# Sreyan88/audio-ssl

Hardware: AMD Instinct MI355X
Metric: upstream clips/sec (1s@16kHz, 64-mel) (higher is better)
Workload: dtype bf16; 1 GPU; delores-m upstream step (log-mel + 2 views + q/k conv encoders + MoCo + 3 Barlow heads + bwd + SGD), 1 s @ 16 kHz, 64 mel, batch 512/GPU, queue 65536; global_batch=512, parallelism=dp1

## Files before the change

audio-ssl_amd/csrc/bnpool.hip:

```cpp
#include "common.h"

namespace {

template <typename T_, bool SQ>
__global__ __launch_bounds__(256) void colstats_kernel(const T_* __restrict__ x, long M, int C, long ld, int rows_per_block,
                                                       double* __restrict__ sum, double* __restrict__ sumsq) {
    __shared__ float red[256][17];
    const int cg = threadIdx.x & 7, r0 = threadIdx.x >> 3;
    const int col0 = blockIdx.y * 64 + cg * 8;
    const long row_begin = (long)blockIdx.x * rows_per_block;
    const long row_end = min(M, row_begin + rows_per_block);
    x += (long)blockIdx.z * M * ld;
    sum += (long)blockIdx.z * C;
    if (SQ) sumsq += (long)blockIdx.z * C;
    float s[8], q[8];
#pragma unroll
    for (int i = 0; i < 8; ++i) { s[i] = 0.f; q[i] = 0.f; }
    if (col0 < C)
        for (long r = row_begin + r0; r < row_end; r += 32) {
            const Vec8<T_> v = Vec8<T_>::load(x + r * ld + col0);
#pragma unroll
            for (int i = 0; i < 8; ++i) { const float f = v.get(i); s[i] += f; if (SQ) q[i] += f * f; }
        }
#pragma unroll
    for (int i = 0; i < 8; ++i) { red[threadIdx.x][i] = s[i]; red[threadIdx.x][8 + i] = q[i]; }
    __syncthreads();
    if (threadIdx.x < 128) {
        const int g = threadIdx.x >> 4, k = threadIdx.x & 15;
        if (SQ || k < 8) {
            double t = 0.0;
            for (int r = 0; r < 32; ++r) t += (double)red[r * 8 + g][k];
            const int c = blockIdx.y * 64 + g * 8 + (k & 7);
            if (c < C) {
                if (k < 8) atomicAdd(&sum[c], t);
                else       atomicAdd(&sumsq[c], t);
            }
        }
    }
}

__global__ void bn_finalize_kernel(const double* __restrict__ sum, const double* __restrict__ sumsq, int groups, double count,
                                   int C, const float* __restrict__ gamma, const float* __restrict__ beta, float* running_mean,
                                   float* running_var, float momentum, float eps, float* scale, float* shift,
                                   float* save_mean, float* save_rstd) {
    const int c = blockIdx.x * blockDim.x + threadIdx.x;
    if (c >= C) return;
    const double g = gamma ? (double)gamma[c] : 1.0, b = beta ? (double)beta[c] : 0.0;
    float rm = running_mean ? running_mean[c] : 0.f, rv = running_mean ? running_var[c] : 0.f;
    for (int k = 0; k < groups; ++k) {
        const int o = k * C + c;
        const double mean = sum[o] / count;
        double var = sumsq[o] / count - mean * mean;
        var = var < 0.0 ? 0.0 : var;
        const double rstd = 1.0 / sqrt(var + (double)eps);
        scale[o] = (float)(g * rstd);
        shift[o] = (float)(b - mean * g * rstd);
        save_mean[o] = (float)mean;
        save_rstd[o] = (float)rstd;
        rm = (1.f - momentum) * rm + momentum * (float)mean;
        const double unb = count > 1.0 ? var * count / (count - 1.0) : var;
        rv = (1.f - momentum) * rv + momentum * (float)unb;
    }
    if (running_mean) { running_mean[c] = rm; running_var[c] = rv; }
}

template <typename TY, typename T_>
__global__ __launch_bounds__(256) void bn_relu_pool_fwd_kernel(const TY* __restrict__ Y, const float* __restrict__ scale,
                                                               const float* __restrict__ shift, T_* __restrict__ P,
                                                               int N, int Ti, int Fi) {
    const int To = Ti / 2, Fo = Fi / 2;
    const long total = (long)N * To * Fo * 8;
    const long idx = (long)blockIdx.x * 256 + threadIdx.x;
    if (idx >= total) return;
    const int c8 = (int)(idx & 7);
    long r = idx >> 3;
    const int fo = (int)(r % Fo); r /= Fo;
    const int to = (int)(r % To);
    const int n = (int)(r / To);
    float sc[8], sh[8], m[8];
#pragma unroll
    for (int i = 0; i < 8; ++i) { sc[i] = scale[c8 * 8 + i]; sh[i] = shift[c8 * 8 + i]; m[i] = 0.f; }
#pragma unroll
    for (int df = 0; df < 2; ++df)
#pragma unroll
        for (int dt = 0; dt < 2; ++dt) {
            const Vec8<TY> v = Vec8<TY>::load(Y + ((((long)n * Ti + 2 * to + dt) * Fi + 2 * fo + df) * 64 + c8 * 8));
#pragma unroll
            for (int i = 0; i < 8; ++i) m[i] = fmaxf(m[i], sc[i] * v.get(i) + sh[i]);
        }
    Vec8<T_> o;
#pragma unroll
    for (int i = 0; i < 8; ++i) o.set(i, m[i]);
    o.store(P + idx * 8);
}

template <typename TY, typename T_>
__global__ __launch_bounds__(256) void bn_relu_pool_train_fwd_kernel(const TY* __restrict__ Y, const double* __restrict__ sum,
                                                                     const double* __restrict__ sumsq, int stat_rep, double count,
                                                                     const float* __restrict__ gamma, const float* __restrict__ beta,
                                                                     float* running_mean, float* running_var, float momentum, float eps,
                                                                     T_* __restrict__ P, float* __restrict__ scale,
                                                                     float* __restrict__ shift, float* __restrict__ save_mean,
                                                                     float* __restrict__ save_rstd, int N, int Ti, int Fi) {
    __shared__ float sc_s[64], sh_s[64];
    if (threadIdx.x < 64) {
        const int c = threadIdx.x;
        const double g = (double)gamma[c], b = (double)beta[c];
        double s1 = 0.0, s2 = 0.0;
        for (int r = 0; r < stat_rep; ++r) { s1 += sum[r * 128 + c]; s2 += sumsq[r * 128 + c]; }
        const double mean = s1 / count;
        double var = s2 / count - mean * mean;
        var = var < 0.0 ? 0.0 : var;
        const double rstd = 1.0 / sqrt(var + (double)eps);
        const float sc = (float)(g * rstd), sh = (float)(b - mean * g * rstd);
        sc_s[c] = sc; sh_s[c] = sh;
        if (blockIdx.x == 0) {
            scale[c] = sc; shift[c] = sh; save_mean[c] = (float)mean; save_rstd[c] = (float)rstd;
            if (running_mean) {
                running_mean[c] = (1.f - momentum) * running_mean[c] + momentum * (float)mean;
                const double unb = count > 1.0 ? var * count / (count - 1.0) : var;
                running_var[c] = (1.f - momentum) * running_var[c] + momentum * (float)unb;
            }
        }
    }
    __syncthreads();
    const int To = Ti / 2, Fo = Fi / 2;
    const long total = (long)N * To * Fo * 8;
    const long idx = (long)blockIdx.x * 256 + threadIdx.x;
    if (idx >= total) return;
    const int c8 = (int)(idx & 7);
    long r = idx >> 3;
    const int fo = (int)(r % Fo); r /= Fo;
    const int to = (int)(r % To);
    const int n = (int)(r / To);
    float sc[8], sh[8], m[8];
#pragma unroll
    for (int i = 0; i < 8; ++i) { sc[i] = sc_s[c8 * 8 + i]; sh[i] = sh_s[c8 * 8 + i]; m[i] = 0.f; }
#pragma unroll
    for (int df = 0; df < 2; ++df)
#pragma unroll
        for (int dt = 0; dt < 2; ++dt) {
            const Vec8<TY> v = Vec8<TY>::load(Y + ((((long)n * Ti + 2 * to + dt) * Fi + 2 * fo + df) * 64 + c8 * 8));
#pragma unroll
            for (int i = 0; i < 8; ++i) m[i] = fmaxf(m[i], sc[i] * v.get(i) + sh[i]);
        }
    Vec8<T_> o;
#pragma unroll
    for (int i = 0; i < 8; ++i) o.set(i, m[i]);
    o.store(P + idx * 8);
}

template <typename T_, typename TO>
__device__ __forceinline__ void tmean_body(const T_* __restrict__ P, TO* __restrict__ xl, int N, int To, int Fo);

template <typename T_, typename TO>
__global__ __launch_bounds__(256) void tmean_fwd_kernel(const T_* __restrict__ P, TO* __restrict__ xl, int N, int To, int Fo) {
    tmean_body<T_, TO>(P, xl, N, To, Fo);
}
struct Tmean3 { const void* P[3]; void* xl[3]; int To[3], Fo[3]; const float* parts; };
template <typename T_, typename TO>
__global__ __launch_bounds__(256) void tmean3_fwd_kernel(Tmean3 a, int N) {
    const int l = blockIdx.z;
    if ((int)blockIdx.x * 64 >= a.Fo[l] * 8) return;
    if (!a.P[l]) {
        if (a.parts && l == 0) {
            const long row = (long)a.Fo[0] * 64, tot = (long)N * row;
            const long i = (long)blockIdx.y * row + blockIdx.x * 512 + threadIdx.x * 2;
            if (blockIdx.x * 512 + threadIdx.x * 2 < row) {
                float2 s = *reinterpret_cast<const float2*>(a.parts + i);
#pragma unroll
                for (int k = 1; k < 4; ++k) {
                    const float2 v = *reinterpret_cast<const float2*>(a.parts + k * tot + i);
                    s.x += v.x; s.y += v.y;
                }
                *reinterpret_cast<float2*>(static_cast<float*>(a.xl[0]) + i) = s;
            }
        }
        return;
    }
    tmean_body<T_, TO>(static_cast<const T_*>(a.P[l]), static_cast<TO*>(a.xl[l]), N, a.To[l], a.Fo[l]);
}

template <typename T_, typename TO>
__device__ __forceinline__ void tmean_body(const T_* __restrict__ P, TO* __restrict__ xl, int N, int To, int Fo) {
    __shared__ float red[4][64][9];
    const int lane = threadIdx.x & 63, w = threadIdx.x >> 6;
    const int nv = Fo * 8;
    const int v = blockIdx.x * 64 + lane;
    const int n = blockIdx.y;
    const bool live = v < nv;
    float s[8];
#pragma unroll
    for (int i = 0; i < 8; ++i) s[i] = 0.f;
    if (live) {
        const T_* p = P + ((long)n * To * nv + v) * 8;
#pragma unroll 4
        for (int t = w; t < To; t += 4) {
            const Vec8<T_> x = Vec8<T_>::load(p + (long)t * nv * 8);
#pragma unroll
            for (int i = 0; i < 8; ++i) s[i] += x.get(i);
        }
    }
#pragma unroll
    for (int i = 0; i < 8; ++i) red[w][lane][i] = s[i];
    __syncthreads();
    if (w == 0 && live) {
        Vec8<TO> o;
        const float inv = 1.f / (float)To;
#pragma unroll
        for (int i = 0; i < 8; ++i) o.set(i, (red[0][lane][i] + red[1][lane][i] + red[2][lane][i] + red[3][lane][i]) * inv);
        o.store(xl + ((long)n * nv + v) * 8);
    }
}

template <typename TY, bool APPLY, typename TG, typename T_>
__global__ __launch_bounds__(256) void bn_relu_pool_bwd_kernel(const TY* __restrict__ Y, const TG* __restrict__ dP,
                                                               const TG* __restrict__ dxl, float inv_To,
                                                               const float* __restrict__ scale, const float* __restrict__ shift,
                                                               const float* __restrict__ mean, const float* __restrict__ rstd,
                                                               float* __restrict__ stat, float inv_count,
                                                               T_* __restrict__ dY, int N, int Ti, int Fi, int fold,
                                                               float* dgamma, float* dbeta) {
    __shared__ float red[256][16];
    __shared__ float folded[128];
    if (APPLY && fold) {
        if (threadIdx.x < 128) {
            float t = 0.f;
            for (int r = 0; r < 32; ++r) t += stat[128 + r * 128 + threadIdx.x];
            folded[threadIdx.x] = t;
        }
        __syncthreads();
        if (blockIdx.x == 0 && threadIdx.x < 64 && dgamma) {
            dbeta[threadIdx.x] += folded[threadIdx.x];
            dgamma[threadIdx.x] += folded[64 + threadIdx.x];
        }
    }
    const int To = Ti / 2, Fo = Fi / 2;
    const int Tq = (Ti + 1) / 2;
    const long total = (long)N * Tq * Fo * 8;
    const long idx = (long)blockIdx.x * 256 + threadIdx.x;
    const bool live = idx < total;
    float db[8], dg[8];
#pragma unroll
    for (int i = 0; i < 8; ++i) { db[i] = 0.f; dg[i] = 0.f; }
    if (live) {
        const int c8 = (int)(idx & 7);
        long r = idx >> 3;
        const int fo = (int)(r % Fo); r /= Fo;
        const int tq = (int)(r % Tq);
        const int n = (int)(r / Tq);
        const bool pooled = tq < To;
        float sc[8], sh[8], mu[8], rs[8], g[8], cb[8], cg[8];
#pragma unroll
        for (int i = 0; i < 8; ++i) {
            const int c = c8 * 8 + i;
            sc[i] = scale[c]; sh[i] = shift[c]; mu[i] = mean[c]; rs[i] = rstd[c]; g[i] = 0.f;
            if (APPLY) { cb[i] = (fold ? folded[c] : stat[c]) * inv_count; cg[i] = (fold ? folded[64 + c] : stat[64 + c]) * inv_count; }
        }
        if (pooled) {
            const Vec8<TG> gp = Vec8<TG>::load(dP + ((((long)n * To + tq) * Fo + fo) * 64 + c8 * 8));
#pragma unroll
            for (int i = 0; i < 8; ++i) g[i] = gp.get(i);
            if (dxl) {
                const Vec8<TG> gx = Vec8<TG>::load(dxl + ((long)n * Fo * 64 + fo * 64 + c8 * 8));
#pragma unroll
                for (int i = 0; i < 8; ++i) g[i] += gx.get(i) * inv_To;
            }
        }
        Vec8<TY> y[4];
        int best[8];
        float bm[8];
#pragma unroll
        for (int i = 0; i < 8; ++i) { best[i] = 0; bm[i] = 0.f; }
#pragma unroll
        for (int p = 0; p < 4; ++p) {
            const int df = p >> 1, dt = p & 1;
            const int t = 2 * tq + dt;
            if (t < Ti) y[p] = Vec8<TY>::load(Y + ((((long)n * Ti + t) * Fi + 2 * fo + df) * 64 + c8 * 8));
            else y[p] = Vec8<TY>::zero();
#pragma unroll
            for (int i = 0; i < 8; ++i) {
                const float a = sc[i] * y[p].get(i) + sh[i];
                if (p == 0 || a > bm[i]) { bm[i] = a; best[i] = p; }
            }
        }
#pragma unroll
        for (int i = 0; i < 8; ++i) {
            const float da = (pooled && bm[i] > 0.f) ? g[i] : 0.f;
            g[i] = da;
            if (!APPLY) {
                float yb = y[0].get(i);
#pragma unroll
                for (int p = 1; p < 4; ++p) yb = best[i] == p ? y[p].get(i) : yb;
                db[i] = da;
                dg[i] = da * (yb - mu[i]) * rs[i];
            }
        }
        if (APPLY) {
#pragma unroll
            for (int p = 0; p < 4; ++p) {
                const int df = p >> 1, dt = p & 1;
                const int t = 2 * tq + dt;
                if (t >= Ti) continue;
                Vec8<T_> o;
#pragma unroll
                for (int i = 0; i < 8; ++i) {
                    const float xhat = (y[p].get(i) - mu[i]) * rs[i];
                    const float da = best[i] == p ? g[i] : 0.f;
                    o.set(i, sc[i] * (da - cb[i] - xhat * cg[i]));
                }
                o.store(dY + ((((long)n * Ti + t) * Fi + 2 * fo + df) * 64 + c8 * 8));
            }
        }
    }
    if (!APPLY) {
#pragma unroll
        for (int i = 0; i < 8; ++i) { red[threadIdx.x][i] = db[i]; red[threadIdx.x][8 + i] = dg[i]; }
        __syncthreads();
        if (threadIdx.x < 128) {
            const int kind = threadIdx.x >> 6, c = threadIdx.x & 63;
            float t = 0.f;
            for (int r = (c >> 3); r < 256; r += 8) t += red[r][kind * 8 + (c & 7)];
            atomicAdd(&stat[128 + (blockIdx.x & 31) * 128 + kind * 64 + c], t);
        }
    }
}

template <typename TP, typename TG>
__global__ __launch_bounds__(256) void bn_pool_bwd_stats_p_kernel(const TP* __restrict__ P, const TG* __restrict__ dP,
                                                                  const TG* __restrict__ dxl, float inv_To,
                                                                  const float* __restrict__ scale, const float* __restrict__ shift,
                                                                  const float* __restrict__ mean, const float* __restrict__ rstd,
                                                                  float* __restrict__ stat, int N, int To, int Fo) {
    __shared__ float red[256][16];
    const long total = (long)N * To * Fo * 8;
    float db[8], dg[8];
#pragma unroll
    for (int i = 0; i < 8; ++i) { db[i] = 0.f; dg[i] = 0.f; }
    const int c8 = threadIdx.x & 7;
    float k1[8], k0[8];
#pragma unroll
    for (int i = 0; i < 8; ++i) {
        const int c = c8 * 8 + i;
        const float sc = scale[c], inv = sc != 0.f ? 1.f / sc : 0.f;
        k1[i] = inv * rstd[c];
        k0[i] = sc != 0.f ? -(shift[c] * inv + mean[c]) * rstd[c] : 0.f;
    }
    for (long idx = (long)blockIdx.x * 256 + threadIdx.x; idx < total; idx += (long)gridDim.x * 256) {
        const long pos = idx >> 3;
        const Vec8<TP> pv = Vec8<TP>::load(P + pos * 64 + c8 * 8);
        const Vec8<TG> gp = Vec8<TG>::load(dP + pos * 64 + c8 * 8);
        float g[8];
#pragma unroll
        for (int i = 0; i < 8; ++i) g[i] = gp.get(i);
        if (dxl) {
            const long n = pos / ((long)To * Fo);
            const int fo = (int)(pos % Fo);
            const Vec8<TG> gx = Vec8<TG>::load(dxl + (n * Fo + fo) * 64 + c8 * 8);
#pragma unroll
            for (int i = 0; i < 8; ++i) g[i] += gx.get(i) * inv_To;
        }
#pragma unroll
        for (int i = 0; i < 8; ++i) {
            const float a = pv.get(i);
            const float da = a > 0.f ? g[i] : 0.f;
            db[i] += da;
            dg[i] += da * (a * k1[i] + k0[i]);
        }
    }
#pragma unroll
    for (int i = 0; i < 8; ++i) { red[threadIdx.x][i] = db[i]; red[threadIdx.x][8 + i] = dg[i]; }
    __syncthreads();
    if (threadIdx.x < 128) {
        const int kind = threadIdx.x >> 6, c = threadIdx.x & 63;
        float t = 0.f;
        for (int r = (c >> 3); r < 256; r += 8) t += red[r][kind * 8 + (c & 7)];
        atomicAdd(&stat[128 + (blockIdx.x & 31) * 128 + kind * 64 + c], t);
    }
}

__global__ void stat_reduce_kernel(float* stat) {
    const int i = threadIdx.x;
    if (i >= 128) return;
    float t = 0.f;
    for (int r = 0; r < 32; ++r) t += stat[128 + r * 128 + i];
    stat[i] = t;
}

template <typename T_>
__global__ __launch_bounds__(256) void im2col_kernel(const T_* __restrict__ X, T_* __restrict__ col, int N, int Ti, int Fi) {
    const long total = (long)N * Ti * Fi * 72;
    const long idx = (long)blockIdx.x * 256 + threadIdx.x;
    if (idx >= total) return;
    const int k8 = (int)(idx % 72);
    long pix = idx / 72;
    const int tap = k8 >> 3, c8 = k8 & 7;
    const int f = (int)(pix % Fi);
    const long r = pix / Fi;
    const int t = (int)(r % Ti);
    const long n = r / Ti;
    const int ff = f + tap / 3 - 1, tt = t + tap % 3 - 1;
    Vec8<T_> v = Vec8<T_>::zero();
    if (ff >= 0 && ff < Fi && tt >= 0 && tt < Ti) v = Vec8<T_>::load(X + (((n * Ti + tt) * Fi + ff) * 64 + c8 * 8));
    v.store(col + idx * 8);
}

template <typename T_>
__global__ void pack_conv_w_kernel(const float* __restrict__ W, T_* __restrict__ Wf, T_* __restrict__ Wd) {
    const int idx = blockIdx.x * 256 + threadIdx.x;
    if (idx >= 64 * 576) return;
    const int row = idx / 576, k = idx % 576, tap = k / 64, c = k % 64;
    Wf[idx] = from_f32<T_>(W[(row * 64 + c) * 9 + tap]);
    Wd[idx] = from_f32<T_>(W[(c * 64 + row) * 9 + (8 - tap)]);
}

template <typename T_>
__global__ void pack_conv_w2_kernel(const float* __restrict__ Wa, T_* __restrict__ Wfa, T_* __restrict__ Wda,
                                    const float* __restrict__ Wb, T_* __restrict__ Wfb, T_* __restrict__ Wdb) {
    const int idx = blockIdx.x * 256 + threadIdx.x;
    if (idx >= 64 * 576) return;
    const float* W = blockIdx.y ? Wb : Wa;
    T_* Wf = blockIdx.y ? Wfb : Wfa;
    T_* Wd = blockIdx.y ? Wdb : Wda;
    const int row = idx / 576, k = idx % 576, tap = k / 64, c = k % 64;
    Wf[idx] = from_f32<T_>(W[(row * 64 + c) * 9 + tap]);
    Wd[idx] = from_f32<T_>(W[(c * 64 + row) * 9 + (8 - tap)]);
}

__global__ void unpack_conv_dw_kernel(const float* __restrict__ dWp, float* __restrict__ dW) {
    const int idx = blockIdx.x * 256 + threadIdx.x;
    if (idx >= 64 * 576) return;
    const int co = idx / 576, k = idx % 576, tap = k / 64, ci = k % 64;
    dW[(co * 64 + ci) * 9 + tap] += dWp[idx];
}

}

extern "C" int audiossl_colstats(int dtype, const void* x, int groups, long M, int C, long ld, int want_sq, double* sum,
                                 double* sumsq, void* stream) {
    ASSL_REQUIRE(x && sum && groups > 0 && M > 0 && C > 0 && (C % 8) == 0 && (ld % 8) == 0);
    ASSL_REQUIRE((dtype == 0 || dtype == 1) && (!want_sq || sumsq));
    hipStream_t s = static_cast<hipStream_t>(stream);
    const size_t nb = sizeof(double) * C * groups;
    if (want_sq && sumsq == sum + (size_t)C * groups) {
        ASSL_ZERO(sum, 2 * nb, s);
    } else {
        ASSL_ZERO(sum, nb, s);
        if (want_sq) ASSL_ZERO(sumsq, nb, s);
    }
    const int slabs = (C + 63) / 64;
    long it = (M * slabs * groups + 32L * 2048 - 1) / (32L * 2048);
    it = it < 1 ? 1 : (it > 128 ? 128 : it);
    const int rpb = 32 * (int)it;
    const dim3 grid(ceil_div(M, rpb), slabs, groups);
    assl_dispatch(dtype, [&](auto t) { using T = typename decltype(t)::type;
        if (want_sq) hipLaunchKernelGGL((colstats_kernel<T, true>), grid, dim3(256), 0, s, static_cast<const T*>(x), M, C, ld, rpb, sum, sumsq);
        else         hipLaunchKernelGGL((colstats_kernel<T, false>), grid, dim3(256), 0, s, static_cast<const T*>(x), M, C, ld, rpb, sum, sumsq);
    });
    ASSL_LAUNCH_CHECK();
}

extern "C" int audiossl_bn_finalize(const double* sum, const double* sumsq, int groups, double count, int C,
                                    const float* gamma, const float* beta, float* running_mean, float* running_var,
                                    float momentum, float eps, float* scale, float* shift, float* save_mean, float* save_rstd,
                                    void* stream) {
    ASSL_REQUIRE(sum && sumsq && scale && shift && save_mean && save_rstd && C > 0 && count > 0 && groups > 0);
    hipLaunchKernelGGL(bn_finalize_kernel, dim3(ceil_div(C, 256)), dim3(256), 0, static_cast<hipStream_t>(stream), sum, sumsq,
                       groups, count, C, gamma, beta, running_mean, running_var, momentum, eps, scale, shift, save_mean, save_rstd);
    ASSL_LAUNCH_CHECK();
}

extern "C" int audiossl_bn_relu_pool_fwd(int dtype, int ydtype, const void* Y, const float* scale, const float* shift, void* P,
                                         int N, int Ti, int Fi, void* stream) {
    ASSL_REQUIRE(Y && scale && shift && P && N > 0 && Ti >= 2 && Fi >= 2 && (Fi % 2) == 0 && (dtype == 0 || dtype == 1));
    ASSL_REQUIRE(ydtype == 0 || ydtype == dtype);
    const long total = (long)N * (Ti / 2) * (Fi / 2) * 8;
    assl_dispatch(dtype, [&](auto to, auto ty) { using TO = typename decltype(to)::type; using TY = typename decltype(ty)::type;
        hipLaunchKernelGGL((bn_relu_pool_fwd_kernel<TY, TO>), dim3(ceil_div(total, 256)), dim3(256), 0, S_(stream),
                           static_cast<const TY*>(Y), scale, shift, static_cast<TO*>(P), N, Ti, Fi);
    }, ydtype);
    ASSL_LAUNCH_CHECK();
}

extern "C" int audiossl_bn_relu_pool_train_fwd(int dtype, int ydtype, const void* Y, const double* sum, const double* sumsq,
                                               int stat_replicas, double count,
                                               const float* gamma, const float* beta, float* running_mean, float* running_var,
                                               float momentum, float eps, void* P, float* scale, float* shift, float* save_mean,
                                               float* save_rstd, int N, int Ti, int Fi, void* stream) {
    ASSL_REQUIRE(Y && sum && sumsq && gamma && beta && P && scale && shift && save_mean && save_rstd && count > 0.0);
    ASSL_REQUIRE(stat_replicas >= 1 && (stat_replicas == 1 || sumsq == sum + 64));
    ASSL_REQUIRE(N > 0 && Ti >= 2 && Fi >= 2 && (Fi % 2) == 0 && (dtype == 0 || dtype == 1) && (ydtype == 0 || ydtype == dtype));
    const long total = (long)N * (Ti / 2) * (Fi / 2) * 8;
    assl_dispatch(dtype, [&](auto to, auto ty) { using TO = typename decltype(to)::type; using TY = typename decltype(ty)::type;
        hipLaunchKernelGGL((bn_relu_pool_train_fwd_kernel<TY, TO>), dim3(ceil_div(total, 256)), dim3(256), 0, S_(stream),
                           static_cast<const TY*>(Y), sum, sumsq, stat_replicas, count, gamma, beta, running_mean, running_var,
                           momentum, eps, static_cast<TO*>(P), scale, shift, save_mean, save_rstd, N, Ti, Fi);
    }, ydtype);
    ASSL_LAUNCH_CHECK();
}

extern "C" int audiossl_tmean_fwd(int dtype, int out_f32, const void* P, void* xl, int N, int To, int Fo, void* stream) {
    ASSL_REQUIRE(P && xl && N > 0 && To > 0 && Fo > 0 && (dtype == 0 || dtype == 1));
    assl_dispatch(dtype, [&](auto ti, auto to) { using TI = typename decltype(ti)::type; using TO = typename decltype(to)::type;
        hipLaunchKernelGGL((tmean_fwd_kernel<TI, TO>), dim3(ceil_div(Fo * 8, 64), N), dim3(256), 0, S_(stream), static_cast<const TI*>(P),
                           static_cast<TO*>(xl), N, To, Fo);
    }, out_f32 ? 0 : dtype);
    ASSL_LAUNCH_CHECK();
}

extern "C" int audiossl_tmean3_fwd(int dtype, int out_f32, const void* P1, void* x1, const float* x1_parts, int To1, int Fo1,
                                   const void* P2, void* x2, int To2, int Fo2, const void* P3, void* x3, int To3, int Fo3, int N,
                                   void* stream) {
    ASSL_REQUIRE(x1 && P2 && x2 && P3 && x3 && N > 0 && To1 > 0 && To2 > 0 && To3 > 0 && Fo1 > 0 && Fo2 > 0 && Fo3 > 0);
    ASSL_REQUIRE((P1 != nullptr) != (x1_parts != nullptr) && (!x1_parts || (out_f32 && dtype == 1)));
    ASSL_REQUIRE(dtype == 0 || dtype == 1);
    Tmean3 a{{P1, P2, P3}, {x1, x2, x3}, {To1, To2, To3}, {Fo1, Fo2, Fo3}, x1_parts};
    const int gx = ceil_div(max(Fo1, max(Fo2, Fo3)) * 8, 64);
    assl_dispatch(dtype, [&](auto ti, auto to) { using TI = typename decltype(ti)::type; using TO = typename decltype(to)::type;
        hipLaunchKernelGGL((tmean3_fwd_kernel<TI, TO>), dim3(gx, N, 3), dim3(256), 0, S_(stream), a, N);
    }, out_f32 ? 0 : dtype);
    ASSL_LAUNCH_CHECK();
}

namespace {
__global__ void add_stat_kernel(const float* __restrict__ stat, float* dgamma, float* dbeta) {
    const int c = threadIdx.x;
    if (c < 64) { dbeta[c] += stat[c]; dgamma[c] += stat[64 + c]; }
}
}

static int bn_relu_pool_bwd_run(int phase, int dtype, int ydtype, int gdtype, const void* Y, const void* P, const void* dP, const void* dxl,
                                const float* scale, const float* shift, const float* mean, const float* rstd, float* stat,
                                const float* gstat, double count, void* dY, float* dgamma, float* dbeta, int N, int Ti, int Fi,
                                void* stream) {
    ASSL_REQUIRE(Y && dP && scale && shift && mean && rstd && stat);
    ASSL_REQUIRE(N > 0 && Ti >= 2 && Fi >= 2 && (Fi % 2) == 0 && (dtype == 0 || dtype == 1) && (gdtype == 0 || gdtype == dtype));
    ASSL_REQUIRE(ydtype == 0 || ydtype == dtype);
    ASSL_REQUIRE(phase == 1 || (dY && dgamma && dbeta));
    hipStream_t s = static_cast<hipStream_t>(stream);
    if (phase != 2) ASSL_ZERO(stat, sizeof(float) * 128 * 33, s);
    const long total = (long)N * ((Ti + 1) / 2) * (Fi / 2) * 8;
    const int grid = ceil_div(total, 256);
    const float inv_To = 1.f / (float)(Ti / 2);
    const float inv_count = (float)(1.0 / (phase == 2 ? count : (double)N * Ti * Fi));
    float* apply_stat = phase == 2 ? const_cast<float*>(gstat) : stat;
    const int fold = phase == 0;
    const long ptotal = (long)N * (Ti / 2) * (Fi / 2) * 8;
    const int pgrid = (int)min((long)2048, (ptotal + 255) / 256);
    assl_dispatch(dtype, [&](auto to, auto ty, auto tg) {
        using TO = typename decltype(to)::type; using TY = typename decltype(ty)::type; using TG = typename decltype(tg)::type;
        const TY* y = static_cast<const TY*>(Y);
        const TG *g = static_cast<const TG*>(dP), *gx = static_cast<const TG*>(dxl);
        TO* dy = static_cast<TO*>(dY);
        if (phase != 2) {
            if (P) hipLaunchKernelGGL((bn_pool_bwd_stats_p_kernel<TO, TG>), dim3(pgrid), dim3(256), 0, s, static_cast<const TO*>(P), g, gx,
                                      inv_To, scale, shift, mean, rstd, stat, N, Ti / 2, Fi / 2);
            else hipLaunchKernelGGL((bn_relu_pool_bwd_kernel<TY, false, TG, TO>), dim3(grid), dim3(256), 0, s, y, g, gx, inv_To, scale,
                                    shift, mean, rstd, stat, inv_count, dy, N, Ti, Fi, 0, dgamma, dbeta);
            if (!fold) hipLaunchKernelGGL(stat_reduce_kernel, dim3(1), dim3(128), 0, s, stat);
        }
        if (phase != 1) hipLaunchKernelGGL((bn_relu_pool_bwd_kernel<TY, true, TG, TO>), dim3(grid), dim3(256), 0, s, y, g, gx, inv_To,
                                           scale, shift, mean, rstd, apply_stat, inv_count, dy, N, Ti, Fi, fold, dgamma, dbeta);
    }, ydtype, gdtype);
    if (phase == 2) hipLaunchKernelGGL(add_stat_kernel, dim3(1), dim3(64), 0, s, stat, dgamma, dbeta);
    ASSL_LAUNCH_CHECK();
}

extern "C" int audiossl_bn_relu_pool_bwd(int dtype, int ydtype, int gdtype, const void* Y, const void* dP, const void* dxl, const float* scale,
                                         const float* shift, const float* mean, const float* rstd, float* stat, void* dY,
                                         float* dgamma, float* dbeta, int N, int Ti, int Fi, void* stream) {
    return bn_relu_pool_bwd_run(0, dtype, ydtype, gdtype, Y, nullptr, dP, dxl, scale, shift, mean, rstd, stat, nullptr, 0.0, dY, dgamma, dbeta, N,
                                Ti, Fi, stream);
}
extern "C" int audiossl_bn_relu_pool_bwd_p(int dtype, int ydtype, int gdtype, const void* Y, const void* P, const void* dP, const void* dxl,
                                           const float* scale, const float* shift, const float* mean, const float* rstd, float* stat,
                                           void* dY, float* dgamma, float* dbeta, int N, int Ti, int Fi, void* stream) {
    ASSL_REQUIRE(P);
    return bn_relu_pool_bwd_run(0, dtype, ydtype, gdtype, Y, P, dP, dxl, scale, shift, mean, rstd, stat, nullptr, 0.0, dY, dgamma, dbeta, N,
                                Ti, Fi, stream);
}
extern "C" int audiossl_bn_relu_pool_bwd_stats(int dtype, int ydtype, int gdtype, const void* Y, const void* dP, const void* dxl,
                                               const float* scale, const float* shift, const float* mean, const float* rstd,
                                               float* stat, int N, int Ti, int Fi, void* stream) {
    return bn_relu_pool_bwd_run(1, dtype, ydtype, gdtype, Y, nullptr, dP, dxl, scale, shift, mean, rstd, stat, nullptr, 0.0, nullptr, nullptr,
                                nullptr, N, Ti, Fi, stream);
}
extern "C" int audiossl_bn_relu_pool_bwd_apply(int dtype, int ydtype, int gdtype, const void* Y, const void* dP, const void* dxl,
                                               const float* scale, const float* shift, const float* mean, const float* rstd,
                                               float* stat, const float* gstat, double count_global, void* dY, float* dgamma,
                                               float* dbeta, int N, int Ti, int Fi, void* stream) {
    ASSL_REQUIRE(gstat && count_global > 1.0);
    return bn_relu_pool_bwd_run(2, dtype, ydtype, gdtype, Y, nullptr, dP, dxl, scale, shift, mean, rstd, stat, gstat, count_global, dY, dgamma,
                                dbeta, N, Ti, Fi, stream);
}

extern "C" int audiossl_im2col3x3(int dtype, const void* X, void* col, int N, int Ti, int Fi, void* stream) {
    ASSL_REQUIRE(X && col && N > 0 && Ti > 0 && Fi > 0 && (dtype == 0 || dtype == 1));
    const long total = (long)N * Ti * Fi * 72;
    ASSL_REQUIRE((total + 255) / 256 < 2147483647L);
    assl_dispatch(dtype, [&](auto t) { using T = typename decltype(t)::type;
        hipLaunchKernelGGL(im2col_kernel<T>, dim3(ceil_div(total, 256)), dim3(256), 0, S_(stream), static_cast<const T*>(X),
                           static_cast<T*>(col), N, Ti, Fi);
    });
    ASSL_LAUNCH_CHECK();
}

extern "C" int audiossl_pack_conv_w(int dtype, const float* W, void* Wf, void* Wd, void* stream) {
    ASSL_REQUIRE(W && Wf && Wd && (dtype == 0 || dtype == 1));
    assl_dispatch(dtype, [&](auto t) { using T = typename decltype(t)::type;
        hipLaunchKernelGGL(pack_conv_w_kernel<T>, dim3(144), dim3(256), 0, S_(stream), W, static_cast<T*>(Wf), static_cast<T*>(Wd));
    });
    ASSL_LAUNCH_CHECK();
}

extern "C" int audiossl_pack_conv_w2(int dtype, const float* Wa, void* Wfa, void* Wda, const float* Wb, void* Wfb, void* Wdb, void* stream) {
    ASSL_REQUIRE(Wa && Wfa && Wda && Wb && Wfb && Wdb && (dtype == 0 || dtype == 1));
    assl_dispatch(dtype, [&](auto t) { using T = typename decltype(t)::type;
        hipLaunchKernelGGL(pack_conv_w2_kernel<T>, dim3(144, 2), dim3(256), 0, S_(stream), Wa, static_cast<T*>(Wfa), static_cast<T*>(Wda), Wb,
                           static_cast<T*>(Wfb), static_cast<T*>(Wdb));
    });
    ASSL_LAUNCH_CHECK();
}

extern "C" int audiossl_unpack_conv_dw(const float* dWp, float* dW, void* stream) {
    ASSL_REQUIRE(dWp && dW);
    hipLaunchKernelGGL(unpack_conv_dw_kernel, dim3(144), dim3(256), 0, static_cast<hipStream_t>(stream), dWp, dW);
    ASSL_LAUNCH_CHECK();
}
```

audio-ssl_amd/csrc/conv.hip:

```cpp
#include <cstdlib>
#include "common.h"

namespace {

constexpr int CH = 64, KTOT = 576;
constexpr int WPITCH = KTOT + 8;
constexpr int PIXP = 72;
constexpr int PIXW = 96;

typedef __attribute__((address_space(3))) bf16x4* lds4_t;

struct ConvArgs {
    const bf16* X; const bf16* W; const float* bias; bf16* Y; double* sum; double* sumsq;
    int Ti, rows_total, tiles, out_f32, dbg, stat_rep;
};

template <int FI, int PITCH, int NTH = 256>
struct Halo {
    static constexpr int TT = 256 / FI;
    static constexpr int COLS = FI + 2;
    static constexpr int ELEMS = (TT + 2) * COLS * PITCH;
    static constexpr int NV = ((TT + 2) * FI * 8 + NTH - 1) / NTH;
    static constexpr int NVEC = (TT + 2) * FI * 8;
    Vec8<bf16> r[NV];
    __device__ __forceinline__ void load(const bf16* __restrict__ X, int g0, int rows_total) {
#pragma unroll
        for (int i = 0; i < NV; ++i) {
            const int v = threadIdx.x + i * NTH;
            const int row = v / (FI * 8), rem = v % (FI * 8);
            const int gr = g0 - 1 + row;
            r[i] = (v < NVEC && gr >= 0 && gr < rows_total) ? Vec8<bf16>::load(X + ((long)gr * FI) * CH + rem * 8) : Vec8<bf16>::zero();
        }
    }
    __device__ __forceinline__ void put(bf16* lds) const {
#pragma unroll
        for (int i = 0; i < NV; ++i) {
            const int v = threadIdx.x + i * NTH;
            const int row = v / (FI * 8), rem = v % (FI * 8);
            if (v < NVEC) r[i].store(lds + (row * COLS + (rem >> 3) + 1) * PITCH + (rem & 7) * 8);
        }
    }
    __device__ __forceinline__ static void zero_border(bf16* lds) {
        for (int i = threadIdx.x; i < (TT + 2) * 2 * 8; i += NTH) {
            const int row = i / 16, side = (i >> 3) & 1, c8 = i & 7;
            Vec8<bf16>::zero().store(lds + (row * COLS + side * (FI + 1)) * PITCH + c8 * 8);
        }
    }
};

template <int FI, int NW>
__global__ __launch_bounds__(64 * NW, 1) void conv3x3_kernel(ConvArgs a) {
    using H = Halo<FI, PIXP, 64 * NW>;
    constexpr int RT = 8 / NW;
    constexpr int TT = H::TT, COLS = H::COLS;
    extern __shared__ __attribute__((aligned(16))) char smem[];
    bf16* const wl = reinterpret_cast<bf16*>(smem);
    bf16* const hl = wl + CH * WPITCH;
    float* const red = reinterpret_cast<float*>(hl);

    const int lane = threadIdx.x & 63, wave = threadIdx.x >> 6;
    const int m = lane & 31, h = lane >> 5;
    for (int v = threadIdx.x; v < CH * KTOT / 8; v += 64 * NW) {
        const int row = v / (KTOT / 8), c = v % (KTOT / 8);
        Vec8<bf16>::load(a.W + row * KTOT + c * 8).store(wl + row * WPITCH + c * 8);
    }
    H::zero_border(hl);

    float ssum[2][16], ssq[2][16];
#pragma unroll
    for (int j = 0; j < 2; ++j)
#pragma unroll
        for (int r = 0; r < 16; ++r) { ssum[j][r] = 0.f; ssq[j][r] = 0.f; }
    f32x4 bias4[2][4];
#pragma unroll
    for (int j = 0; j < 2; ++j)
#pragma unroll
        for (int q = 0; q < 4; ++q)
            bias4[j][q] = a.bias ? *reinterpret_cast<const f32x4*>(a.bias + j * 32 + 8 * q + 4 * h) : f32x4{0.f, 0.f, 0.f, 0.f};
    H halo;
    int tile = blockIdx.x;
    if (tile < a.tiles) { halo.load(a.X, tile * TT, a.rows_total); halo.put(hl); }
    __syncthreads();

    for (; tile < a.tiles; tile += gridDim.x) {
        const int g0 = tile * TT;
        const int next = tile + gridDim.x;
        if (next < a.tiles && !(a.dbg & 2)) halo.load(a.X, next * TT, a.rows_total);

        int tl[RT], fcol[RT];
        bool ok[RT][3];
#pragma unroll
        for (int i = 0; i < RT; ++i) {
            const int rt = RT * wave + i;
            tl[i] = FI == 32 ? rt : 2 * rt + (m >> 4);
            fcol[i] = FI == 32 ? m : (m & 15);
            const int g = g0 + tl[i];
            const int ti = g % a.Ti;
#pragma unroll
            for (int dt = 0; dt < 3; ++dt) ok[i][dt] = g < a.rows_total && ti + dt - 1 >= 0 && ti + dt - 1 < a.Ti;
        }
        f32x16 acc[RT][2];
#pragma unroll
        for (int i = 0; i < RT; ++i)
#pragma unroll
            for (int j = 0; j < 2; ++j)
#pragma unroll
                for (int r = 0; r < 16; ++r) acc[i][j][r] = 0.f;

        if (!(a.dbg & 4))
#pragma unroll
        for (int tap = 0; tap < 9; ++tap) {
            const int dt = tap % 3, df = tap / 3;
#pragma unroll
            for (int cc = 0; cc < 4; ++cc) {
                Vec8<bf16> fa[RT], fb[2];
#pragma unroll
                for (int i = 0; i < RT; ++i) {
                    const bf16* p = hl + ((tl[i] + dt) * COLS + fcol[i] + df) * PIXP + cc * 16 + 8 * h;
                    fa[i] = ok[i][dt] ? Vec8<bf16>::load(p) : Vec8<bf16>::zero();
                }
#pragma unroll
                for (int j = 0; j < 2; ++j) fb[j] = Vec8<bf16>::load(wl + (j * 32 + m) * WPITCH + tap * 64 + cc * 16 + 8 * h);
#pragma unroll
                for (int i = 0; i < RT; ++i)
#pragma unroll
                    for (int j = 0; j < 2; ++j)
                        acc[i][j] = __builtin_amdgcn_mfma_f32_32x32x16_bf16(fb[j].v, fa[i].v, acc[i][j], 0, 0, 0);
            }
        }
#pragma unroll
        for (int i = 0; i < RT; ++i) {
            const int g = g0 + tl[i];
            if (g < a.rows_total && !(a.dbg & 1)) {
                const long o = ((long)g * FI + fcol[i]) * CH;
#pragma unroll
                for (int j = 0; j < 2; ++j)
#pragma unroll
                    for (int q = 0; q < 4; ++q) {
                        f32x4 v;
#pragma unroll
                        for (int e = 0; e < 4; ++e) {
                            v[e] = acc[i][j][4 * q + e] + bias4[j][q][e];
                            ssum[j][4 * q + e] += v[e];
                            ssq[j][4 * q + e] += v[e] * v[e];
                        }
                        const int co = j * 32 + 8 * q + 4 * h;
                        if (a.out_f32) *reinterpret_cast<f32x4*>(reinterpret_cast<float*>(a.Y) + o + co) = v;
                        else *reinterpret_cast<bf16x4*>(a.Y + o + co) = bf16x4{(bf16)v[0], (bf16)v[1], (bf16)v[2], (bf16)v[3]};
                    }
            }
        }
        __syncthreads();
        if (next < a.tiles) halo.put(hl);
        __syncthreads();
    }
    if (a.sum) {
#pragma unroll
        for (int j = 0; j < 2; ++j)
#pragma unroll
            for (int r = 0; r < 16; ++r) {
                float s = ssum[j][r], q = ssq[j][r];
#pragma unroll
                for (int o = 16; o > 0; o >>= 1) { s += __shfl_xor(s, o, 64); q += __shfl_xor(q, o, 64); }
                if (m == 0) {
                    const int co = j * 32 + (r & 3) + 8 * (r >> 2) + 4 * h;
                    red[(wave * 64 + co) * 2] = s; red[(wave * 64 + co) * 2 + 1] = q;
                }
            }
        __syncthreads();
        if (threadIdx.x < 128) {
            const int c = threadIdx.x >> 1, k = threadIdx.x & 1;
            double t = 0.0;
#pragma unroll
            for (int w = 0; w < NW; ++w) t += (double)red[(w * 64 + c) * 2 + k];
            const int rep = (blockIdx.x % a.stat_rep) * 128;
            atomicAdd(k == 0 ? &a.sum[rep + c] : &a.sumsq[rep + c], t);
        }
    }
}

template <int FI>
struct WsGeom {
    static constexpr int TT = 256 / FI, COLS = FI + 2, ROWS = TT + 2, SEGS = FI / 8;
    static constexpr int UNITS = ROWS * SEGS;
    static constexpr int UPW = (UNITS + 3) / 4;
    static constexpr int BYTES = ROWS * COLS * 128;
};

template <int FI, bool STATS, bool F32OUT, int PF = 2>
__global__ __launch_bounds__(256, 1) void conv3x3_ws_kernel(ConvArgs a) {
    using G = WsGeom<FI>;
    constexpr int TT = G::TT, COLS = G::COLS;
    typedef __attribute__((address_space(3))) void* lptr_t;
    extern __shared__ __attribute__((aligned(16))) char smem[];
    float* const biasl = reinterpret_cast<float*>(smem + 2 * G::BYTES);
    float* const red = biasl + 64;
    constexpr int OPIX = F32OUT ? 256 : 128;
    char* const stg = reinterpret_cast<char*>(red + 4 * 64 * 2) + (threadIdx.x >> 6) * 64 * OPIX;
    char* const zblk = reinterpret_cast<char*>(red + 4 * 64 * 2) + 4 * 64 * OPIX;
    if (threadIdx.x < 32) *reinterpret_cast<f32x4*>(zblk + threadIdx.x * 16) = f32x4{0.f, 0.f, 0.f, 0.f};

    const int lane = threadIdx.x & 63, wave = __builtin_amdgcn_readfirstlane(threadIdx.x >> 6);
    const int m = lane & 31, h = lane >> 5;
    long* const rts = (!STATS && (a.dbg & 16) && threadIdx.x == 0 && (blockIdx.x == 0 || blockIdx.x == gridDim.x - 1))
                          ? reinterpret_cast<long*>(a.sum) + 64 + (blockIdx.x ? 8 : 0) : nullptr;
    if (rts) rts[0] = __builtin_amdgcn_s_memrealtime();

    {
        bf16* const wl = reinterpret_cast<bf16*>(smem);
        Vec8<bf16> tmp[CH * KTOT / 8 / 256];
#pragma unroll
        for (int k = 0; k < CH * KTOT / 8 / 256; ++k) tmp[k] = Vec8<bf16>::load(a.W + (threadIdx.x + 256 * k) * 8);
#pragma unroll
        for (int k = 0; k < CH * KTOT / 8 / 256; ++k) {
            const int v = threadIdx.x + 256 * k, row = v / (KTOT / 8), c = v % (KTOT / 8);
            tmp[k].store(wl + row * WPITCH + c * 8);
        }
        __syncthreads();
    }
    Vec8<bf16> wr[2][36];
#pragma unroll
    for (int j = 0; j < 2; ++j)
#pragma unroll
        for (int ks = 0; ks < 36; ++ks)
            wr[j][ks] = Vec8<bf16>::load(reinterpret_cast<const bf16*>(smem) + (j * 32 + m) * WPITCH + ks * 16 + 8 * h);
#pragma unroll
    for (int ks = 0; ks < 36; ++ks) {
        asm volatile("" : "+v"(wr[0][ks].v));
        asm volatile("" : "+a"(wr[1][ks].v));
    }

    __syncthreads();
    for (int i = threadIdx.x; i < 2 * G::ROWS * 2 * 8; i += 256) {
        const int b = i / (G::ROWS * 16), r = (i / 16) % G::ROWS, side = (i >> 3) & 1, c8 = i & 7;
        *reinterpret_cast<f32x4*>(smem + b * G::BYTES + (r * COLS + side * (FI + 1)) * 128 + c8 * 16) = f32x4{0.f, 0.f, 0.f, 0.f};
    }
    if (threadIdx.x < 64) biasl[threadIdx.x] = a.bias ? a.bias[threadIdx.x] : 0.f;

    if (rts) { asm volatile("s_waitcnt vmcnt(0)" ::: "memory"); rts[3] = __builtin_amdgcn_s_memrealtime(); }
    const __amdgpu_buffer_rsrc_t rsrc = __builtin_amdgcn_make_buffer_rsrc(const_cast<bf16*>(a.X), 0, (unsigned)((long)a.rows_total * FI * 128), 0x00020000);
    const int pl = lane >> 3, cp = lane & 7;
    const int key0 = ((1 + pl) >> 1) & 7;
    const int voff0 = pl * 128 + ((cp ^ key0) << 4), voff1 = pl * 128 + ((cp ^ key0 ^ 4) << 4);
    auto dma_unit = [&](int g0, char* buf, int i) {
        {
            const int u = wave + 4 * i;
            if (u < G::UNITS) {
                const int row = u / G::SEGS, seg = u % G::SEGS;
                const int gr = g0 - 1 + row;
                const int so = (gr >= 0 && gr < a.rows_total) ? (gr * FI + 8 * seg) * 128 : 0x7FFFFF00;
                __builtin_amdgcn_raw_ptr_buffer_load_lds(rsrc, (lptr_t)(buf + (row * COLS + 1 + 8 * seg) * 128), 16, (seg & 1) ? voff1 : voff0, so, 0, 0);
            }
        }
    };
    auto dma_tile = [&](int g0, char* buf) {
#pragma unroll
        for (int i = 0; i < G::UPW; ++i) dma_unit(g0, buf, i);
    };

    int tl[2];
    const int fcol = FI == 32 ? m : (m & 15);
#pragma unroll
    for (int i = 0; i < 2; ++i) {
        const int rt = 2 * wave + i;
        tl[i] = FI == 32 ? rt : 2 * rt + (m >> 4);
    }
    int hs[3];
#pragma unroll
    for (int df = 0; df < 3; ++df) hs[df] = (h ^ (((fcol + df) >> 1) & 7)) << 4;

    constexpr int NS = F32OUT ? 4 : 8;
    float ssum[NS], ssq[NS];
    if (STATS) {
#pragma unroll
        for (int e = 0; e < NS; ++e) { ssum[e] = 0.f; ssq[e] = 0.f; }
    }

    int tile = blockIdx.x, cur = 0;
    if (tile < a.tiles) dma_tile(tile * TT, smem);
    asm volatile("s_waitcnt vmcnt(0) lgkmcnt(0)" ::: "memory");
    __builtin_amdgcn_s_barrier();

    long* const ts = (!STATS && (a.dbg & 16) && blockIdx.x == 0 && threadIdx.x == 0) ? reinterpret_cast<long*>(a.sum) : nullptr;
    int tsi = 0;
    if (rts) rts[1] = __builtin_amdgcn_s_memrealtime();
    for (; tile < a.tiles; tile += gridDim.x, cur ^= 1) {
        if (ts) ts[tsi++] = __builtin_amdgcn_s_memtime();
        const int g0 = tile * TT;
        const int next = tile + gridDim.x;
        if (next < a.tiles && !(a.dbg & 2)) dma_tile(next * TT, smem + (cur ^ 1) * G::BYTES);
        const char* const hl = smem + cur * G::BYTES;

        int bdt[2][3];
#pragma unroll
        for (int i = 0; i < 2; ++i) {
            const int g = g0 + tl[i];
            const int ti = g % a.Ti;
#pragma unroll
            for (int dt = 0; dt < 3; ++dt) {
                const bool ok = g < a.rows_total && ti + dt - 1 >= 0 && ti + dt - 1 < a.Ti;
                bdt[i][dt] = ok ? (int)(size_t)((lptr_t)const_cast<char*>(hl)) + ((tl[i] + dt) * COLS + fcol) * 128
                                : (int)(size_t)((lptr_t)zblk);
            }
        }
        f32x16 acc[2][2];
#pragma unroll
        for (int j = 0; j < 2; ++j)
#pragma unroll
            for (int q = 0; q < 4; ++q) {
                const f32x4 b4 = *reinterpret_cast<const f32x4*>(biasl + j * 32 + 8 * q + 4 * h);
#pragma unroll
                for (int e = 0; e < 4; ++e) { acc[0][j][4 * q + e] = b4[e]; acc[1][j][4 * q + e] = b4[e]; }
            }

        Vec8<bf16> fa[PF + 1][2];
        auto fetch = [&](int ks, Vec8<bf16> (&f)[2]) {
            const int tap = ks >> 2, cc = ks & 3, dt = tap % 3, df = tap / 3;
#pragma unroll
            for (int i = 0; i < 2; ++i)
                f[i] = Vec8<bf16>::load(reinterpret_cast<const bf16*>((const char*)(lptr_t)(size_t)(bdt[i][dt] + df * 128 + (hs[df] ^ (cc * 32)))));
        };
        if (!(a.dbg & 4)) {
#pragma unroll
        for (int ks = 0; ks < PF; ++ks) fetch(ks, fa[ks]);
#pragma unroll
        for (int ks = 0; ks < 36; ++ks) {
            if (ks + PF < 36) fetch(ks + PF, fa[(ks + PF) % (PF + 1)]);
            __builtin_amdgcn_sched_barrier(0);
            Vec8<bf16> (&f)[2] = fa[ks % (PF + 1)];
#pragma unroll
            for (int i = 0; i < 2; ++i) {
#pragma unroll
                for (int j = 0; j < 2; ++j)
                    acc[i][j] = __builtin_amdgcn_mfma_f32_32x32x16_bf16(wr[j][ks].v, f[i].v, acc[i][j], 0, 0, 0);
            }
            __builtin_amdgcn_sched_barrier(0);
        }
        }
        if (ts) ts[tsi++] = __builtin_amdgcn_s_memtime();
        asm volatile("s_waitcnt vmcnt(0)" ::: "memory");
        if (ts) ts[tsi++] = __builtin_amdgcn_s_memtime();
        if (!(a.dbg & 1)) {
#pragma unroll
            for (int i = 0; i < 2; ++i) {
                char* const st = stg + i * 32 * OPIX;
#pragma unroll
                for (int j = 0; j < 2; ++j)
#pragma unroll
                    for (int q = 0; q < 4; ++q) {
                        const int slot = j * 8 + 2 * q + h;
                        const f32x4 v = f32x4{acc[i][j][4 * q], acc[i][j][4 * q + 1], acc[i][j][4 * q + 2], acc[i][j][4 * q + 3]};
                        if (F32OUT) *reinterpret_cast<f32x4*>(st + m * 256 + ((slot ^ (m & 15)) << 4)) = v;
                        else *reinterpret_cast<bf16x4*>(st + m * 128 + ((slot ^ ((m >> 1) & 15)) << 3)) =
                                 bf16x4{(bf16)v[0], (bf16)v[1], (bf16)v[2], (bf16)v[3]};
                    }
            }
            asm volatile("s_waitcnt lgkmcnt(0)" ::: "memory");
#pragma unroll
            for (int i = 0; i < 2; ++i) {
                const char* const st = stg + i * 32 * OPIX;
                const int grow = g0 + (2 * wave + i) * (32 / FI);
                const int prow_ok = a.rows_total - grow;
                char* const yrow = reinterpret_cast<char*>(a.Y) + (long)grow * FI * 64 * (F32OUT ? 4 : 2);
                if (F32OUT) {
#pragma unroll
                    for (int it = 0; it < 8; ++it) {
                        const int p = it * 4 + (lane >> 4), c = lane & 15;
                        const f32x4 v = *reinterpret_cast<const f32x4*>(st + p * 256 + ((c ^ (p & 15)) << 4));
                        if ((p >> (FI == 32 ? 5 : 4)) < prow_ok) {
                            *reinterpret_cast<f32x4*>(yrow + p * 256 + c * 16) = v;
                            if (STATS) {
#pragma unroll
                                for (int e = 0; e < 4; ++e) { ssum[e] += v[e]; ssq[e] += v[e] * v[e]; }
                            }
                        }
                    }
                } else {
#pragma unroll
                    for (int it = 0; it < 4; ++it) {
                        const int p = it * 8 + (lane >> 3), c = lane & 7, k = (p >> 1) & 15;
                        f32x4 v = *reinterpret_cast<const f32x4*>(st + p * 128 + ((c ^ (k >> 1)) << 4));
                        if (k & 1) v = f32x4{v[2], v[3], v[0], v[1]};
                        if ((p >> (FI == 32 ? 5 : 4)) < prow_ok) {
                            *reinterpret_cast<f32x4*>(yrow + p * 128 + c * 16) = v;
                            if (STATS) {
                                const bf16x8 hv = __builtin_bit_cast(bf16x8, v);
#pragma unroll
                                for (int e = 0; e < 8; ++e) {
                                    const float x = (float)hv[e];
                                    ssum[e] += x; ssq[e] += x * x;
                                }
                            }
                        }
                    }
                }
            }
        }
        if (ts) ts[tsi++] = __builtin_amdgcn_s_memtime();
        asm volatile("s_waitcnt lgkmcnt(0)" ::: "memory");
        __builtin_amdgcn_s_barrier();
    }
    if (rts) rts[2] = __builtin_amdgcn_s_memrealtime();
    if (STATS) {
#pragma unroll
        for (int e = 0; e < NS; ++e) {
            float s = ssum[e], q = ssq[e];
#pragma unroll
            for (int o = 64 / NS; o < 64; o <<= 1) { s += __shfl_xor(s, o, 64); q += __shfl_xor(q, o, 64); }
            if (lane < 64 / NS) {
                const int co = lane * NS + e;
                red[(wave * 64 + co) * 2] = s; red[(wave * 64 + co) * 2 + 1] = q;
            }
        }
        __syncthreads();
        if (threadIdx.x < 128) {
            const int c = threadIdx.x >> 1, k = threadIdx.x & 1;
            double t = 0.0;
#pragma unroll
            for (int w = 0; w < 4; ++w) t += (double)red[(w * 64 + c) * 2 + k];
            const int rep = (blockIdx.x % a.stat_rep) * 128;
            atomicAdd(k == 0 ? &a.sum[rep + c] : &a.sumsq[rep + c], t);
        }
    }
}

__host__ __device__ __forceinline__ int wg_cot(int w, int n) { return n < 8 ? (n & 1) : (w & 1); }
__host__ __device__ __forceinline__ int wg_nt(int w, int n) { return n < 8 ? 4 * w + (n >> 1) : 16 + (w >> 1); }

struct WgradArgs {
    const bf16* dY; const bf16* X; float* dW; int Ti, rows_total, tiles;
    float* partial;
    int dbg;
};

template <int FI, int KG>
__global__ __launch_bounds__(256 * KG, 1) void conv3x3_wgrad_kernel(WgradArgs a) {
    using H = Halo<FI, PIXW, 256 * KG>;
    constexpr int TT = H::TT, COLS = H::COLS;
    constexpr int NTH = 256 * KG;
    constexpr int NVY = 256 * 8 / NTH;
    extern __shared__ __attribute__((aligned(16))) char smem[];
    bf16* const yl = reinterpret_cast<bf16*>(smem);
    bf16* const hl = yl + 256 * PIXW;

    const int lane = threadIdx.x & 63, wave = (threadIdx.x >> 6) & 3, grp = threadIdx.x >> 8;
    const int h = lane >> 5, half = (lane >> 4) & 1, q = (lane & 15) >> 2, p = lane & 3;
    H::zero_border(hl);

    f32x16 acc[9];
#pragma unroll
    for (int n = 0; n < 9; ++n)
#pragma unroll
        for (int r = 0; r < 16; ++r) acc[n][r] = 0.f;

    H halo;
    Vec8<bf16> ry[NVY];
    auto load_y = [&](int g0) {
#pragma unroll
        for (int i = 0; i < NVY; ++i) {
            const int v = threadIdx.x + i * NTH;
            const long pix = (long)g0 * FI + (v >> 3);
            ry[i] = pix < (long)a.rows_total * FI ? Vec8<bf16>::load(a.dY + pix * CH + (v & 7) * 8) : Vec8<bf16>::zero();
        }
    };
    auto put_y = [&]() {
#pragma unroll
        for (int i = 0; i < NVY; ++i) {
            const int v = threadIdx.x + i * NTH;
            ry[i].store(yl + (v >> 3) * PIXW + (v & 7) * 8);
        }
    };
    int tile = blockIdx.x;
    if (tile < a.tiles) { halo.load(a.X, tile * TT, a.rows_total); load_y(tile * TT); halo.put(hl); put_y(); }
    __syncthreads();

    for (; tile < a.tiles; tile += gridDim.x) {
        const int g0 = tile * TT;
        const int next = tile + gridDim.x;
        if (next < a.tiles && !(a.dbg & 2)) { halo.load(a.X, next * TT, a.rows_total); load_y(next * TT); }

#pragma unroll 1
        for (int ks = grp * (16 / KG); ks < (grp + 1) * (16 / KG) && !(a.dbg & 4); ++ks) {
            const int t_local = FI == 32 ? (ks >> 1) : ks;
            const int f0 = FI == 32 ? (ks & 1) * 16 : 0;
            const int g = g0 + t_local;
            if (g >= a.rows_total) break;
            const int ti = g % a.Ti;
            const bool okt[3] = {ti - 1 >= 0, true, ti + 1 < a.Ti};
            bf16x8 fa[2];
#pragma unroll
            for (int c2 = 0; c2 < 2; ++c2) {
                const bf16* ay = yl + (ks * 16 + 8 * h + q) * PIXW + c2 * 32 + 16 * half + 4 * p;
                const bf16x4 a0 = __builtin_amdgcn_ds_read_tr16_b64_v4bf16((lds4_t)ay);
                const bf16x4 a1 = __builtin_amdgcn_ds_read_tr16_b64_v4bf16((lds4_t)(ay + 4 * PIXW));
                fa[c2] = bf16x8{a0[0], a0[1], a0[2], a0[3], a1[0], a1[1], a1[2], a1[3]};
            }
            bf16x8 fb;
#pragma unroll
            for (int n = 0; n < 9; ++n) {
                if (n == 8 || (n & 1) == 0) {
                    const int nt = wg_nt(wave, n), tap = nt >> 1, cih = nt & 1;
                    const int dt = tap % 3, df = tap / 3;
                    const bf16* bx = hl + ((t_local + dt) * COLS + f0 + df + 8 * h + q) * PIXW + cih * 32 + 16 * half + 4 * p;
                    const bf16x4 b0 = __builtin_amdgcn_ds_read_tr16_b64_v4bf16((lds4_t)bx);
                    const bf16x4 b1 = __builtin_amdgcn_ds_read_tr16_b64_v4bf16((lds4_t)(bx + 4 * PIXW));
                    const bf16 z = (bf16)0.f;
                    fb = okt[dt] ? bf16x8{b0[0], b0[1], b0[2], b0[3], b1[0], b1[1], b1[2], b1[3]} : bf16x8{z, z, z, z, z, z, z, z};
                }
                const int c2 = wg_cot(wave, n);
                acc[n] = __builtin_amdgcn_mfma_f32_32x32x16_bf16(c2 ? fa[1] : fa[0], fb, acc[n], 0, 0, 0);
            }
        }
        __syncthreads();
        if (next < a.tiles) { halo.put(hl); put_y(); }
        __syncthreads();
    }
    if (a.partial) {
        if (KG == 2) {
            f32x4* xch = reinterpret_cast<f32x4*>(smem);
            __syncthreads();
            if (grp == 1) {
#pragma unroll
                for (int n = 0; n < 9; ++n)
#pragma unroll
                    for (int r4 = 0; r4 < 4; ++r4)
                        xch[((wave * 9 + n) * 4 + r4) * 64 + lane] = f32x4{acc[n][4 * r4], acc[n][4 * r4 + 1], acc[n][4 * r4 + 2], acc[n][4 * r4 + 3]};
            }
            __syncthreads();
            if (grp == 1) return;
            f32x4* part = reinterpret_cast<f32x4*>(a.partial + (long)blockIdx.x * (CH * KTOT));
#pragma unroll
            for (int n = 0; n < 9; ++n)
#pragma unroll
                for (int r4 = 0; r4 < 4; ++r4) {
                    const f32x4 o = xch[((wave * 9 + n) * 4 + r4) * 64 + lane];
                    part[((wave * 9 + n) * 4 + r4) * 64 + lane] = f32x4{acc[n][4 * r4] + o[0], acc[n][4 * r4 + 1] + o[1], acc[n][4 * r4 + 2] + o[2], acc[n][4 * r4 + 3] + o[3]};
                }
            return;
        }
        f32x4* part = reinterpret_cast<f32x4*>(a.partial + (long)blockIdx.x * (CH * KTOT));
#pragma unroll
        for (int n = 0; n < 9; ++n)
#pragma unroll
            for (int r4 = 0; r4 < 4; ++r4)
                part[((wave * 9 + n) * 4 + r4) * 64 + lane] = f32x4{acc[n][4 * r4], acc[n][4 * r4 + 1], acc[n][4 * r4 + 2], acc[n][4 * r4 + 3]};
        return;
    }
#pragma unroll
    for (int n = 0; n < 9; ++n) {
        const int nt = wg_nt(wave, n), tap = nt >> 1, cih = nt & 1;
        const int col = tap * 64 + cih * 32 + (lane & 31);
#pragma unroll
        for (int r = 0; r < 16; ++r) {
            const int co = wg_cot(wave, n) * 32 + (r & 3) + 8 * (r >> 2) + 4 * h;
            atomicAdd(&a.dW[co * KTOT + col], acc[n][r]);
        }
    }
}

__global__ __launch_bounds__(256) void wgrad_reduce_kernel(const float* __restrict__ partial, int nparts, float* __restrict__ dW) {
    const int i = blockIdx.x * 256 + threadIdx.x;
    if (i >= CH * KTOT) return;
    float s0 = 0.f, s1 = 0.f, s2 = 0.f, s3 = 0.f;
    int w = blockIdx.y;
    const int step = gridDim.y;
    for (; w + 3 * step < nparts; w += 4 * step) {
        s0 += partial[(long)w * (CH * KTOT) + i];
        s1 += partial[(long)(w + step) * (CH * KTOT) + i];
        s2 += partial[(long)(w + 2 * step) * (CH * KTOT) + i];
        s3 += partial[(long)(w + 3 * step) * (CH * KTOT) + i];
    }
    for (; w < nparts; w += step) s0 += partial[(long)w * (CH * KTOT) + i];
    const int e = i & 3, lane = (i >> 2) & 63, r4 = (i >> 8) & 3, wn = i >> 10;
    const int wave = wn / 9, n = wn - wave * 9;
    const int nt = wg_nt(wave, n), tap = nt >> 1, cih = nt & 1;
    const int col = tap * 64 + cih * 32 + (lane & 31);
    const int co = wg_cot(wave, n) * 32 + e + 8 * r4 + 4 * (lane >> 5);
    atomicAdd(&dW[co * KTOT + col], (s0 + s1) + (s2 + s3));
}

template <typename K>
int set_lds(K kernel, size_t bytes) {
    return hipFuncSetAttribute(reinterpret_cast<const void*>(kernel), hipFuncAttributeMaxDynamicSharedMemorySize, (int)bytes) ==
           hipSuccess ? 0 : -1;
}

}

extern "C" int audiossl_conv3x3_fwd(const void* X, const void* W, const float* bias, void* Y, int out_f32, double* sum,
                                    double* sumsq, int stat_replicas, int N, int Ti, int Fi, void* stream) {
    ASSL_REQUIRE(X && W && Y && N > 0 && Ti > 0 && (Fi == 32 || Fi == 16) && (!sum == !sumsq));
    ASSL_REQUIRE(stat_replicas >= 1 && stat_replicas <= 64 && (stat_replicas == 1 || !sum || sumsq == sum + 64));
    if (!ASSL_ALIGNED16(X) || !ASSL_ALIGNED16(W) || !ASSL_ALIGNED16(Y)) return ASSL_EALIGN;
    hipStream_t s = static_cast<hipStream_t>(stream);
#ifdef AUDIOSSL_ABLATE
    static const int conv_dbg = getenv("AUDIOSSL_CONV_DBG") ? atoi(getenv("AUDIOSSL_CONV_DBG")) : 0;
#else
    constexpr int conv_dbg = 0;
#endif
    if (sum && !(conv_dbg & 16)) {
        if (sumsq == sum + 64) {
            ASSL_ZERO(sum, sizeof(double) * 128 * stat_replicas, s);
        } else {
            ASSL_ZERO(sum, sizeof(double) * 64, s);
            ASSL_ZERO(sumsq, sizeof(double) * 64, s);
        }
    }
    const int rows = N * Ti, TT = 256 / Fi, tiles = (rows + TT - 1) / TT;
    ConvArgs a{static_cast<const bf16*>(X), static_cast<const bf16*>(W), bias, static_cast<bf16*>(Y), sum, sumsq, Ti, rows, tiles, out_f32, conv_dbg, stat_replicas};
    const int grid = tiles < 256 ? tiles : 256;
    static const int ws = getenv("AUDIOSSL_CONV_WS") ? atoi(getenv("AUDIOSSL_CONV_WS")) : 1;
    if (ws && (long)rows * Fi * 128 < 0x7FFFFF00L) {
        static bool wattr[8] = {false, false, false, false, false, false, false, false};
#define WS_LAUNCH(FI_, ST_, F32_, SLOT)                                                                    \
    do {                                                                                                  \
        const size_t lds = 2 * WsGeom<FI_>::BYTES + sizeof(float) * (64 + 4 * 64 * 2) + 4 * 64 * (F32_ ? 256 : 128) + 512; \
        if (!wattr[SLOT]) { if (set_lds(conv3x3_ws_kernel<FI_, ST_, F32_>, lds)) return ASSL_ELAUNCH; wattr[SLOT] = true; } \
        hipLaunchKernelGGL((conv3x3_ws_kernel<FI_, ST_, F32_>), dim3(grid), dim3(256), lds, s, a);       \
    } while (0)
        if (Fi == 32) {
            if (sum && !(conv_dbg & 16)) { if (out_f32) WS_LAUNCH(32, true, true, 0); else WS_LAUNCH(32, true, false, 1); }
            else     { if (out_f32) WS_LAUNCH(32, false, true, 2); else WS_LAUNCH(32, false, false, 3); }
        } else {
            if (sum) { if (out_f32) WS_LAUNCH(16, true, true, 4); else WS_LAUNCH(16, true, false, 5); }
            else     { if (out_f32) WS_LAUNCH(16, false, true, 6); else WS_LAUNCH(16, false, false, 7); }
        }
#undef WS_LAUNCH
        ASSL_LAUNCH_CHECK();
    }
    static const int nw = getenv("AUDIOSSL_CONV_WAVES") ? atoi(getenv("AUDIOSSL_CONV_WAVES")) : 8;
    static bool attr[4] = {false, false, false, false};
#define CONV_LAUNCH(FI_, NW_, SLOT)                                                                       \
    do {                                                                                                  \
        const size_t lds = sizeof(bf16) * (CH * WPITCH + Halo<FI_, PIXP>::ELEMS);                         \
        if (!attr[SLOT]) { if (set_lds(conv3x3_kernel<FI_, NW_>, lds)) return ASSL_ELAUNCH; attr[SLOT] = true; } \
        hipLaunchKernelGGL((conv3x3_kernel<FI_, NW_>), dim3(grid), dim3(64 * NW_), lds, s, a);           \
    } while (0)
    if (Fi == 32) { if (nw == 8) CONV_LAUNCH(32, 8, 0); else CONV_LAUNCH(32, 4, 1); }
    else          { if (nw == 8) CONV_LAUNCH(16, 8, 2); else CONV_LAUNCH(16, 4, 3); }
#undef CONV_LAUNCH
    ASSL_LAUNCH_CHECK();
}

extern "C" int audiossl_conv3x3_wgrad(const void* dY, const void* X, float* dWp, float* workspace, long workspace_floats, int N,
                                      int Ti, int Fi, void* stream) {
    ASSL_REQUIRE(dY && X && dWp && N > 0 && Ti > 0 && (Fi == 32 || Fi == 16));
    if (!ASSL_ALIGNED16(X) || !ASSL_ALIGNED16(dY)) return ASSL_EALIGN;
    hipStream_t s = static_cast<hipStream_t>(stream);
    const int rows = N * Ti, TT = 256 / Fi, tiles = (rows + TT - 1) / TT;
    const int grid = tiles < 256 ? tiles : 256;
    const bool two_stage = workspace != nullptr && workspace_floats >= (long)grid * CH * KTOT;
#ifdef AUDIOSSL_ABLATE
    static const int wg_dbg = getenv("AUDIOSSL_CONV_DBG") ? atoi(getenv("AUDIOSSL_CONV_DBG")) : 0;
#else
    constexpr int wg_dbg = 0;
#endif
    WgradArgs a{static_cast<const bf16*>(dY), static_cast<const bf16*>(X), dWp, Ti, rows, tiles, two_stage ? workspace : nullptr, wg_dbg};
    static const int kg_env = getenv("AUDIOSSL_WGRAD_KG") ? atoi(getenv("AUDIOSSL_WGRAD_KG")) : 0;
    const int kg = kg_env ? kg_env : (two_stage ? 2 : 1);
    static bool attr[4] = {false, false, false, false};
#define WGRAD_LAUNCH(FI_, KG_, SLOT)                                                                      \
    do {                                                                                                  \
        const size_t lds = max(sizeof(bf16) * (256 * PIXW + Halo<FI_, PIXW>::ELEMS), (size_t)(KG_ == 2 ? 4 * 9 * 16 * 64 * 4 : 0)); \
        if (!attr[SLOT]) { if (set_lds(conv3x3_wgrad_kernel<FI_, KG_>, lds)) return ASSL_ELAUNCH; attr[SLOT] = true; } \
        hipLaunchKernelGGL((conv3x3_wgrad_kernel<FI_, KG_>), dim3(grid), dim3(256 * KG_), lds, s, a);    \
    } while (0)
    if (Fi == 32) { if (kg == 2) WGRAD_LAUNCH(32, 2, 0); else WGRAD_LAUNCH(32, 1, 1); }
    else          { if (kg == 2) WGRAD_LAUNCH(16, 2, 2); else WGRAD_LAUNCH(16, 1, 3); }
#undef WGRAD_LAUNCH
    if (two_stage)
        hipLaunchKernelGGL(wgrad_reduce_kernel, dim3(CH * KTOT / 256, 8), dim3(256), 0, s, workspace, grid, dWp);
    ASSL_LAUNCH_CHECK();
}
```

audio-ssl_amd/src/encoder/audiontt.py:

```python
import logging
import os
import re
from pathlib import Path

import torch
from torch import nn

from src import _native as N
from src import engine as E

_DROPOUT_IN_GEMM = os.environ.get("AUDIOSSL_DROPOUT_IN_GEMM", "1") != "0"


def default_precision():
    return {"fp32": N.F32, "bf16": N.BF16}[os.environ.get("AUDIOSSL_PRECISION", "bf16")]


class NetworkCommonMixIn():

    def load_weight(self, weight_file, device):
        state_dict = torch.load(weight_file, map_location=device, weights_only=True)
        if 'state_dict' in state_dict:
            state_dict = state_dict['state_dict']
        weights = {}
        for k in state_dict:
            m = re.search(r'(^fc\.|\.fc\.|^features\.|\.features\.)', k)
            if m is None:
                continue
            new_k = k[m.start():]
            weights[new_k[1:] if new_k[0] == '.' else new_k] = state_dict[k]
        self.load_state_dict(weights)
        self.eval()
        logging.info(f'Using audio embbeding network pretrained weight: {Path(weight_file).name}')
        return self

    def set_trainable(self, trainable=False):
        for p in self.parameters():
            p.requires_grad = trainable


class DropoutMasks:

    def __init__(self, p=0.3, seed=0x5EED):
        self.p, self.seed, self.queue = p, seed, []
        self.counter = None

    @property
    def calls(self):
        return 0 if self.counter is None else int(self.counter[0])

    def next(self, M, d, device, virtual=False):
        if self.queue:
            m = self.queue.pop(0)
            return m.reshape(M, d).to(device=device, dtype=torch.uint8).contiguous()
        if self.counter is None or self.counter.device != torch.device(device):
            self.counter = torch.zeros(1, dtype=torch.int64, device=device)
        self.counter.add_(1)
        vk = VirtualKeep((self.seed * 0x9E3779B1) & 0xFFFFFFFFFFFF, self.p, self.counter, M, d)
        return vk if virtual else vk.materialise()


class VirtualKeep:

    def __init__(self, seed, p, counter, M, d):
        self.seed, self.p, self.counter, self.M, self.d = seed, p, counter, M, d

    def materialise(self):
        keep = torch.empty(self.M, self.d, dtype=torch.uint8, device=self.counter.device)
        N.call("dropout_mask", keep, self.M * self.d, self.seed, self.p, self.counter)
        return keep


class _EncoderFn(torch.autograd.Function):

    @staticmethod
    def forward(ctx, mod, x, keep, *params):
        P = mod.param_dict()
        x1, x2, x3, h, c = E.encoder_forward(P, x, mod.precision, keep=keep, p_drop=mod.fc[2].p, train=mod.training)
        ctx.mod, ctx.c = mod, c
        return x1, x2, x3, h

    @staticmethod
    def backward(ctx, g1, g2, g3, gh):
        mod, c = ctx.mod, ctx.c
        td = N.torch_dtype(c.dtype)
        P = mod.param_dict()
        names = mod.engine_param_names()
        G = {n: torch.zeros_like(P[n], dtype=torch.float32) for n in names}

        def prep(g, like):
            return None if g is None else g.float().contiguous()
        gh = torch.zeros_like(c.H2.view(c.N, -1, c.d)) if gh is None else gh.to(td).contiguous()
        E.encoder_backward(c, G, dH2=gh.view(c.M, c.d), dx1=prep(g1, None), dx2=prep(g2, None), dx3=prep(g3, None))
        return (None, None, None) + tuple(G[n] for n in names)


class AudioNTT2020Task6(nn.Module, NetworkCommonMixIn):

    def __init__(self, n_mels, d, return_all_layers):
        super().__init__()
        self.return_all_layers = return_all_layers

        def block(cin):
            return nn.Sequential(nn.Conv2d(cin, 64, 3, stride=1, padding=1), nn.BatchNorm2d(64), nn.ReLU(),
                                 nn.MaxPool2d(2, stride=2))
        self.features_1 = block(1)
        self.features_2 = block(64)
        self.features_3 = block(64)
        self.fc = nn.Sequential(nn.Linear(64 * (n_mels // (2 ** 3)), d), nn.ReLU(), nn.Dropout(p=0.3), nn.Linear(d, d),
                                nn.ReLU())
        self.d = d
        self.n_mels = n_mels
        self.precision = default_precision()
        self.dropout_masks = DropoutMasks(0.3)

    def param_dict(self):
        from src.flat import cached_param_dict
        return cached_param_dict(self)

    def engine_param_names(self):
        return [n for n, _ in self.named_parameters()]

    def next_keep_mask(self, n_img, T):
        if not self.training:
            return None
        return self.dropout_masks.next(n_img * (T // 8), self.d, self.fc[0].weight.device, virtual=_DROPOUT_IN_GEMM)

    def forward(self, x):
        if not x.is_cuda:
            raise RuntimeError("AudioNTT2020Task6 (HIP) needs a GPU tensor - there is no CPU fallback")
        x = x.float().contiguous()
        keep = self.next_keep_mask(x.shape[0], x.shape[-1])
        params = tuple(p for _, p in self.named_parameters())
        if torch.is_grad_enabled() and any(p.requires_grad for p in params):
            x1, x2, x3, h = _EncoderFn.apply(self, x, keep, *params)
        else:
            x1, x2, x3, h, _ = E.encoder_forward(self.param_dict(), x, self.precision, keep=keep, p_drop=self.fc[2].p,
                                                 train=self.training)
        if self.return_all_layers:
            return x1, x2, x3, h
        return h

    def __repr__(self):
        return "AudioNTT2020Task6"
```

audio-ssl_amd/src/engine.py:

```python
import os

import torch

from src import _native as N

import os as _os
_STEM_VALU = _os.environ.get("AUDIOSSL_STEM_VALU") == "1"
BN_MOMENTUM = 0.1
BN_EPS = 1e-5
_BN_FUSED = _os.environ.get("AUDIOSSL_BN_FUSED", "1") != "0"


ONE_STREAM = os.environ.get("AUDIOSSL_ONE_STREAM", "0") == "1"


_CAPTURE_ORIGIN = []


class capture_scope:

    def __enter__(self):
        _CAPTURE_ORIGIN.append(torch.cuda.current_stream())
        return self

    def __exit__(self, *exc):
        _CAPTURE_ORIGIN.pop()
        return False


def fork(side, parent=None, device=None):
    parent = parent if parent is not None else torch.cuda.current_stream(device)
    if _CAPTURE_ORIGIN and parent.cuda_stream != _CAPTURE_ORIGIN[-1].cuda_stream and side.cuda_stream != _CAPTURE_ORIGIN[-1].cuda_stream \
            and os.environ.get("AUDIOSSL_ALLOW_NESTED_FORK", "0") != "1":
        raise RuntimeError("nested stream fork inside a hipGraph capture: a side stream may only be forked from the capture's origin "
                           "stream (a fork from an already forked stream crashed hipStreamEndCapture on ROCm 7.2 - engine.py, "
                           "DESIGN.md section 7); restructure the step or set AUDIOSSL_ALLOW_NESTED_FORK=1 to experiment")
    side.wait_stream(parent)


class SideStream:

    def __init__(self):
        self._streams = {}

    def stream(self, device):
        if ONE_STREAM:
            return torch.cuda.current_stream(device)
        key = str(device)
        if key not in self._streams:
            self._streams[key] = torch.cuda.Stream(device=device)
        return self._streams[key]

    def run(self, device, fn):
        if ONE_STREAM:
            return fn()
        s = self.stream(device)
        fork(s, torch.cuda.current_stream(device))
        with torch.cuda.stream(s):
            return fn()

    def join(self, device):
        if not ONE_STREAM:
            torch.cuda.current_stream(device).wait_stream(self.stream(device))


WGRAD = SideStream()


def _empty(shape, dtype, like=None, device=None):
    return torch.empty(shape, dtype=dtype, device=device if device is not None else like.device)


class ZeroArena:

    def __init__(self, nbytes=8 << 20):
        self.nbytes, self.buf, self.off, self.active = nbytes, None, 0, False

    def step(self, device):
        arena = self

        class _Ctx:
            def __enter__(self_):
                if arena.buf is None or arena.buf.device != device:
                    arena.buf = torch.empty(arena.nbytes, dtype=torch.uint8, device=device)
                arena.off, arena.active = 0, True
                arena.buf.zero_()
                N.call_host("set_prezeroed", 1)

            def __exit__(self_, *exc):
                arena.active = False
                N.call_host("set_prezeroed", 0)
                return False
        return _Ctx()

    def zeros(self, shape, dtype, like=None, device=None):
        dev = device if device is not None else like.device
        if self.active and self.buf.device == dev:
            n = 1
            for d in (shape if isinstance(shape, (tuple, list)) else (shape,)):
                n *= int(d)
            nb = n * torch.empty((), dtype=dtype).element_size()
            if self.off + nb <= self.nbytes:
                t = self.buf[self.off:self.off + nb].view(dtype).view(shape)
                self.off += (nb + 255) // 256 * 256
                return t
        return torch.zeros(shape, dtype=dtype, device=dev)

    def scratch(self, shape, dtype, like):
        return self.zeros(shape, dtype, like=like) if self.active else _empty(shape, dtype, like=like)


ARENA = ZeroArena()


def fast_copy(dst, src):
    n = src.numel()
    if src.dtype == torch.float32 and dst.dtype == torch.float32 and src.is_contiguous() and dst.is_contiguous() and n % 1024 == 0 \
            and n // 1024 < (1 << 31) and src.data_ptr() % 16 == 0 and dst.data_ptr() % 16 == 0:
        N.call("tile_rows", src, dst, n // 1024, n // 1024, 1, 1.0, 1024)
    else:
        dst.copy_(src)
    return dst


def _ksplit(M, Nn, K, target=512):
    tiles = ((M + 127) // 128) * ((Nn + 127) // 128)
    return int(max(1, min(target // max(tiles, 1), (K // 64) // 32)))


def gemm(dtype, ta, tb, M, Nn, K, A, lda, B, ldb, C, ldc, alpha=1.0, bias=None, relu=0, keep=None, ldk=0, keep_scale=1.0,
         gate=None, ldg=0, out_f32=0, atomic=0, ksplit=1, resid=None, ldr=0):
    N.call("gemm", dtype, ta, tb, M, Nn, K, float(alpha), A, lda, B, ldb, C, ldc, bias, relu, keep, ldk, float(keep_scale),
           gate, ldg, out_f32, atomic, ksplit, resid, ldr)


def linear_fwd(dtype, X, W, M, Nout, K, bias=None, relu=0, keep=None, keep_scale=1.0, out=None, out_f32=0):
    if out is None and dtype == N.BF16 and out_f32 and not relu and keep is None and M * Nout <= (1 << 16) and K >= 1024 and K % 512 == 0:
        out = ARENA.zeros((M, Nout), torch.float32, like=X)
        gemm(dtype, 0, 0, M, Nout, K, X, K, W, K, out, Nout, bias=bias, out_f32=1, atomic=1, ksplit=min(8, K // 256))
        return out
    if out is None:
        out = _empty((M, Nout), torch.float32 if (out_f32 or dtype == 0) else torch.bfloat16, like=X)
    gemm(dtype, 0, 0, M, Nout, K, X, K, W, K, out, Nout, bias=bias, relu=relu, keep=keep, ldk=Nout, keep_scale=keep_scale,
         out_f32=out_f32)
    return out


def linear_bwd_w(dtype, dY, X, dW, M, Nout, K, dw_zero=False):
    ks = _ksplit(Nout, K, M)
    atomic = 1 if (ks > 1 or dtype != N.BF16) else (0 if dw_zero else 2)
    gemm(dtype, 1, 1, Nout, K, M, dY, Nout, X, K, dW, K, out_f32=1, atomic=atomic, ksplit=ks)


def linear_bwd_x(dtype, dY, W, M, Nout, K, alpha=1.0, gate=None, out=None, out_f32=0):
    if out is None:
        out = _empty((M, K), torch.float32 if (out_f32 or dtype == N.F32) else torch.bfloat16, like=dY)
    gemm(dtype, 0, 1, M, K, Nout, dY, Nout, W, K, out, K, alpha=alpha, gate=gate, ldg=K, out_f32=out_f32)
    return out


GD = N.F32

HP = False


def set_high_precision(flag):
    global HP
    HP = bool(flag)


SYNC_BN = None


class SyncBN:
    def __init__(self, group=None):
        import torch.distributed as dist
        self.dist, self.group = dist, group
        self.world = dist.get_world_size(group)

    def all_reduce(self, t):
        self.dist.all_reduce(t, group=self.group)
        return t


def set_sync_bn(sync):
    global SYNC_BN
    SYNC_BN = sync if (sync is not None and sync.world > 1) else None


def _ad(dtype):
    return N.F32 if (HP or dtype == N.F32) else dtype


def pooled_dtype(dtype):
    return torch.float32


def center_cast(Y, groups, B):
    C = Y.shape[1]
    yc = _empty((groups * B, C), torch.bfloat16, like=Y)
    cmean = _empty((groups, C), torch.float32, like=Y)
    N.call("center_cast", Y, yc, cmean, groups, B, C)
    return yc, cmean


def colsum_add(dtype, X, M, C, dst, tmp=None):
    tmp = tmp if tmp is not None else ARENA.scratch((C,), torch.float64, X)
    N.call("colstats", dtype, X, 1, M, C, C, 0, tmp, None)
    N.call("add_d2f", tmp, dst, C)


def cast(dtype, src, n=None):
    if dtype == N.F32:
        return src
    out = torch.empty(src.shape, dtype=torch.bfloat16, device=src.device)
    N.call("cast", dtype, src, out, src.numel())
    return out


class EncoderCtx:
    pass


def _bn_train(dtype, Y, M, C, gamma, beta, rm, rv, update_running, groups=1):
    sq = ARENA.scratch((2, groups * C), torch.float64, Y)
    N.call("colstats", dtype, Y, groups, M, C, C, 1, sq[0], sq[1])
    if SYNC_BN is not None:
        SYNC_BN.all_reduce(sq)
        M = M * SYNC_BN.world
    st = _empty((4, groups * C), torch.float32, like=Y)
    N.call("bn_finalize", sq[0], sq[1], groups, float(M), C, gamma, beta, rm if update_running else None,
           rv if update_running else None, BN_MOMENTUM, BN_EPS, st[0], st[1], st[2], st[3])
    return st[0], st[1], st[2], st[3]


def bn_train_apply(dtype, ad, a, M, C, gamma, beta, rm, rv, update_running, groups, relu, out):
    if M <= 1024 and C % 32 == 0 and _BN_FUSED and SYNC_BN is None:
        st = _empty((4, groups * C), torch.float32, like=a)
        N.call("colbn_train_fwd", dtype, ad, a, gamma, beta, rm if update_running else None, rv if update_running else None,
               BN_MOMENTUM, BN_EPS, relu, groups, M, C, out, st[0], st[1], st[2], st[3])
        return st[0], st[1], st[2], st[3]
    st = _bn_train(ad, a, M, C, gamma, beta, rm, rv, update_running, groups)
    N.call("colbn_fwd", dtype, ad, a, st[0], st[1], relu, out, groups, M, C)
    return st


def _bn_eval(like, C, gamma, beta, rm, rv):
    scale, shift = _empty((C,), torch.float32, like=like), _empty((C,), torch.float32, like=like)
    N.call("bn_eval_affine", gamma, beta, rm, rv, BN_EPS, C, scale, shift)
    return scale, shift


_WGRAD_WS = {}


def _wgrad_workspace(device):
    key = device.index if device.index is not None else torch.cuda.current_device()
    ws = _WGRAD_WS.get(key)
    if ws is None:
        ws = _WGRAD_WS[key] = torch.empty(256 * 64 * 576, dtype=torch.float32, device=device)
    return ws


STAT_REPLICAS = 8
LOSS_REPLICAS = 32
_BN_STATS_P = os.environ.get("AUDIOSSL_BN_STATS_P", "1") != "0"
_DP1_BF16 = os.environ.get("AUDIOSSL_DP1_BF16", "1") != "0"


def _conv_block_fwd(dtype, Pin, Nimg, Ti, Fi, W, bias, bn, train, update_running, col, packed=None):
    td = N.torch_dtype(dtype)
    if packed is not None:
        Wf, Wd = packed
    else:
        Wf, Wd = _empty((64, 576), td, like=Pin), _empty((64, 576), td, like=Pin)
        N.call("pack_conv_w", dtype, W, Wf, Wd)
    M = Nimg * Ti * Fi
    ad = _ad(dtype)
    Y = _empty((M, 64), N.torch_dtype(ad), like=Pin)
    gamma, beta, rm, rv = bn
    fused = dtype == N.BF16 and Fi in (16, 32)
    rep = STAT_REPLICAS if (fused and train and SYNC_BN is None) else 1
    sq = ARENA.scratch((rep, 2, 64), torch.float64, Pin) if (fused and train) else None
    if fused:
        N.call("conv3x3_fwd", Pin, Wf, bias, Y, int(ad == N.F32), None if sq is None else sq[0, 0], None if sq is None else sq[0, 1],
               rep, Nimg, Ti, Fi)
    else:
        N.call("im2col3x3", dtype, Pin, col, Nimg, Ti, Fi)
        gemm(dtype, 0, 0, M, 64, 576, col, 576, Wf, 576, Y, 64, bias=bias, out_f32=int(ad == N.F32))
    Pout = _empty((Nimg, Ti // 2, Fi // 2, 64), td, like=Pin)
    if train and fused and SYNC_BN is None:
        st = _empty((4, 64), torch.float32, like=Pin)
        N.call("bn_relu_pool_train_fwd", dtype, ad, Y, sq[0, 0], sq[0, 1], rep, float(M), gamma, beta, rm if update_running else None,
               rv if update_running else None, BN_MOMENTUM, BN_EPS, Pout, st[0], st[1], st[2], st[3], Nimg, Ti, Fi)
        return Y, Pout, (st[0], st[1], st[2], st[3]), Wf, Wd
    if train and fused:
        st = _empty((4, 64), torch.float32, like=Pin)
        sq = sq[0]
        SYNC_BN.all_reduce(sq)
        N.call("bn_finalize", sq[0], sq[1], 1, float(M * SYNC_BN.world), 64, gamma, beta, rm if update_running else None,
               rv if update_running else None, BN_MOMENTUM, BN_EPS, st[0], st[1], st[2], st[3])
        scale, shift, mean, rstd = st[0], st[1], st[2], st[3]
    elif train:
        scale, shift, mean, rstd = _bn_train(ad, Y, M, 64, gamma, beta, rm, rv, update_running)
    else:
        scale, shift = _bn_eval(Y, 64, gamma, beta, rm, rv)
        mean = rstd = None
    N.call("bn_relu_pool_fwd", dtype, ad, Y, scale, shift, Pout, Nimg, Ti, Fi)
    return Y, Pout, (scale, shift, mean, rstd), Wf, Wd


def _col_buffer(dtype, Nimg, T1, F1, like):
    if dtype == N.BF16 and F1 in (16, 32):
        return None
    return _empty((Nimg * T1 * F1, 576), N.torch_dtype(dtype), like=like)


MOM_SLOT = 17 * 54


def stem_fused(dtype, train=True):
    return bool(train) and dtype == N.BF16 and not HP and not _STEM_VALU and SYNC_BN is None


def stem_moments_pair(xa, xb=None):
    Nimg, _, F, T = xa.shape
    assert xb is None or xb.shape == xa.shape
    mom = ARENA.scratch((1 if xb is None else 2, MOM_SLOT), torch.float64, xa)
    N.call("conv1_moments_pair", xa.reshape(Nimg, F, T).contiguous(), None if xb is None else xb.reshape(Nimg, F, T).contiguous(),
           Nimg, F, T, mom)
    return mom


def encoder_forward(P, x, dtype, keep=None, p_drop=0.3, train=True, update_running=True, want_layers=True, Wc=None,
                    layer_out=None, before_fc=None, stem_moments=None):
    Nimg, _, F, T = x.shape
    assert F == 64, "the HIP encoder is built for n_mels = 64 (the reference's only setting)"
    td = N.torch_dtype(dtype)
    c = EncoderCtx()
    c.P = P
    c.dtype, c.N, c.F, c.T, c.train, c.p_drop = dtype, Nimg, F, T, train, p_drop
    img = x.reshape(Nimg, F, T).contiguous()
    c.img = img
    w1 = P["features_1.0.weight"].reshape(64, 9)
    b1 = P["features_1.0.bias"]
    g1, be1 = P["features_1.1.weight"], P["features_1.1.bias"]
    c.stem_mfma = dtype == N.BF16 and not HP and not _STEM_VALU
    fused = stem_fused(dtype, train)
    assert stem_moments is None or fused, "precomputed stem moments are for the fused bf16 training stem only"
    rm1 = rv1 = None
    if train:
        c.sc1, c.sh1, c.mean1, c.rstd1 = (_empty((64,), torch.float32, like=x) for _ in range(4))
        rm1 = P["features_1.1.running_mean"] if update_running else None
        rv1 = P["features_1.1.running_var"] if update_running else None
    if fused:
        c.mom1 = stem_moments if stem_moments is not None else stem_moments_pair(x)[0]
    elif train:
        c.mom1 = ARENA.scratch((16 * 54,), torch.float64, x)
        if SYNC_BN is None:
            N.call("conv1_stats", img, Nimg, F, T, w1, b1, g1, be1, rm1, rv1, BN_MOMENTUM, BN_EPS, c.mom1, c.sc1, c.sh1, c.mean1, c.rstd1)
        else:
            N.call("conv1_moments", img, Nimg, F, T, c.mom1)
            mom_g = SYNC_BN.all_reduce(c.mom1[:54].clone())
            N.call("conv1_finalize", mom_g, w1, b1, g1, be1, rm1, rv1, BN_MOMENTUM, BN_EPS, float(Nimg * F * T * SYNC_BN.world),
                   c.sc1, c.sh1, c.mean1, c.rstd1)
    else:
        c.sc1, c.sh1 = _bn_eval(x, 64, g1, be1, P["features_1.1.running_mean"], P["features_1.1.running_var"])
    T1, F1 = T // 2, F // 2
    c.P1 = _empty((Nimg, T1, F1, 64), td, like=x)
    x1 = x2 = x3 = None
    if want_layers:
        x1, x2, x3 = layer_out if layer_out is not None else (_empty((Nimg, f * 64), td, like=x) for f in (F // 2, F // 4, F // 8))
    x1_fused = c.stem_mfma and x1 is not None and x1.dtype == torch.float32 and x1.is_contiguous()
    x1_parts = _empty((4, Nimg, (F // 2) * 64), torch.float32, like=x) if x1_fused else None
    if fused:
        N.call("conv1_fwd_train", img, Nimg, F, T, c.mom1, float(Nimg * F * T), w1, b1, g1, be1, rm1, rv1, BN_MOMENTUM, BN_EPS,
               c.sc1, c.sh1, c.mean1, c.rstd1, c.P1, x1_parts)
    else:
        N.call("conv1_fwd", dtype if (dtype == N.F32 or c.stem_mfma) else 2, img, Nimg, F, T, w1, b1, c.sc1, c.sh1, c.P1, x1_parts)
    col = _col_buffer(dtype, Nimg, T1, F1, x)
    bn2 = (P["features_2.1.weight"], P["features_2.1.bias"], P["features_2.1.running_mean"], P["features_2.1.running_var"])
    packs = [_empty((64, 576), td, like=x) for _ in range(4)]
    N.call("pack_conv_w2", dtype, P["features_2.0.weight"], packs[0], packs[1], P["features_3.0.weight"], packs[2], packs[3])
    c.Y2, c.P2, c.st2, c.W2f, c.W2d = _conv_block_fwd(dtype, c.P1, Nimg, T1, F1, P["features_2.0.weight"],
                                                       P["features_2.0.bias"], bn2, train, update_running, col, packed=packs[:2])
    T2, F2 = T1 // 2, F1 // 2
    bn3 = (P["features_3.1.weight"], P["features_3.1.bias"], P["features_3.1.running_mean"], P["features_3.1.running_var"])
    c.Y3, c.P3, c.st3, c.W3f, c.W3d = _conv_block_fwd(dtype, c.P2, Nimg, T2, F2, P["features_3.0.weight"],
                                                       P["features_3.0.bias"], bn3, train, update_running, col, packed=packs[2:])
    del col
    T3, F3 = T2 // 2, F2 // 2
    c.dims = (T1, F1, T2, F2, T3, F3)
    if want_layers:
        o32 = int(x1.dtype == torch.float32)
        N.call("tmean3_fwd", dtype, o32, None if x1_fused else c.P1, x1, x1_parts, T1, F1, c.P2, x2, T2, F2, c.P3, x3, T3, F3, Nimg)
    d = P["fc.0.weight"].shape[0]
    kin = F3 * 64
    M = Nimg * T3
    c.d, c.kin, c.M = d, kin, M
    if before_fc is not None:
        before_fc()
    if Wc is not None:
        c.fw1, c.fw2 = Wc["fc.0.weight"], Wc["fc.3.weight"]
    else:
        c.fw1, c.fw2 = cast(dtype, P["fc.0.weight"]), cast(dtype, P["fc.3.weight"])
    if keep is not None and not isinstance(keep, torch.Tensor) and (dtype != N.BF16 or not train):
        keep = keep.materialise()
    c.keep = keep if train else None
    scale = 1.0 / (1.0 - p_drop) if c.keep is not None else 1.0
    if c.keep is not None and not isinstance(c.keep, torch.Tensor):
        vk = c.keep
        c.H1 = torch.empty(M, d, dtype=torch.bfloat16, device=c.P3.device)
        N.call("gemm_dropout", 0, 0, M, d, kin, 1.0, c.P3, kin, c.fw1, kin, c.H1, d, P["fc.0.bias"], 1, vk.seed, float(vk.p), vk.counter,
               float(scale))
    else:
        c.H1 = linear_fwd(dtype, c.P3, c.fw1, M, d, kin, bias=P["fc.0.bias"], relu=1, keep=c.keep, keep_scale=scale)
    c.H2 = linear_fwd(dtype, c.H1, c.fw2, M, d, d, bias=P["fc.3.bias"], relu=1)
    return x1, x2, x3, c.H2.view(Nimg, T3, d), c


def _conv_block_bwd(dtype, Y, dP, dxl, st, Nimg, Ti, Fi, Pin, Wd, G_w, G_gamma, G_beta, need_dx, col, keep, dx_bf16=False, Pout=None):
    td = N.torch_dtype(dtype)
    scale, shift, mean, rstd = st
    M = Nimg * Ti * Fi
    dY = torch.empty((M, 64), dtype=td, device=Y.device)
    stat = ARENA.scratch((33 * 128,), torch.float32, Y)
    yd = N.F32 if Y.dtype == torch.float32 else dtype
    if SYNC_BN is None and Pout is not None and _BN_STATS_P and Pout.dtype == td:
        N.call("bn_relu_pool_bwd_p", dtype, yd, GD, Y, Pout, dP, dxl, scale, shift, mean, rstd, stat, dY, G_gamma, G_beta, Nimg, Ti, Fi)
    elif SYNC_BN is None:
        N.call("bn_relu_pool_bwd", dtype, yd, GD, Y, dP, dxl, scale, shift, mean, rstd, stat, dY, G_gamma, G_beta, Nimg, Ti, Fi)
    else:
        N.call("bn_relu_pool_bwd_stats", dtype, yd, GD, Y, dP, dxl, scale, shift, mean, rstd, stat, Nimg, Ti, Fi)
        gstat = SYNC_BN.all_reduce(stat[:128].clone())
        N.call("bn_relu_pool_bwd_apply", dtype, yd, GD, Y, dP, dxl, scale, shift, mean, rstd, stat, gstat, float(M * SYNC_BN.world), dY,
               G_gamma, G_beta, Nimg, Ti, Fi)
    fused = dtype == N.BF16 and Fi in (16, 32)
    if fused:
        def wg():
            dWp = ARENA.zeros((64, 576), torch.float32, device=Y.device)
            ws = _wgrad_workspace(Y.device)
            N.call("conv3x3_wgrad", dY, Pin, dWp, ws, ws.numel(), Nimg, Ti, Fi)
            N.call("unpack_conv_dw", dWp, G_w)
            return dWp
        keep.append((dY, WGRAD.run(Y.device, wg)))
    else:
        dWp = ARENA.zeros((64, 576), torch.float32, device=Y.device)
        N.call("im2col3x3", dtype, Pin, col, Nimg, Ti, Fi)
        gemm(dtype, 1, 1, 64, 576, M, dY, 64, col, 576, dWp, 576, out_f32=1, atomic=1, ksplit=_ksplit(64, 576, M, 1024))
        N.call("unpack_conv_dw", dWp, G_w)
    if not need_dx:
        return None
    dx_bf16 = dx_bf16 and fused
    dPin = _empty((Nimg, Ti, Fi, 64), torch.bfloat16 if dx_bf16 else torch.float32, like=Y)
    if fused:
        N.call("conv3x3_fwd", dY, Wd, None, dPin, 0 if dx_bf16 else 1, None, None, 1, Nimg, Ti, Fi)
    else:
        N.call("im2col3x3", dtype, dY, col, Nimg, Ti, Fi)
        gemm(dtype, 0, 0, M, 64, 576, col, 576, Wd, 576, dPin, 64)
    return dPin


def encoder_backward(c, G, dA2=None, dH2=None, dx1=None, dx2=None, dx3=None, dx_late=None, grads_zero=False):
    dtype, Nimg, M, d, kin = c.dtype, c.N, c.M, c.d, c.kin
    T1, F1, T2, F2, T3, F3 = c.dims
    td = N.torch_dtype(dtype)
    assert c.train, "backward needs a train-mode forward (batch statistics)"
    if dA2 is None:
        dA2 = _empty((M, d), td, like=c.H2)
        N.call("relu_bwd", dtype, dH2.contiguous(), c.H2, dA2, M * d)
    dev = c.H2.device
    def w2():
        linear_bwd_w(dtype, dA2, c.H1, G["fc.3.weight"], M, d, d, dw_zero=grads_zero)
        colsum_add(dtype, dA2, M, d, G["fc.3.bias"])
    WGRAD.run(dev, w2)
    scale = 1.0 / (1.0 - c.p_drop) if c.keep is not None else 1.0
    dA1 = linear_bwd_x(dtype, dA2, c.fw2, M, d, d, alpha=scale, gate=c.H1)
    def w1():
        linear_bwd_w(dtype, dA1, c.P3, G["fc.0.weight"], M, d, kin, dw_zero=grads_zero)
        colsum_add(dtype, dA1, M, d, G["fc.0.bias"])
    WGRAD.run(dev, w1)
    dP3 = linear_bwd_x(dtype, dA1, c.fw1, M, d, kin, out_f32=1)
    if dx_late is not None:
        dx1, dx2, dx3 = dx_late()
    col = _col_buffer(dtype, Nimg, T1, F1, c.H2)
    keep = []
    dP2 = _conv_block_bwd(dtype, c.Y3, dP3, dx3, c.st3, Nimg, T2, F2, c.P2, c.W3d, G["features_3.0.weight"],
                          G["features_3.1.weight"], G["features_3.1.bias"], True, col, keep, Pout=c.P3)
    dP1 = _conv_block_bwd(dtype, c.Y2, dP2, dx2, c.st2, Nimg, T1, F1, c.P1, c.W2d, G["features_2.0.weight"],
                          G["features_2.1.weight"], G["features_2.1.bias"], True, col, keep, dx_bf16=bool(c.stem_mfma) and _DP1_BF16,
                          Pout=c.P2)
    gd1 = N.BF16 if dP1.dtype == torch.bfloat16 else GD
    acc = ARENA.scratch((32 * 64 * 11,), torch.float32, c.H2)
    P = c.P
    w1, b1, g1 = P["features_1.0.weight"].reshape(64, 9), P["features_1.0.bias"], P["features_1.1.weight"]
    gw, gb = G["features_1.0.weight"].view(64, 9), G["features_1.0.bias"]
    if SYNC_BN is None:
        N.call("conv1_bwd", gd1, int(c.stem_mfma), c.img, Nimg, c.F, c.T, w1, b1, g1, c.sc1, c.sh1, c.mean1, c.rstd1, c.mom1, dP1, dx1,
               acc, gw, gb, G["features_1.1.weight"], G["features_1.1.bias"])
    else:
        lstat = _empty((128,), torch.float32, like=c.H2)
        N.call("conv1_bwd_sums", gd1, int(c.stem_mfma), c.img, Nimg, c.F, c.T, w1, b1, g1, c.sc1, c.sh1, c.mean1, c.rstd1, c.mom1, dP1,
               dx1, acc, lstat)
        gstat = SYNC_BN.all_reduce(lstat.clone())
        N.call("conv1_bwd_finalize", acc, c.mom1, w1, b1, g1, c.mean1, c.rstd1, float(Nimg * c.F * c.T * SYNC_BN.world), gstat, gw, gb,
               G["features_1.1.weight"], G["features_1.1.bias"])
    WGRAD.join(dev)


def maxmean_forward(dtype, H2, out=None):
    Nimg, T3, d = H2.shape
    y = out if out is not None else _empty((Nimg, d), N.torch_dtype(dtype), like=H2)
    arg = _empty((Nimg, d), torch.uint8, like=H2)
    N.call("maxmean_fwd", dtype, int(y.dtype == torch.float32), H2, y, arg, Nimg, T3, d)
    return y, arg


def maxmean_backward(dtype, dy, arg, H2):
    Nimg, T3, d = H2.shape
    dA2 = _empty((Nimg * T3, d), N.torch_dtype(dtype), like=H2)
    N.call("maxmean_bwd", dtype, GD, dy, arg, H2, dA2, Nimg, T3, d)
    return dA2


class ProjCtx:
    pass


def projector_forward(PP, Y, dtype, groups, B, update_running=True, Wc=None, final_bn=True):
    kin = Y.shape[1]
    c = ProjCtx()
    c.dtype, c.B, c.groups, c.kin, c.y = dtype, B, groups, kin, Y
    W = Wc if Wc is not None else tuple(cast(dtype, PP[f"projector.{i}.weight"]) for i in (0, 3, 6))
    c.W = W
    D = W[0].shape[0]
    c.D = D
    M = groups * B

    def bn(a, prefix, affine, relu, out, adt=None):
        g = PP[prefix + ".weight"] if affine else None
        b = PP[prefix + ".bias"] if affine else None
        return bn_train_apply(dtype, ad if adt is None else adt, a, B, D, g, b, PP[prefix + ".running_mean"], PP[prefix + ".running_var"],
                              update_running, groups, relu, out)
    td = N.torch_dtype(dtype)
    ad = _ad(dtype)
    c.ad = ad
    o32 = int(ad == N.F32)
    c.cmean = None
    if dtype == N.BF16 and Y.dtype == torch.float32 and not HP and B <= 1024 and kin % 32 == 0 and SYNC_BN is None:
        c.y_hi, c.cmean = center_cast(Y, groups, B)
        c.y_lo = None
        c.a1 = linear_fwd(dtype, c.y_hi, W[0], M, D, kin, out_f32=o32)
    elif dtype == N.BF16 and Y.dtype == torch.float32:
        c.y_hi, c.y_lo = _empty((M, kin), td, like=Y), _empty((M, kin), td, like=Y)
        N.call("split_bf16", Y, c.y_hi, c.y_lo, M * kin)
        c.a1 = torch.zeros(M, D, dtype=torch.float32, device=Y.device)
        gemm(dtype, 0, 0, M, D, kin, c.y_hi, kin, W[0], kin, c.a1, D, out_f32=1, atomic=1)
        gemm(dtype, 0, 0, M, D, kin, c.y_lo, kin, W[0], kin, c.a1, D, out_f32=1, atomic=1)
    else:
        c.y_hi, c.y_lo = Y, None
        c.a1 = linear_fwd(dtype, Y, W[0], M, D, kin, out_f32=o32)
    c.ad1 = N.F32 if c.a1.dtype == torch.float32 else ad
    c.h1 = _empty((M, D), td, like=Y)
    c.st1 = bn(c.a1, "projector.1", True, 1, c.h1, adt=c.ad1)
    if c.cmean is not None and update_running:
        N.call("shift_running_mean", W[0], c.cmean, PP["projector.1.running_mean"], D, kin, groups, BN_MOMENTUM)
    c.a2 = linear_fwd(dtype, c.h1, W[1], M, D, D, out_f32=o32)
    c.h2 = _empty((M, D), td, like=Y)
    c.st2 = bn(c.a2, "projector.4", True, 1, c.h2)
    c.final_bn = final_bn
    if not final_bn:
        c.z = linear_fwd(dtype, c.h2, W[2], M, D, D, out_f32=1)
        return c.z, c
    c.z = linear_fwd(dtype, c.h2, W[2], M, D, D, out_f32=o32)
    c.zn = _empty((M, D), td, like=Y)
    c.st0 = bn(c.z, "bn", False, 0, c.zn)
    return c.zn, c


def projector_backward(c, PP, G, dzn, dy_rows=None):
    dtype, B, D, kin, groups = c.dtype, c.B, c.D, c.kin, c.groups
    M = groups * B
    td = N.torch_dtype(dtype)

    def bn_bwd(a, dh, st, relu, da, g_gamma, g_beta, adt=None):
        adt = c.ad if adt is None else adt
        """BatchNorm1d(train) backward per group (view).  SyncBatchNorm (`extras/delores-s/main.py:79` converts every BatchNorm of
        the model, the projector's included): the two means of the backward are over the GLOBAL batch of the view - this rank's
        sums are all-reduced between the statistics pass and the apply pass; the parameter gradients stay this rank's own sums
        (the data-parallel gradient all-reduce adds the ranks up afterwards)."""
        t = ARENA.scratch((2 * groups * D,), torch.float64, dzn)
        if SYNC_BN is None:
            N.call("colbn_bwd", dtype, adt, GD, a, dh, *st, relu, groups, B, D, t, da, g_gamma, g_beta)
            return
        N.call("colbn_bwd_stats", dtype, adt, GD, a, dh, *st, relu, groups, B, D, t)
        tg = SYNC_BN.all_reduce(t.clone())
        N.call("colbn_bwd_apply", dtype, adt, GD, a, dh, *st, relu, groups, B, D, tg, float(B * SYNC_BN.world), da)
        if g_gamma is not None:
            for g in range(groups):
                N.call("add_d2f", t[g * D:(g + 1) * D], g_beta, D)
                N.call("add_d2f", t[(groups + g) * D:(groups + g + 1) * D], g_gamma, D)
    if c.final_bn:
        dz = _empty((M, D), td, like=c.zn)
        bn_bwd(c.z, dzn, c.st0, 0, dz, None, None)
    else:
        dz = dzn
    linear_bwd_w(dtype, dz, c.h2, G["projector.6.weight"], M, D, D)
    dh2 = linear_bwd_x(dtype, dz, c.W[2], M, D, D, out_f32=1)
    da2 = _empty((M, D), td, like=dz)
    bn_bwd(c.a2, dh2, c.st2, 1, da2, G["projector.4.weight"], G["projector.4.bias"])
    linear_bwd_w(dtype, da2, c.h1, G["projector.3.weight"], M, D, D)
    dh1 = linear_bwd_x(dtype, da2, c.W[1], M, D, D, out_f32=1)
    da1 = _empty((M, D), td, like=dz)
    bn_bwd(c.a1, dh1, c.st1, 1, da1, G["projector.1.weight"], G["projector.1.bias"], adt=c.ad1)
    linear_bwd_w(dtype, da1, c.y_hi, G["projector.0.weight"], M, D, kin)
    if c.y_lo is not None:
        linear_bwd_w(dtype, da1, c.y_lo, G["projector.0.weight"], M, D, kin)
    rows = M if dy_rows is None else dy_rows
    if rows == 0:
        return None
    return linear_bwd_x(dtype, da1, c.W[0], rows, D, kin, out_f32=1)


def barlow_forward_backward(PP, G, Y, dtype, lambd, scale_loss, loss_out, need_dy1=True, need_dy2=True,
                            update_running=True, all_reduce=None, global_batch=None, backward=True, Wc=None):
    B = Y.shape[0] // 2
    zn, c = projector_forward(PP, Y, dtype, 2, B, update_running, Wc)
    D = c.D
    zn1, zn2 = zn[:B], zn[B:]
    denom = float(global_batch if global_batch else B)
    cmat = _empty((D, D), torch.float32, like=Y)
    gemm(dtype, 1, 1, D, D, B, zn1, D, zn2, D, cmat, D, alpha=1.0 / denom, out_f32=1)
    if all_reduce is not None:
        all_reduce(cmat)
    coef = (lambd if lambd else 1.0) * scale_loss
    dc = _empty((D, D), N.torch_dtype(dtype), like=Y)
    N.call("barlow_loss", dtype, cmat, D, coef, 2.0 * coef / denom, dc, loss_out)
    if not backward:
        return None
    dzn = _empty((2 * B, D), torch.float32, like=Y)
    gemm(dtype, 0, 0, B, D, D, zn2, D, dc, D, dzn[:B], D, out_f32=1)
    gemm(dtype, 0, 1, B, D, D, zn1, D, dc, D, dzn[B:], D, out_f32=1)
    rows = 2 * B if need_dy2 else (B if need_dy1 else 0)
    return projector_backward(c, PP, G, dzn, rows)


def _harr(ctype, xs):
    import ctypes
    vals = [x.data_ptr() if isinstance(x, torch.Tensor) else x for x in xs]
    return (ctype * len(vals))(*vals)


def _multi_check(*lists):
    for ts in lists:
        for t in ts:
            if t is not None and (not t.is_cuda or not t.is_contiguous()):
                raise RuntimeError("multi-problem launches need contiguous device tensors")


def gemm_multi(ta, tb, M, Nn, Ks, As, ldas, Bs, ldbs, Cs, ldc, alpha=1.0, out_f32=0, atomic=0, ksplit=1):
    import ctypes
    n = len(As)
    _multi_check(As, Bs, Cs)
    Ns = [Nn] * n if isinstance(Nn, int) else list(Nn)
    ldcs = [ldc] * n if isinstance(ldc, int) else list(ldc)
    adr = ctypes.addressof
    arrs = (_harr(ctypes.c_int, Ns), _harr(ctypes.c_int, Ks), _harr(ctypes.c_void_p, As), _harr(ctypes.c_long, ldas),
            _harr(ctypes.c_void_p, Bs), _harr(ctypes.c_long, ldbs), _harr(ctypes.c_void_p, Cs), _harr(ctypes.c_long, ldcs))
    N_, K_, A_, la_, B_, lb_, C_, lc_ = arrs
    if N.PROFILE is not None:
        N.PROFILE_NOTE = float(sum(2.0 * M * nn * kk for nn, kk in zip(Ns, Ks)))
    N.call("gemm_multi", n, ta, tb, M, adr(N_), adr(K_), float(alpha), adr(A_), adr(la_), adr(B_), adr(lb_), adr(C_), adr(lc_),
           out_f32, atomic, ksplit)


def gemm_multi_sgd(ta, tb, M, Nn, Ks, As, ldas, Bs, ldbs, Ps, Moms, Shadows, ldp, hyper, alpha=1.0):
    import ctypes
    n = len(As)
    _multi_check(As, Bs, Ps, Moms, [] if Shadows is None else Shadows)
    Ns = [Nn] * n if isinstance(Nn, int) else list(Nn)
    ldps = [ldp] * n if isinstance(ldp, int) else list(ldp)
    adr = ctypes.addressof
    vp = ctypes.c_void_p
    arrs = (_harr(ctypes.c_int, Ns), _harr(ctypes.c_int, Ks), _harr(vp, As), _harr(ctypes.c_long, ldas), _harr(vp, Bs),
            _harr(ctypes.c_long, ldbs), _harr(vp, Ps), _harr(vp, Moms), _harr(vp, Shadows if Shadows is not None else [None] * n),
            _harr(ctypes.c_long, ldps))
    if N.PROFILE is not None:
        N.PROFILE_NOTE = (float(sum(2.0 * M * nn * kk for nn, kk in zip(Ns, Ks))),
                          float(sum(2.0 * kk * (M + nn) + M * nn * (16.0 + (2.0 if Shadows is not None else 0.0)) for nn, kk in zip(Ns, Ks))))
    lr, mu, wd, gs, gs_dev = hyper
    N.call("gemm_multi_sgd", n, ta, tb, M, adr(arrs[0]), adr(arrs[1]), float(alpha), adr(arrs[2]), adr(arrs[3]), adr(arrs[4]), adr(arrs[5]),
           adr(arrs[6]), adr(arrs[7]), adr(arrs[8]), adr(arrs[9]), float(lr), float(mu), float(wd), float(gs), gs_dev)


def _heads_wgrad_split(D, kmax, M, nh):
    return _ksplit(D, kmax, M, max(256 // nh, 1))


def heads_wgrads_store(D, kins, M, grads_zero=True):
    nh = len(kins)
    return bool(grads_zero) and all(_heads_wgrad_split(D, k, M, nh) == 1 for k in (D, max(kins)))


def barlow_heads_forward_backward(PPs, Gs, Ys, dtype, lambds, scale_losses, loss_outs, update_running=True, backward=True,
                                  Wcs=None, grads_zero=False, dy_ready=None, sgd=None):
    import ctypes
    nh = len(Ys)
    B = Ys[0].shape[0] // 2
    M = 2 * B
    td = N.torch_dtype(dtype)
    dev = Ys[0].device
    W = Wcs if Wcs is not None else [tuple(cast(dtype, PP[f"projector.{i}.weight"]) for i in (0, 3, 6)) for PP in PPs]
    D = W[0][0].shape[0]
    kins = [Y.shape[1] for Y in Ys]
    ad = _ad(dtype)
    if dtype != N.BF16 or ad != N.BF16 or B > 1024 or D % 32:
        raise RuntimeError("grouped Barlow heads: bf16 path with B <= 1024 only")
    H = range(nh)
    vp, fl, adr = ctypes.c_void_p, ctypes.c_float, ctypes.addressof
    new = lambda rows, cols, t: [torch.empty(rows, cols, dtype=t, device=dev) for _ in H]

    def layer(xs, ws, ks, prefix, affine, relu):
        a = new(M, D, td)
        gemm_multi(0, 0, M, D, ks, xs, ks, ws, ks, a, D)
        out, st = new(M, D, td), new(4, 2 * D, torch.float32)
        par = lambda suffix, on=True: _harr(vp, [PP[prefix + suffix] if on else None for PP in PPs])
        arrs = (_harr(vp, a), par(".weight", affine), par(".bias", affine), par(".running_mean", update_running),
                par(".running_var", update_running), _harr(vp, out), _harr(vp, st))
        _multi_check(a, out, st)
        N.call("colbn_train_fwd_multi", nh, ad, adr(arrs[0]), adr(arrs[1]), adr(arrs[2]), adr(arrs[3]), adr(arrs[4]),
               BN_MOMENTUM, BN_EPS, relu, 2, B, D, adr(arrs[5]), adr(arrs[6]))
        return a, st, out
    ycs = [torch.empty(M, k, dtype=torch.bfloat16, device=dev) for k in kins]
    cms = [torch.empty(2, k, dtype=torch.float32, device=dev) for k in kins]
    _multi_check(list(Ys), ycs, cms)
    if any(Y.dtype != torch.float32 or k % 32 for Y, k in zip(Ys, kins)):
        raise RuntimeError("grouped Barlow heads: fp32 inputs with width % 32 == 0")
    arrs = (_harr(vp, list(Ys)), _harr(vp, ycs), _harr(vp, cms), _harr(ctypes.c_int, kins))
    N.call("center_cast_multi", nh, adr(arrs[0]), adr(arrs[1]), adr(arrs[2]), adr(arrs[3]), 2, B)
    a1, st1, h1 = layer(ycs, [W[h][0] for h in H], kins, "projector.1", True, 1)

    def shift_running():
        rms = [PP["projector.1.running_mean"] for PP in PPs]
        w0 = [W[h][0] for h in H]
        _multi_check(w0, rms)
        arrs = (_harr(vp, w0), _harr(vp, cms), _harr(vp, rms), _harr(ctypes.c_int, kins))
        N.call("shift_running_mean_multi", nh, adr(arrs[0]), adr(arrs[1]), adr(arrs[2]), D, adr(arrs[3]), 2, BN_MOMENTUM)
    shift_late = update_running and backward and dy_ready is not None
    if update_running and not shift_late:
        shift_running()
    a2, st2, h2 = layer(h1, [W[h][1] for h in H], [D] * nh, "projector.4", True, 1)
    z, st0, zn = layer(h2, [W[h][2] for h in H], [D] * nh, "bn", False, 0)
    dc = new(D, D, td)
    coefs = [(lambds[h] if lambds[h] else 1.0) * scale_losses[h] for h in H]
    dsc = [2.0 * c / B for c in coefs]
    if all(l.numel() == LOSS_REPLICAS for l in loss_outs) and D % 64 == 0:
        _multi_check([zn[h] for h in H], dc, list(loss_outs))
        arrs = (_harr(ctypes.c_int, [B] * nh), _harr(vp, [zn[h][:B] for h in H]), _harr(ctypes.c_long, [D] * nh),
                _harr(vp, [zn[h][B:] for h in H]), _harr(ctypes.c_long, [D] * nh), _harr(vp, dc), _harr(fl, coefs), _harr(fl, dsc),
                _harr(vp, list(loss_outs)))
        if N.PROFILE is not None:
            N.PROFILE_NOTE = float(nh * 2.0 * D * D * B)
        N.call("gemm_multi_barlow", nh, D, adr(arrs[0]), 1.0 / B, adr(arrs[1]), adr(arrs[2]), adr(arrs[3]), adr(arrs[4]), adr(arrs[5]),
               adr(arrs[6]), adr(arrs[7]), adr(arrs[8]))
    else:
        cm = new(D, D, torch.float32)
        gemm_multi(1, 1, D, D, [B] * nh, [zn[h][:B] for h in H], [D] * nh, [zn[h][B:] for h in H], [D] * nh, cm, D,
                   alpha=1.0 / B, out_f32=1)
        arrs = (_harr(vp, cm), _harr(fl, coefs), _harr(fl, dsc), _harr(vp, dc), _harr(vp, list(loss_outs)))
        _multi_check(list(loss_outs))
        N.call("barlow_loss_multi", nh, adr(arrs[0]), D, adr(arrs[1]), adr(arrs[2]), adr(arrs[3]), adr(arrs[4]))
    if not backward:
        return [None] * nh
    dzn = new(M, D, torch.float32)
    gemm_multi(0, 0, B, D, [D] * nh, [zn[h][B:] for h in H], [D] * nh, dc, [D] * nh, [dzn[h][:B] for h in H], D, out_f32=1)
    gemm_multi(0, 1, B, D, [D] * nh, [zn[h][:B] for h in H], [D] * nh, dc, [D] * nh, [dzn[h][B:] for h in H], D, out_f32=1)

    def bn_bwd(a, dh, st, relu, names):
        out = new(M, D, td)
        grads = lambda k: _harr(vp, [Gs[h][names[k]] if names else None for h in H])
        arrs = (_harr(vp, a), _harr(vp, dh), _harr(vp, st), _harr(vp, out), grads(0), grads(1))
        _multi_check(a, dh, st)
        N.call("colbn_bwd_multi", nh, ad, GD, adr(arrs[0]), adr(arrs[1]), adr(arrs[2]), relu, 2, B, D, adr(arrs[3]),
               adr(arrs[4]), adr(arrs[5]))
        return out

    def wgrad(dys, xs, name, ks):
        split = _heads_wgrad_split(D, max(ks), M, nh)
        if sgd is not None:
            if split != 1 or Wcs is None:
                raise RuntimeError("fused SGD needs unsplit weight gradients and the flat weight shadows")
            li = {"projector.0.weight": 0, "projector.3.weight": 1, "projector.6.weight": 2}[name]
            gemm_multi_sgd(1, 1, D, ks, [M] * nh, dys, [D] * nh, xs, ks, [PPs[h][name] for h in H], [sgd["momentum"][h][name] for h in H],
                           [W[h][li] for h in H], ks, sgd["hyper"])
            return
        gemm_multi(1, 1, D, ks, [M] * nh, dys, [D] * nh, xs, ks, [Gs[h][name] for h in H], ks, out_f32=1,
                   atomic=1 if split > 1 else (0 if grads_zero else 2), ksplit=split)

    def dgrad(dys, ws, Ks, rows):
        out = [torch.empty(rows, k, dtype=torch.float32, device=dev) for k in Ks]
        gemm_multi(0, 1, rows, Ks, [D] * nh, [dy[:rows] for dy in dys], [D] * nh, ws, Ks, out, Ks, out_f32=1)
        return out
    later = []
    defer = (lambda fn: later.append(fn)) if dy_ready is not None else (lambda fn: fn())
    dz = bn_bwd(z, dzn, st0, 0, None)
    defer(lambda: wgrad(dz, h2, "projector.6.weight", [D] * nh))
    dh2 = dgrad(dz, [W[h][2] for h in H], [D] * nh, M)
    da2 = bn_bwd(a2, dh2, st2, 1, ("projector.4.weight", "projector.4.bias"))
    defer(lambda: wgrad(da2, h1, "projector.3.weight", [D] * nh))
    dh1 = dgrad(da2, [W[h][1] for h in H], [D] * nh, M)
    da1 = bn_bwd(a1, dh1, st1, 1, ("projector.1.weight", "projector.1.bias"))
    defer(lambda: wgrad(da1, ycs, "projector.0.weight", kins))
    dy = dgrad(da1, [W[h][0] for h in H], kins, B)
    if dy_ready is not None:
        dy_ready()
    if shift_late:
        shift_running()
    for fn in later:
        fn()
    return dy


def moco_forward_backward(dtype, q, k, queue, queue_shadow, temperature, loss_out, backward=True):
    B, dim = q.shape
    K = queue.shape[1]
    td = N.torch_dtype(dtype)
    qn, kn = _empty((B, dim), td, like=q), _empty((B, dim), td, like=q)
    qn32, kn32 = _empty((B, dim), torch.float32, like=q), _empty((B, dim), torch.float32, like=q)
    qinv, kinv = _empty((B,), torch.float32, like=q), _empty((B,), torch.float32, like=q)
    lpos = _empty((B,), torch.float32, like=q)
    N.call("moco_prep", dtype, q, k, B, dim, 1.0 / temperature, qn, qn32, qinv, kn, kn32, kinv, lpos)
    lse = _empty((B,), torch.float32, like=q)
    dlpos = _empty((B,), torch.float32, like=q)
    Pm = None
    if dtype == N.BF16 and K % 8 == 0 and dim % 8 == 0:
        nslot = (K + 63) // 64
        part = _empty((B, nslot, 2), torch.float32, like=q)
        N.call("moco_logits", 1, qn, queue_shadow, B, K, dim, 1.0 / temperature, part, None, 0.0, None)
        N.call("moco_lse_merge", lpos, part, B, nslot, 1.0 / (B * temperature), lse, loss_out, dlpos)
        if not backward:
            return None, kn32
        Pm = _empty((B, K), td, like=q)
        N.call("moco_logits", 2, qn, queue_shadow, B, K, dim, 1.0 / temperature, None, lse, 1.0 / (B * temperature), Pm)
    else:
        lneg = _empty((B, K), torch.float32, like=q)
        gemm(dtype, 0, 1, B, K, dim, qn, dim, queue_shadow, K, lneg, K, alpha=1.0 / temperature, out_f32=1)
        N.call("moco_ce_fwd", lpos, lneg, B, K, lse, loss_out)
        if not backward:
            return None, kn32
        Pm = _empty((B, K), td, like=q)
        N.call("moco_ce_bwd", dtype, lpos, lneg, lse, B, K, 1.0 / (B * temperature), Pm, dlpos)
    dqn = ARENA.zeros((B, dim), torch.float32, device=q.device)
    gemm(dtype, 0, 0, B, dim, K, Pm, K, queue_shadow, K, dqn, dim, out_f32=1, atomic=1, ksplit=_ksplit(B, dim, K, 256))
    dq = _empty((B, dim), td, like=q)
    N.call("l2norm_bwd", dtype, dqn, dlpos, kn32, qn32, qinv, B, dim, dq)
    return dq, kn32
```

audio-ssl_amd/src/upstream/decar_v2/model.py:

```python
import torch
from torch import nn

from src import _native as N
from src import engine as E
from src.encoder.audiontt import DropoutMasks, _EncoderFn, default_precision
from src.functional import BatchNorm1dFn, LinearFn, MaxMeanFn

_TO_ENGINE = {"features.0.": "features_1.0.", "features.1.": "features_1.1.", "features.4.": "features_2.0.",
              "features.5.": "features_2.1.", "features.8.": "features_3.0.", "features.9.": "features_3.1.", "fc.": "fc."}


class MultiPrototypes(nn.Module):
    def __init__(self, output_dim, nmb_prototypes):
        super().__init__()
        self.nmb_heads = len(nmb_prototypes)
        for i, k in enumerate(nmb_prototypes):
            self.add_module("prototypes" + str(i), nn.Linear(output_dim, k, bias=False))

    def forward(self, x):
        return [LinearFn.apply(x, getattr(self, "prototypes" + str(i)).weight, None, False) for i in range(self.nmb_heads)]


class AudioNTT2020(nn.Module):

    def __init__(self, args, out_dim, n_mels=64, d=512, nmb_prototypes=3000):
        super().__init__()
        self.args = args
        layers = []
        for cin in (1, 64, 64):
            layers += [nn.Conv2d(cin, 64, 3, stride=1, padding=1), nn.BatchNorm2d(64), nn.ReLU(), nn.MaxPool2d(2, stride=2)]
        self.features = nn.Sequential(*layers)
        self.fc = nn.Sequential(nn.Linear(64 * (n_mels // (2 ** 3)), d), nn.ReLU(), nn.Dropout(p=0.3), nn.Linear(d, d), nn.ReLU())
        self.d = d
        self.projection_head = nn.Sequential(nn.Linear(d, 2048), nn.BatchNorm1d(2048), nn.ReLU(inplace=True),
                                             nn.Linear(2048, out_dim))
        if isinstance(args.nmb_prototypes, list):
            self.prototypes = MultiPrototypes(out_dim, list(getattr(args, "prototype_sizes", None) or [1024]))
        elif args.nmb_prototypes > 0:
            self.prototypes = nn.Linear(out_dim, 1024, bias=False)
        self.precision = default_precision()
        self.dropout_masks = DropoutMasks(0.3)

    def _encoder_items(self):
        out = []
        for n, t in list(self.named_parameters()) + list(self.named_buffers()):
            for a, b in _TO_ENGINE.items():
                if n.startswith(a):
                    out.append((b + n[len(a):], n, t))
        return out

    def param_dict(self):
        p0 = self.features[0].weight
        c = self.__dict__.get("_enc_cache")
        if c is None or c[0] != p0.data_ptr():
            c = self.__dict__["_enc_cache"] = (p0.data_ptr(), {k: (t.data if isinstance(t, nn.Parameter) else t)
                                                                for k, _, t in self._encoder_items()})
        return c[1]

    def engine_param_names(self):
        return [k for k, _, t in self._encoder_items() if isinstance(t, nn.Parameter)]

    def encoder_parameters(self):
        return tuple(t for _, _, t in self._encoder_items() if isinstance(t, nn.Parameter))

    def encode(self, x):
        if not x.is_cuda:
            raise RuntimeError("AudioNTT2020 (HIP) needs a GPU tensor - there is no CPU fallback")
        x = x.float().contiguous()
        keep = self.dropout_masks.next(x.shape[0] * (x.shape[-1] // 8), self.d, x.device) if self.training else None
        params = self.encoder_parameters()
        if torch.is_grad_enabled() and any(p.requires_grad for p in params):
            return _EncoderFn.apply(self, x, keep, *params)[3]
        return E.encoder_forward(self.param_dict(), x, self.precision, keep=keep, p_drop=self.fc[2].p, train=self.training)[3]

    def project(self, z):
        ph = self.projection_head
        act = z.dtype
        a = LinearFn.apply(z, ph[0].weight, ph[0].bias, False)
        h = BatchNorm1dFn.apply(a, ph[1].weight, ph[1].bias, ph[1].running_mean, ph[1].running_var, self.precision, True,
                                self.training)
        return LinearFn.apply(h.to(act), ph[3].weight, ph[3].bias, False)

    def forward(self, batch):
        z = MaxMeanFn.apply(self.encode(batch[0]))
        z_new = MaxMeanFn.apply(self.encode(batch[1]))
        x = self.project(z)
        x_new = self.project(z_new)
        protos = self.prototypes(x_new.to(z.dtype)) if isinstance(self.prototypes, MultiPrototypes) else \
            LinearFn.apply(x_new.to(z.dtype), self.prototypes.weight, None, False)
        return x, protos
```

audio-ssl_amd/src/upstream/delores_m/upstream_expert.py:

```python
import os

import torch
import torch.nn as nn

from src import _native as N
from src import engine as E
from src.encoder.audiontt import default_precision
from src.flat import FlatGroup
from src.module_base import UpstreamModule
from src.upstream.common import EAGER, FusedExpertMixin, FusedStepFn, MocoQueueMixin, Projection, strip
from src.upstream.delores_m.upstream_encoder import DELORES_M as DELORES_M_ENCODER
from src.utils import concat_all_gather


_PREP_ASIDE = os.environ.get("AUDIOSSL_PREP_ASIDE", "1") != "0"
_HEADS_ASIDE = os.environ.get("AUDIOSSL_HEADS_ASIDE", "1") != "0"
_FUSED_SGD = os.environ.get("AUDIOSSL_FUSED_SGD", "1") != "0"
_SKIP_ZERO = os.environ.get("AUDIOSSL_SKIP_ZERO", "1") != "0"
_GRADS_ZERO = os.environ.get("AUDIOSSL_GRADS_ZERO", "1") != "0"
_DY_EVENT = os.environ.get("AUDIOSSL_DY_EVENT", "1") != "0"
_LATE_JOIN = os.environ.get("AUDIOSSL_LATE_JOIN", "1") != "0"
_SGD_ASIDE = os.environ.get("AUDIOSSL_SGD_ASIDE", "1") != "0"
_STEM_PAIR = os.environ.get("AUDIOSSL_STEM_PAIR", "0") == "1"


def _world():
    import torch.distributed as dist
    return dist.get_world_size() if dist.is_available() and dist.is_initialized() else 1


class Upstream_Expert(MocoQueueMixin, FusedExpertMixin, UpstreamModule):
    prefer_phases = False

    def __init__(self, config, base_encoder, datamodule=None, emb_dim: int = 128, num_negatives: int = 65536,
                 encoder_momentum: float = 0.999, softmax_temperature: float = 0.07, learning_rate: float = 0.03,
                 momentum: float = 0.9, weight_decay: float = 1e-4, data_dir: str = './', batch_size: int = 256,
                 use_mlp: bool = False, num_workers: int = 8, *args, **kwargs):
        super().__init__()
        self.save_hyperparameters()
        if use_mlp:
            raise NotImplementedError("use_mlp is not part of the HIP path")
        self.config = config
        self.base_encoder = base_encoder
        self.datamodule = datamodule
        self.encoder_q, self.encoder_k = self.init_encoders(self.base_encoder)
        for param_q, param_k in zip(self.encoder_q.parameters(), self.encoder_k.parameters()):
            param_k.data.copy_(param_q.data)
            param_k.requires_grad = False
        self.register_buffer("queue", nn.functional.normalize(torch.randn(emb_dim, num_negatives), dim=0))
        self.register_buffer("queue_ptr", torch.zeros(1, dtype=torch.long))
        lam, scale = self.config["pretrain"]["lambda_barlow"], self.config["pretrain"]["loss_scale"]
        self.p1 = Projection(2048, lam[0], scale)
        self.p2 = Projection(1024, lam[1], scale)
        self.p3 = Projection(512, lam[2], scale)
        prec = config.get("run", {}).get("precision")
        self.precision = {"fp32": N.F32, "bf16": N.BF16, "bf16_hp": N.BF16}.get(prec, default_precision())
        self.high_precision = prec == "bf16_hp"
        self.grouped_heads = bool(config.get("run", {}).get("grouped_heads", os.environ.get("AUDIOSSL_GROUPED_HEADS", "1") != "0"))
        self.encoder_q.encoder.precision = self.encoder_k.encoder.precision = self.precision
        self.flat_k = None
        self._key_stream = E.SideStream()
        self._prep_stream = E.SideStream()

    def init_encoders(self, base_encoder):
        return DELORES_M_ENCODER(self.config, base_encoder), DELORES_M_ENCODER(self.config, base_encoder)

    def trainable_named(self):
        named = [(n, p) for n, p in self.named_parameters() if n.startswith("encoder_q.")]
        named += [(n, p) for n, p in self.named_parameters() if n.startswith(("p1.", "p2.", "p3."))]
        return named

    def fused_loss(self, img_q, img_k, need_grad=True, parts=None, runner=None, optimizer=None):
        with E.ARENA.step(img_q.device):
            return self._fused_loss(img_q, img_k, need_grad, parts, runner, optimizer)

    def _fused_loss(self, img_q, img_k, need_grad, parts, runner, optimizer):
        R = runner or EAGER
        dt = self.precision
        E.set_high_precision(self.high_precision)
        flat = self.ensure_flat()
        dev = img_q.device
        B = img_q.shape[0]
        eq, ek = self.encoder_q, self.encoder_k
        ddp = _world() > 1
        img_k = img_k.float().contiguous()
        img_q = img_q.float().contiguous()
        pending_k = self._shuffle_begin(img_k) if ddp else None
        main = torch.cuda.current_stream()
        G = flat.grad_dict
        Ys = R.alloc("Ys", lambda: [torch.empty(2 * B, f, dtype=E.pooled_dtype(dt), device=dev) for f in (2048, 1024, 512)])

        moms = None
        if _STEM_PAIR and not ddp and E.stem_fused(dt, self.training):
            moms = R.phase("stem_moments", lambda: E.stem_moments_pair(img_q, img_k))
            if not E.ONE_STREAM:
                moms.record_stream(self._key_stream.stream(dev))

        def key_phase(x):
            self._momentum_update_key_encoder(shadow_dtype=dt)
            self.flat_k.refresh_shadow(dt)
            Wk = self.flat_k.shadow_dict()
            keepk = ek.encoder.next_keep_mask(B, x.shape[-1])
            _, _, _, Hk, _ = E.encoder_forward(ek.encoder.param_dict(), x, dt, keep=keepk, p_drop=0.3, train=self.training,
                                               Wc=strip(Wk, "encoder."), layer_out=tuple(y[B:] for y in Ys),
                                               stem_moments=None if moms is None else moms[1])
            yk, _ = E.maxmean_forward(dt, Hk)
            wk = Wk["fc.weight"]
            return E.linear_fwd(dt, yk, wk, B, wk.shape[0], wk.shape[1], bias=ek.fc.bias.data, out_f32=1)

        def key_branch():
            x, idx_unshuffle = img_k, None
            if ddp:
                x, idx_unshuffle = self._shuffle_end(pending_k, B)
                x = R.static("key_in", x)
            kk = R.phase("key", lambda: key_phase(x))
            if ddp:
                kk = R.static("key_out", self._batch_unshuffle_ddp(kk, idx_unshuffle))
            return kk
        k = self._key_stream.run(dev, key_branch)

        heads = (self.p1, self.p2, self.p3)
        grouped = not (self.high_precision or dt == N.F32 or not self.grouped_heads or E.SYNC_BN is not None)
        D_ = self.p1.param_dict()["projector.3.weight"].shape[0]
        kins_ = [p.param_dict()["projector.0.weight"].shape[1] for p in heads]
        stored_grads = tuple(f"p{i + 1}.projector.{j}.weight" for i in range(3) for j in (0, 3, 6)) \
            if (need_grad and grouped and _GRADS_ZERO and _SKIP_ZERO and E.heads_wgrads_store(D_, kins_, 2 * B)) else ()

        sgd_ctx = None
        if stored_grads and _FUSED_SGD and optimizer is not None and not ddp and hasattr(optimizer, "fused_wgrad"):
            sgd_ctx = optimizer.fused_wgrad(flat, [f"p{i + 1}." for i in range(3)])

        def query_phase():
            def prep():
                if need_grad:
                    flat.zero_grad(stores_ok=bool(stored_grads))
                flat.refresh_shadow(dt)
            busy = (need_grad and not (flat._fresh_grad is True or (flat._fresh_grad == "partial" and stored_grads))) or \
                   not (flat._fresh_shadow or dt == N.F32)
            if _PREP_ASIDE and busy:
                self._prep_stream.run(dev, prep)
            else:
                prep()
            Wq = flat.shadow_dict("encoder_q.")
            wq = Wq["fc.weight"]
            fold = not (self.high_precision or dt == N.F32 or not self.grouped_heads)
            loss = torch.zeros(4 + (3 * E.LOSS_REPLICAS if fold else 0), dtype=torch.float32, device=dev)
            keep = eq.encoder.next_keep_mask(B, img_q.shape[-1])
            _, _, _, Hq, cq = E.encoder_forward(eq.encoder.param_dict(), img_q, dt, keep=keep, p_drop=0.3, train=self.training,
                                                Wc=strip(Wq, "encoder."), layer_out=tuple(y[:B] for y in Ys),
                                                before_fc=(lambda: self._prep_stream.join(dev)) if (_PREP_ASIDE and busy) else None,
                                                stem_moments=None if moms is None else moms[0])
            yq, argq = E.maxmean_forward(dt, Hq)
            q = E.linear_fwd(dt, yq, wq, B, wq.shape[0], wq.shape[1], bias=eq.fc.bias.data, out_f32=1)
            return loss, wq, Hq, cq, yq, argq, q
        loss, wq, Hq, cq, yq, argq, q = R.phase("query", query_phase)
        self._key_stream.join(dev)
        k.record_stream(main)

        streams = self._streams(dev)
        dys = [None, None, None]
        dy_event = None

        def head_phase(i, p):
            Wp = flat.shadow_dict(f"p{i + 1}.")
            return E.barlow_forward_backward(p.param_dict(), G(f"p{i + 1}."), Ys[i], dt, p.lambd, p.scale_loss,
                                             loss[i + 1:i + 2], need_dy1=True, need_dy2=False,
                                             update_running=self.training, backward=need_grad,
                                             Wc=tuple(Wp[f"projector.{j}.weight"] for j in (0, 3, 6)))
        if not grouped:
            for i, p in enumerate(heads):
                if not E.ONE_STREAM:
                    E.fork(streams[i], main)
                with torch.cuda.stream(streams[i]):
                    dys[i] = R.phase(f"head{i + 1}", lambda i=i, p=p: head_phase(i, p))
        else:
            def heads_phase():
                Wps = [flat.shadow_dict(f"p{i + 1}.") for i in range(3)]
                return E.barlow_heads_forward_backward(
                    [p.param_dict() for p in heads], [G(f"p{i + 1}.") for i in range(3)], Ys, dt, [p.lambd for p in heads],
                    [p.scale_loss for p in heads],
                    [loss[4 + i * E.LOSS_REPLICAS:4 + (i + 1) * E.LOSS_REPLICAS] for i in range(3)], update_running=self.training,
                    backward=need_grad, Wcs=[tuple(Wp[f"projector.{j}.weight"] for j in (0, 3, 6)) for Wp in Wps],
                    grads_zero=need_grad and _GRADS_ZERO,
                    dy_ready=(lambda: dy_event.record()) if dy_event is not None else None, sgd=sgd_ctx)
            hs = streams[0] if _HEADS_ASIDE else main
            if not E.ONE_STREAM and _HEADS_ASIDE:
                E.fork(streams[0], main)
            if need_grad and not ddp and not E.ONE_STREAM and _HEADS_ASIDE and _SGD_ASIDE and _DY_EVENT:
                dy_event = torch.cuda.Event()
            with torch.cuda.stream(hs):
                dys = list(R.phase("heads", heads_phase))

        def moco_phase():
            shadow = self.queue_shadow(dt)
            dq, kn32 = E.moco_forward_backward(dt, q, k, self.queue, shadow, float(self.hparams.softmax_temperature),
                                               loss[0:1], backward=need_grad)
            dA2 = None
            if need_grad:
                Gq = G("encoder_q.")
                E.linear_bwd_w(dt, dq, yq, Gq["fc.weight"], B, wq.shape[0], wq.shape[1])
                E.colsum_add(dt, dq, B, wq.shape[0], Gq["fc.bias"])
                dyq = E.linear_bwd_x(dt, dq, wq, B, wq.shape[0], wq.shape[1], out_f32=1)
                dA2 = E.maxmean_backward(dt, dyq, argq, Hq)
            return kn32, dA2
        kn32, dA2 = R.phase("moco", moco_phase)
        self._dequeue_and_enqueue(kn32, self.queue_shadow(dt) if dt != N.F32 else None)
        early_box = [None]

        def join_heads():
            for i, st in enumerate(streams):
                if E.ONE_STREAM:
                    continue
                if i == 0 and dy_event is not None:
                    main.wait_event(dy_event)
                else:
                    main.wait_stream(st)
            for d in dys:
                if d is not None:
                    d.record_stream(main)
            if not need_grad:
                return dys
            self.reduce_begin("heads")
            if optimizer is not None and not ddp and hasattr(optimizer, "step_tail"):
                early = streams[0] if _SGD_ASIDE else main
                if not E.ONE_STREAM and _SGD_ASIDE and dy_event is None:
                    E.fork(early, main)
                with torch.cuda.stream(early):
                    if R.phase("sgd_heads", lambda: optimizer.step_tail(flat, self.head_offset(), stored=stored_grads,
                                                                        stepped=sgd_ctx is not None)):
                        optimizer.mark_early(flat, self.head_offset())
                        early_box[0] = early
                    elif sgd_ctx is not None:
                        raise RuntimeError("the projector weights were stepped by their weight-gradient GEMMs but the head-segment "
                                           "SGD pass declined: the optimiser's step() would step them again")
            return dys

        late = need_grad and not ddp and _LATE_JOIN
        if not late:
            join_heads()
        if need_grad:
            def backward_phase():
                if late:
                    box = [None]

                    def join_and_sum():
                        d = join_heads()
                        box[0] = loss.sum()
                        return d
                    E.encoder_backward(cq, G("encoder_q.encoder."), dA2=dA2, dx_late=join_and_sum, grads_zero=_GRADS_ZERO)
                    return box[0]
                E.encoder_backward(cq, G("encoder_q.encoder."), dA2=dA2, dx1=dys[0], dx2=dys[1], dx3=dys[2],
                                   grads_zero=_GRADS_ZERO)
                return loss.sum()
            total = R.phase("encoder_bwd", backward_phase)
            if early_box[0] is not None and not E.ONE_STREAM and _SGD_ASIDE:
                main.wait_stream(early_box[0])
            elif dy_event is not None:
                main.wait_stream(streams[0])
            self.reduce_begin("enc")
        else:
            total = loss.sum()
        if parts is not None:
            parts["losses"] = loss if loss.numel() == 4 else torch.cat([loss[:1], loss[4:].view(3, E.LOSS_REPLICAS).sum(1)])
        return total

    def _streams(self, dev):
        if E.ONE_STREAM:
            return [torch.cuda.current_stream(dev)] * 3
        if getattr(self, "_side_streams", None) is None or self._side_streams[0].device != dev:
            self._side_streams = [torch.cuda.Stream(device=dev) for _ in range(3)]
        return self._side_streams

    def forward(self, img_q=None, img_k=None):
        raise NotImplementedError("the HIP expert fuses forward and loss; call training_step((img_1, img_2), i)")

    def training_step(self, batch, batch_idx):
        img_1, img_2 = batch
        params = self.ensure_flat().params
        loss = FusedStepFn.apply(self, torch.is_grad_enabled(), img_1, img_2, *params)
        self.log_dict({'train_loss': loss})
        return loss
```

include/audiossl_hip.h:

```cpp
#ifndef AUDIOSSL_HIP_H
#define AUDIOSSL_HIP_H

#include <stdint.h>

#ifdef __cplusplus
extern "C" {
#endif

#define AUDIOSSL_OK 0
#define AUDIOSSL_EINVAL (-1)
#define AUDIOSSL_ELAUNCH (-2)
#define AUDIOSSL_EALIGN (-3)

int audiossl_logmel_fwd(const float* wave, float* out, int B, int L, int T, int n_fft, int hop, int n_mels, int taps,
                        const float* win, const float* tw, const float* melw, const int* mel_start, float eps_pow,
                        float eps_log, int apply_log, void* stream);

int audiossl_fbank_fwd(const float* wave, const int* lens, const int* partner, const float* lam, float* clip_mean,
                       const int* bands, const int* bands_host, float* out, int B, int Lmax, int win_len, int shift, int n_fft, int n_mels,
                       int taps, int T_target, const float* win, const float* tw, const float* melw, const int* mel_start,
                       float preemph, float eps_log, float mean, float std, int skip_norm, int time_major, void* stream);

int audiossl_clip_moments(const float* x, double* mom, int B, int n, void* stream);
int audiossl_runnorm_scan(const double* mom, int B, int n_elem, long long* state_i, float* state_f, float* mu_out,
                          float* sd_out, void* stream);
int audiossl_aug_normalize(const float* x, const float* mu, const float* sd, float* bank, long slot0, int R, int B, int n,
                           void* stream);
int audiossl_aug_views(const float* bank, int R, const int* ip, const float* fp, float* out1, float* out2, int B, int F,
                       int T, int canvas_h, int canvas_w, int log_mix, void* stream);
int audiossl_aug_plan_host(uint32_t* np_key, int* np_pos, uint32_t* py_key, int* py_pos, int B, int F, int T,
                           long long clips_seen, long long* n_entries, int R, int n_memory, int use_mix, double ratio,
                           int use_rrc, double fs_lo, double fs_hi, double ts_lo, double ts_hi, int canvas_h,
                           int canvas_w, int use_spec, int spec_F, int spec_T, int spec_nf, int spec_nt, const int* lens,
                           int unit, int* starts, int* ip, float* fp, int* masks);

int audiossl_resample_sinc(const float* x, float* y, int clips, int n_orig, int n_out, const int* n, const int* off_l,
                           const int* off_r, const double* eta_l, const double* eta_r, const double* win, const double* delta,
                           int nwin, int index_step, void* stream);

int audiossl_pcm_window(const void* pcm, long pcm_bytes, const long long* tab, const long long* tab_host, float* out, int B,
                        int unit, int align, void* stream);

int audiossl_kmix_cluster(const float* views, const float* centroids, int n_views, int F, int T, int K, int* cluster,
                          void* stream);
int audiossl_kmix_apply(const float* views, const float* ring, const int* slot, const float* coef, int n_views, int n,
                        int log_mix, float* out, void* stream);
int audiossl_mask_fill(float* x, const int* tab, int n_img, int max_masks, int F, int T, int zero_fill, void* stream);

int audiossl_conv1_stats(const float* img, int N, int F, int T, const float* w, const float* bias, const float* gamma,
                         const float* beta, float* running_mean, float* running_var, float momentum, float eps,
                         double* mom, float* scale, float* shift, float* save_mean, float* save_rstd, void* stream);
#define AUDIOSSL_CONV1_XL_PARTS 4
int audiossl_conv1_fwd(int dtype, const float* img, int N, int F, int T, const float* w, const float* bias,
                       const float* scale, const float* shift, void* out, float* xl, void* stream);
#define AUDIOSSL_CONV1_MOM_SLOT (17 * 54)
int audiossl_conv1_moments_pair(const float* img_a, const float* img_b, int N, int F, int T, double* mom, void* stream);
int audiossl_conv1_fwd_train(const float* img, int N, int F, int T, double* mom, double count, const float* w, const float* bias,
                             const float* gamma, const float* beta, float* running_mean, float* running_var, float momentum,
                             float eps, float* scale, float* shift, float* save_mean, float* save_rstd, void* out, float* xl,
                             void* stream);
int audiossl_conv1_bwd(int dtype, int conv_dtype, const float* img, int N, int F, int T, const float* w, const float* bias,
                       const float* gamma, const float* scale, const float* shift, const float* mean, const float* rstd,
                       const double* mom, const void* dP, const void* dxl, float* acc, float* dW, float* dbias,
                       float* dgamma, float* dbeta, void* stream);

int audiossl_colstats(int dtype, const void* x, int groups, long M, int C, long ld, int want_sq, double* sum,
                      double* sumsq, void* stream);
int audiossl_bn_finalize(const double* sum, const double* sumsq, int groups, double count, int C, const float* gamma,
                         const float* beta, float* running_mean, float* running_var, float momentum, float eps,
                         float* scale, float* shift, float* save_mean, float* save_rstd, void* stream);
int audiossl_bn_relu_pool_fwd(int dtype, int ydtype, const void* Y, const float* scale, const float* shift, void* P, int N,
                              int Ti, int Fi, void* stream);
int audiossl_bn_relu_pool_train_fwd(int dtype, int ydtype, const void* Y, const double* sum, const double* sumsq, int stat_replicas,
                                    double count, const float* gamma, const float* beta, float* running_mean, float* running_var,
                                    float momentum, float eps, void* P, float* scale, float* shift, float* save_mean, float* save_rstd,
                                    int N, int Ti, int Fi, void* stream);
int audiossl_tmean_fwd(int dtype, int out_f32, const void* P, void* xl, int N, int To, int Fo, void* stream);
int audiossl_tmean3_fwd(int dtype, int out_f32, const void* P1, void* x1, const float* x1_parts, int To1, int Fo1, const void* P2,
                        void* x2, int To2, int Fo2, const void* P3, void* x3, int To3, int Fo3, int N, void* stream);
int audiossl_bn_relu_pool_bwd(int dtype, int ydtype, int gdtype, const void* Y, const void* dP, const void* dxl, const float* scale,
                              const float* shift, const float* mean, const float* rstd, float* stat, void* dY,
                              float* dgamma, float* dbeta, int N, int Ti, int Fi, void* stream);
int audiossl_bn_relu_pool_bwd_p(int dtype, int ydtype, int gdtype, const void* Y, const void* P, const void* dP, const void* dxl,
                                const float* scale, const float* shift, const float* mean, const float* rstd, float* stat, void* dY,
                                float* dgamma, float* dbeta, int N, int Ti, int Fi, void* stream);
int audiossl_conv1_moments(const float* img, int N, int F, int T, double* mom, void* stream);
int audiossl_conv1_finalize(double* mom_totals, const float* w, const float* bias, const float* gamma, const float* beta,
                            float* running_mean, float* running_var, float momentum, float eps, double count, float* scale,
                            float* shift, float* save_mean, float* save_rstd, void* stream);
int audiossl_conv1_bwd_sums(int dtype, int conv_dtype, const float* img, int N, int F, int T, const float* w, const float* bias,
                            const float* gamma, const float* scale, const float* shift, const float* mean, const float* rstd,
                            const double* mom, const void* dP, const void* dxl, float* acc, float* lstat, void* stream);
int audiossl_conv1_bwd_finalize(const float* acc, const double* mom, const float* w, const float* bias, const float* gamma,
                                const float* mean, const float* rstd, double count_global, const float* gstat, float* dW,
                                float* dbias, float* dgamma, float* dbeta, void* stream);
int audiossl_bn_relu_pool_bwd_stats(int dtype, int ydtype, int gdtype, const void* Y, const void* dP, const void* dxl,
                                    const float* scale, const float* shift, const float* mean, const float* rstd, float* stat,
                                    int N, int Ti, int Fi, void* stream);
int audiossl_bn_relu_pool_bwd_apply(int dtype, int ydtype, int gdtype, const void* Y, const void* dP, const void* dxl,
                                    const float* scale, const float* shift, const float* mean, const float* rstd, float* stat,
                                    const float* gstat, double count_global, void* dY, float* dgamma, float* dbeta, int N, int Ti,
                                    int Fi, void* stream);
int audiossl_colbn_bwd_stats(int dtype, int adtype, int gdtype, const void* a, const void* dh, const float* scale,
                             const float* shift, const float* mean, const float* rstd, int relu, int groups, long M, int C,
                             double* tmp, void* stream);
int audiossl_colbn_bwd_apply(int dtype, int adtype, int gdtype, const void* a, const void* dh, const float* scale,
                             const float* shift, const float* mean, const float* rstd, int relu, int groups, long M, int C,
                             const double* sums, double count, void* da, void* stream);
int audiossl_im2col3x3(int dtype, const void* X, void* col, int N, int Ti, int Fi, void* stream);
int audiossl_pack_conv_w(int dtype, const float* W, void* Wf, void* Wd, void* stream);
int audiossl_pack_conv_w2(int dtype, const float* Wa, void* Wfa, void* Wda, const float* Wb, void* Wfb, void* Wdb, void* stream);
int audiossl_unpack_conv_dw(const float* dWp, float* dW, void* stream);

int audiossl_conv3x3_fwd(const void* X, const void* W, const float* bias, void* Y, int out_f32, double* sum,
                         double* sumsq, int stat_replicas, int N, int Ti, int Fi, void* stream);
int audiossl_conv3x3_wgrad(const void* dY, const void* X, float* dWp, float* workspace, long workspace_floats, int N, int Ti,
                           int Fi, void* stream);

int audiossl_gemm(int dtype, int trans_a, int trans_b, int M, int N, int K, float alpha, const void* A, long lda,
                  const void* B, long ldb, void* C, long ldc, const float* bias, int relu, const uint8_t* keep, long ldk,
                  float keep_scale, const void* gate, long ldg, int out_f32, int atomic, int ksplit, const float* resid,
                  long ldr, void* stream);

int audiossl_gemm_dropout(int trans_a, int trans_b, int M, int N, int K, float alpha, const void* A, long lda, const void* B,
                          long ldb, void* C, long ldc, const float* bias, int relu, unsigned long long seed, float p,
                          const long long* counter, float keep_scale, void* stream);

int audiossl_gemm_multi(int count, int trans_a, int trans_b, int M, const int* N, const int* K, float alpha,
                        const void* const* A, const long* lda, const void* const* B, const long* ldb, void* const* C,
                        const long* ldc, int out_f32, int atomic, int ksplit, void* stream);
int audiossl_gemm_multi_sgd(int count, int trans_a, int trans_b, int M, const int* Nv, const int* K, float alpha,
                            const void* const* A, const long* lda, const void* const* B, const long* ldb, float* const* P,
                            float* const* Mom, void* const* Shadow, const long* ldp, float lr, float momentum, float weight_decay,
                            float grad_scale, const float* grad_scale_dev, void* stream);
int audiossl_gemm_multi_barlow(int count, int D, const int* K, float alpha, const void* const* A, const long* lda,
                               const void* const* B, const long* ldb, void* const* dc, const float* coef, const float* dscale,
                               float* const* loss_rep, void* stream);

int audiossl_maxmean_fwd(int dtype, int out_f32, const void* H, void* y, uint8_t* arg, int N, int Tt, int D, void* stream);
int audiossl_maxmean_bwd(int dtype, int gdtype, const void* dy, const uint8_t* arg, const void* H, void* dA, int N, int Tt,
                         int D, void* stream);

int audiossl_colbn_fwd(int dtype, int adtype, const void* a, const float* scale, const float* shift, int relu, void* h,
                       int groups, long M, int C, void* stream);
int audiossl_colbn_train_fwd(int dtype, int adtype, const void* a, const float* gamma, const float* beta,
                             float* running_mean, float* running_var, float momentum, float eps, int relu, int groups,
                             long M, int C, void* h, float* scale, float* shift, float* save_mean, float* save_rstd,
                             void* stream);
int audiossl_colbn_bwd(int dtype, int adtype, int gdtype, const void* a, const void* dh, const float* scale, const float* shift, const float* mean,
                       const float* rstd, int relu, int groups, long M, int C, double* tmp, void* da, float* dgamma,
                       float* dbeta, void* stream);
int audiossl_colbn_train_fwd_multi(int count, int adtype, const void* const* a, const float* const* gamma,
                                   const float* const* beta, float* const* running_mean, float* const* running_var,
                                   float momentum, float eps, int relu, int groups, long M, int C, void* const* h,
                                   float* const* stats, void* stream);
int audiossl_colbn_bwd_multi(int count, int adtype, int gdtype, const void* const* a, const void* const* dh,
                             const float* const* stats, int relu, int groups, long M, int C, void* const* da,
                             float* const* dgamma, float* const* dbeta, void* stream);
int audiossl_barlow_loss_multi(int count, const float* const* c, int D, const float* coef, const float* dscale,
                               void* const* dc, float* const* loss_out, void* stream);
int audiossl_add_d2f(const double* src, float* dst, int n, void* stream);
int audiossl_barlow_loss(int dtype, const float* c, int D, float coef, float dscale, void* dc, float* loss_out,
                         void* stream);

int audiossl_l2norm_fwd(int dtype, const float* q, int B, int D, void* qn, float* qn32, float* inv_norm, void* stream);
int audiossl_moco_prep(int dtype, const float* q, const float* k, int B, int D, float scale, void* qn, float* qn32, float* qinv,
                       void* kn, float* kn32, float* kinv, float* lpos, void* stream);
int audiossl_rowdot(const float* a, const float* b, int B, int D, float scale, float* out, void* stream);
int audiossl_moco_ce_fwd(const float* lpos, const float* lneg, int B, int K, float* lse, float* loss_out, void* stream);
int audiossl_moco_ce_bwd(int dtype, const float* lpos, const float* lneg, const float* lse, int B, int K, float gscale,
                         void* P, float* dlpos, void* stream);
int audiossl_moco_logits(int mode, const void* qn, const void* queue, int B, int K, int dim, float inv_t, float* part,
                         const float* lse, float gscale, void* P, void* stream);
int audiossl_moco_lse_merge(const float* lpos, const float* part, int B, int nslot, float gscale, float* lse,
                            float* loss_out, float* dlpos, void* stream);
int audiossl_l2norm_bwd(int dtype, const float* dqn, const float* dlpos, const float* kn32, const float* qn32,
                        const float* inv_norm, int B, int D, void* dq, void* stream);
int audiossl_enqueue(int dtype, const float* keys, int B, int D, int K, int ptr, long long* ptr_dev, float* queue, void* shadow,
                     void* stream);
int audiossl_ema_update(float* pk, const float* pq, long n, float m, void* shadow, void* stream);

int audiossl_set_prezeroed(int on);
int audiossl_last_kernel(char* name, int capacity);

int audiossl_sgd_momentum(float* p, float* g, float* buf, long n, float lr, float momentum, float weight_decay,
                          int first, float grad_scale, const float* grad_scale_dev, void* shadow_bf16, int zero_grad,
                          void* stream);
int audiossl_sgd_momentum_segments(float* p, float* g, float* buf, const long* segs, int nseg, long max_n, float lr, float momentum,
                                   float weight_decay, int first, float grad_scale, const float* grad_scale_dev, void* shadow_bf16,
                                   int zero_grad, void* stream);
int audiossl_zero_segments(float* g, const long* segs, int nseg, long max_n, void* stream);
int audiossl_cast(int dtype, const float* src, void* dst, long n, void* stream);
int audiossl_cast_back(int dtype, const void* src, float* dst, long n, void* stream);
int audiossl_dropout_mask(uint8_t* keep, long n, unsigned long long seed, float p, const long long* counter, void* stream);
int audiossl_relu_bwd(int dtype, const void* g, const void* h, void* out, long n, void* stream);
int audiossl_bn_eval_affine(const float* gamma, const float* beta, const float* running_mean, const float* running_var,
                            float eps, int C, float* scale, float* shift, void* stream);
int audiossl_axpy(float* y, const float* x, float a, long n, void* stream);
int audiossl_split_bf16(const float* x, void* hi, void* lo, long n, void* stream);
int audiossl_center_cast(const float* y, void* yc, float* cmean, int groups, long M, int C, void* stream);
int audiossl_shift_running_mean(const void* W, const float* cmean, float* running_mean, int D, int K, int groups,
                                float momentum, void* stream);
int audiossl_center_cast_multi(int count, const float* const* y, void* const* yc, float* const* cmean, const int* C, int groups,
                               long M, void* stream);
int audiossl_shift_running_mean_multi(int count, const void* const* W, const float* const* cmean, float* const* running_mean,
                                      int D, const int* K, int groups, float momentum, void* stream);

int audiossl_ntxent_fwd(const float* sim, int N, int B, float* lse, float* loss_out, void* stream);
int audiossl_ntxent_bwd(int dtype, const float* sim, const float* lse, int N, int B, float gscale, void* dsim, void* stream);

int audiossl_row_argmax(const float* dot, long N, int K, long long* assign, void* stream);
int audiossl_kmeans_accumulate(const float* x, const long long* assign, long N, int K, int D, float* sums, int* counts,
                               void* stream);
int audiossl_kmeans_update(const float* sums, const int* counts, int K, int D, float* centroids, void* stream);
int audiossl_kmeans_update_mean(const float* sums, const int* counts, int K, int D, float* centroids, void* stream);
int audiossl_row_sqnorm(const float* x, int rows, int D, float scale, float* out, void* stream);
int audiossl_ce_rows(int dtype, const float* logits, const long long* target, int B, int K, int ignore_index, int* cnt,
                     float* loss_out, void* dlogits, void* stream);

int audiossl_unfused_loss(int gdtype, const float* z1, const float* z2, const float* z3, const float* t,
                          const long long* label, int B, int C, long ld, float alpha, float beta, float gamma,
                          float* loss4, void* dz1, void* dz2, void* dz3, void* dt, void* stream);

int audiossl_knn_workspace(int Nq, long Nb, int k, long* bytes);
int audiossl_knn_topk(const void* q, const void* bank, int Nq, long Nb, int D, int k, float* top_sim, int* top_idx,
                      void* workspace, long workspace_bytes, void* stream);
int audiossl_knn_vote(const float* top_sim, const int* top_idx, const long long* bank_label, int Nq, int k, long Nb,
                      float inv_t, long long* pred, float* conf, void* stream);

int audiossl_softmax_rows_fwd(const float* x, float* y, int M, int C, void* stream);
int audiossl_softmax_rows_bwd(const float* y, const float* gy, float* gx, int M, int C, void* stream);

int audiossl_attn_fwd(const void* qkv, void* out, float* lse, int B, int S, int H, float scale, void* stream);
int audiossl_attn_bwd(const void* qkv, const void* out, const void* dout, const float* lse, void* dqkv, int B, int S, int H,
                      float scale, void* stream);
int audiossl_layernorm_fwd(const float* x, const float* gamma, const float* beta, void* y, float* y32, float* mean, float* rstd,
                           int M, int C, float eps, void* stream);
int audiossl_layernorm_bwd(const float* dy, const float* x, const float* mean, const float* rstd, const float* gamma,
                           float* dres, float* dgamma, float* dbeta, int M, int C, void* stream);
int audiossl_gelu_fwd(const void* a, void* h, long n, void* stream);
int audiossl_gelu_bwd(const void* a, const void* dh, void* da, long n, void* stream);
int audiossl_patch_unfold(const float* x, void* out, int B, int F, int T, int fstride, int tstride, void* stream);
int audiossl_tile_rows(const float* src, float* out, long rows, int period, int group, float scale, int C, void* stream);
int audiossl_adamw(float* p, const float* g, float* m, float* v, long n, float lr, float beta1, float beta2, float eps,
                   float weight_decay, float grad_scale, const long long* step, void* stream);

int audiossl_mvit_pool_fwd(const void* qkv, int ldq, int col0, const float* w, const float* gamma, const float* beta, float* out,
                           float* z, float* mean, float* rstd, int B, int heads, int d, int H, int W, int Ho, int Wo, int sh, int sw,
                           float eps, void* stream);
int audiossl_mvit_pool_bwd(const void* qkv, int ldq, int col0, const float* w, const float* gamma, const float* dout, const float* z,
                           const float* mean, const float* rstd, float* dz, float* dw, float* dgamma, float* dbeta, void* dqkv, int B,
                           int heads, int d, int H, int W, int Ho, int Wo, int sh, int sw, void* stream);
int audiossl_mvit_attn_fwd(const float* q, const float* k, const float* v, const float* rh, const float* rw, const int* ih,
                           const int* iw, void* out, float* lse, int B, int heads, int d, int qh, int qw, int kh, int kw, int nrh,
                           int nrw, int residual, float scale, void* stream);
int audiossl_mvit_attn_bwd(const float* q, const float* k, const float* v, const float* rh, const float* rw, const int* ih,
                           const int* iw, const void* dout, const float* lse, float* dq, float* dk, float* dv, float* drh, float* drw,
                           int B, int heads, int d, int qh, int qw, int kh, int kw, int nrh, int nrw, int residual, float scale,
                           void* stream);
int audiossl_tokpool_max_fwd(const float* x, float* y, void* arg, int B, int H, int W, int C, int kh, int kw, int sh, int sw,
                             void* stream);
int audiossl_tokpool_max_bwd(const float* dy, const void* arg, float* dx, int B, int H, int W, int C, int kh, int kw, int sh, int sw,
                             void* stream);

int audiossl_lars_step(float* p, const float* g, float* mu, const void* seg, int n_seg, const float* lr, float weight_decay,
                       float momentum, float eta, float grad_scale, double* norms, void* stream);
int audiossl_larc_step(float* p, const float* g, float* mu, const void* seg, int n_seg, float lr, float weight_decay,
                       float momentum, float trust_coefficient, float eps, int clip, float grad_scale, double* norms,
                       void* stream);

#ifdef __cplusplus
}
#endif
#endif
```

Measured before the change: 267,600 clips/s.

## Fuse 2x2 max-pool into conv3x3 epilogue and skip storing conv output for key encoder

The conv3x3 workspace kernel gains a POOL mode that computes a sign-adjusted 2x2 max of the raw bf16 conv outputs in its epilogue, using the sign of gamma so the max commutes with the per-channel BN affine. It writes a quarter-size pre-BN pooled tensor alongside the stats. A light kernel then applies BN+ReLU to the pooled tensor, replacing the full-size BN/ReLU/pool pass over Y. When no backward is needed (the MoCo key encoder), the full conv output Y is not stored at all, cutting write and read traffic. This adds epilogue complexity and relies on the max/affine commutation, which is exact only for bf16 values.

```diff
diff --git a/audio-ssl_amd/csrc/bnpool.hip b/audio-ssl_amd/csrc/bnpool.hip
--- a/audio-ssl_amd/csrc/bnpool.hip
+++ b/audio-ssl_amd/csrc/bnpool.hip
@@ -94,15 +94,11 @@
     o.store(P + idx * 8);
 }
 
-template <typename TY, typename T_>
-__global__ __launch_bounds__(256) void bn_relu_pool_train_fwd_kernel(const TY* __restrict__ Y, const double* __restrict__ sum,
-                                                                     const double* __restrict__ sumsq, int stat_rep, double count,
-                                                                     const float* __restrict__ gamma, const float* __restrict__ beta,
-                                                                     float* running_mean, float* running_var, float momentum, float eps,
-                                                                     T_* __restrict__ P, float* __restrict__ scale,
-                                                                     float* __restrict__ shift, float* __restrict__ save_mean,
-                                                                     float* __restrict__ save_rstd, int N, int Ti, int Fi) {
-    __shared__ float sc_s[64], sh_s[64];
+__device__ __forceinline__ void bn_train_prologue(const double* __restrict__ sum, const double* __restrict__ sumsq, int stat_rep,
+                                                  double count, const float* __restrict__ gamma, const float* __restrict__ beta,
+                                                  float* running_mean, float* running_var, float momentum, float eps,
+                                                  float* __restrict__ scale, float* __restrict__ shift, float* __restrict__ save_mean,
+                                                  float* __restrict__ save_rstd, float* sc_s, float* sh_s) {
     if (threadIdx.x < 64) {
         const int c = threadIdx.x;
         const double g = (double)gamma[c], b = (double)beta[c];
@@ -124,6 +120,19 @@
         }
     }
     __syncthreads();
+}
+
+template <typename TY, typename T_>
+__global__ __launch_bounds__(256) void bn_relu_pool_train_fwd_kernel(const TY* __restrict__ Y, const double* __restrict__ sum,
+                                                                     const double* __restrict__ sumsq, int stat_rep, double count,
+                                                                     const float* __restrict__ gamma, const float* __restrict__ beta,
+                                                                     float* running_mean, float* running_var, float momentum, float eps,
+                                                                     T_* __restrict__ P, float* __restrict__ scale,
+                                                                     float* __restrict__ shift, float* __restrict__ save_mean,
+                                                                     float* __restrict__ save_rstd, int N, int Ti, int Fi) {
+    __shared__ float sc_s[64], sh_s[64];
+    bn_train_prologue(sum, sumsq, stat_rep, count, gamma, beta, running_mean, running_var, momentum, eps, scale, shift, save_mean,
+                      save_rstd, sc_s, sh_s);
     const int To = Ti / 2, Fo = Fi / 2;
     const long total = (long)N * To * Fo * 8;
     const long idx = (long)blockIdx.x * 256 + threadIdx.x;
@@ -148,6 +157,41 @@
 #pragma unroll
     for (int i = 0; i < 8; ++i) o.set(i, m[i]);
     o.store(P + idx * 8);
+}
+
+template <typename T_>
+__device__ __forceinline__ void bn_relu_pooled_apply(const T_* Praw, const float* sc_s, const float* sh_s, T_* P, long vecs) {
+    const int c8 = threadIdx.x & 7;
+    float sc[8], sh[8];
+#pragma unroll
+    for (int i = 0; i < 8; ++i) { sc[i] = sc_s[c8 * 8 + i]; sh[i] = sh_s[c8 * 8 + i]; }
+    for (long idx = (long)blockIdx.x * 256 + threadIdx.x; idx < vecs; idx += (long)gridDim.x * 256) {
+        const Vec8<T_> v = Vec8<T_>::load(Praw + idx * 8);
+        Vec8<T_> o;
+#pragma unroll
+        for (int i = 0; i < 8; ++i) o.set(i, fmaxf(0.f, sc[i] * v.get(i) + sh[i]));
+        o.store(P + idx * 8);
+    }
+}
+
+template <typename T_>
+__global__ __launch_bounds__(256) void bn_relu_pooled_fwd_kernel(const T_* Praw, const float* __restrict__ scale,
+                                                                 const float* __restrict__ shift, T_* P, long vecs) {
+    bn_relu_pooled_apply<T_>(Praw, scale, shift, P, vecs);
+}
+
+template <typename T_>
+__global__ __launch_bounds__(256) void bn_relu_pooled_train_fwd_kernel(const T_* Praw, const double* __restrict__ sum,
+                                                                       const double* __restrict__ sumsq, int stat_rep, double count,
+                                                                       const float* __restrict__ gamma, const float* __restrict__ beta,
+                                                                       float* running_mean, float* running_var, float momentum,
+                                                                       float eps, T_* P, float* __restrict__ scale,
+                                                                       float* __restrict__ shift, float* __restrict__ save_mean,
+                                                                       float* __restrict__ save_rstd, long vecs) {
+    __shared__ float sc_s[64], sh_s[64];
+    bn_train_prologue(sum, sumsq, stat_rep, count, gamma, beta, running_mean, running_var, momentum, eps, scale, shift, save_mean,
+                      save_rstd, sc_s, sh_s);
+    bn_relu_pooled_apply<T_>(Praw, sc_s, sh_s, P, vecs);
 }
 
 template <typename T_, typename TO>
@@ -496,6 +540,35 @@
                            static_cast<const TY*>(Y), sum, sumsq, stat_replicas, count, gamma, beta, running_mean, running_var,
                            momentum, eps, static_cast<TO*>(P), scale, shift, save_mean, save_rstd, N, Ti, Fi);
     }, ydtype);
+    ASSL_LAUNCH_CHECK();
+}
+
+extern "C" int audiossl_bn_relu_pooled_fwd(int dtype, const void* Praw, const float* scale, const float* shift, void* P, int N,
+                                           int To, int Fo, void* stream) {
+    ASSL_REQUIRE(Praw && scale && shift && P && N > 0 && To > 0 && Fo > 0 && (dtype == 0 || dtype == 1));
+    const long vecs = (long)N * To * Fo * 8;
+    const int grid = (int)min((long)2048, (vecs + 255) / 256);
+    assl_dispatch(dtype, [&](auto t) { using T = typename decltype(t)::type;
+        hipLaunchKernelGGL((bn_relu_pooled_fwd_kernel<T>), dim3(grid), dim3(256), 0, S_(stream), static_cast<const T*>(Praw), scale, shift,
+                           static_cast<T*>(P), vecs);
+    });
+    ASSL_LAUNCH_CHECK();
+}
+
+extern "C" int audiossl_bn_relu_pooled_train_fwd(int dtype, const void* Praw, const double* sum, const double* sumsq, int stat_replicas,
+                                                 double count, const float* gamma, const float* beta, float* running_mean,
+                                                 float* running_var, float momentum, float eps, void* P, float* scale, float* shift,
+                                                 float* save_mean, float* save_rstd, int N, int To, int Fo, void* stream) {
+    ASSL_REQUIRE(Praw && sum && sumsq && gamma && beta && P && scale && shift && save_mean && save_rstd && count > 0.0);
+    ASSL_REQUIRE(stat_replicas >= 1 && (stat_replicas == 1 || sumsq == sum + 64));
+    ASSL_REQUIRE(N > 0 && To > 0 && Fo > 0 && (dtype == 0 || dtype == 1));
+    const long vecs = (long)N * To * Fo * 8;
+    const int grid = (int)min((long)2048, (vecs + 255) / 256);
+    assl_dispatch(dtype, [&](auto t) { using T = typename decltype(t)::type;
+        hipLaunchKernelGGL((bn_relu_pooled_train_fwd_kernel<T>), dim3(grid), dim3(256), 0, S_(stream), static_cast<const T*>(Praw), sum,
+                           sumsq, stat_replicas, count, gamma, beta, running_mean, running_var, momentum, eps, static_cast<T*>(P), scale,
+                           shift, save_mean, save_rstd, vecs);
+    });
     ASSL_LAUNCH_CHECK();
 }
 
diff --git a/audio-ssl_amd/csrc/conv.hip b/audio-ssl_amd/csrc/conv.hip
--- a/audio-ssl_amd/csrc/conv.hip
+++ b/audio-ssl_amd/csrc/conv.hip
@@ -13,6 +13,7 @@
 struct ConvArgs {
     const bf16* X; const bf16* W; const float* bias; bf16* Y; double* sum; double* sumsq;
     int Ti, rows_total, tiles, out_f32, dbg, stat_rep;
+    const float* gamma; bf16* Praw;
 };
 
 template <int FI, int PITCH, int NTH = 256>
@@ -179,6 +180,15 @@
     }
 }
 
+typedef unsigned int u32x4 __attribute__((ext_vector_type(4)));
+
+__device__ __forceinline__ float vmax4(float a, float b, float c, float d) {
+    float t, r;
+    asm("v_max3_f32 %0, %1, %2, %3" : "=v"(t) : "v"(a), "v"(b), "v"(c));
+    asm("v_max_f32 %0, %1, %2" : "=v"(r) : "v"(t), "v"(d));
+    return r;
+}
+
 template <int FI>
 struct WsGeom {
     static constexpr int TT = 256 / FI, COLS = FI + 2, ROWS = TT + 2, SEGS = FI / 8;
@@ -187,10 +197,13 @@
     static constexpr int BYTES = ROWS * COLS * 128;
 };
 
-template <int FI, bool STATS, bool F32OUT, int PF = 2>
+template <int FI, bool STATS, bool F32OUT, int PF = 2, bool POOL = false, bool KEEP_Y = true>
 __global__ __launch_bounds__(256, 1) void conv3x3_ws_kernel(ConvArgs a) {
+    static_assert(!POOL || (STATS && !F32OUT), "pooled emission: bf16 output with statistics");
+    static_assert(KEEP_Y || POOL, "a convolution that stores nothing");
     using G = WsGeom<FI>;
     constexpr int TT = G::TT, COLS = G::COLS;
+    const int dbg = POOL ? 0 : a.dbg;
     typedef __attribute__((address_space(3))) void* lptr_t;
     extern __shared__ __attribute__((aligned(16))) char smem[];
     float* const biasl = reinterpret_cast<float*>(smem + 2 * G::BYTES);
@@ -199,10 +212,11 @@
     char* const stg = reinterpret_cast<char*>(red + 4 * 64 * 2) + (threadIdx.x >> 6) * 64 * OPIX;
     char* const zblk = reinterpret_cast<char*>(red + 4 * 64 * 2) + 4 * 64 * OPIX;
     if (threadIdx.x < 32) *reinterpret_cast<f32x4*>(zblk + threadIdx.x * 16) = f32x4{0.f, 0.f, 0.f, 0.f};
+    unsigned* const gsign = reinterpret_cast<unsigned*>(zblk + 512);
 
     const int lane = threadIdx.x & 63, wave = __builtin_amdgcn_readfirstlane(threadIdx.x >> 6);
     const int m = lane & 31, h = lane >> 5;
-    long* const rts = (!STATS && (a.dbg & 16) && threadIdx.x == 0 && (blockIdx.x == 0 || blockIdx.x == gridDim.x - 1))
+    long* const rts = (!STATS && (dbg & 16) && threadIdx.x == 0 && (blockIdx.x == 0 || blockIdx.x == gridDim.x - 1))
                           ? reinterpret_cast<long*>(a.sum) + 64 + (blockIdx.x ? 8 : 0) : nullptr;
     if (rts) rts[0] = __builtin_amdgcn_s_memrealtime();
 
@@ -236,6 +250,11 @@
         *reinterpret_cast<f32x4*>(smem + b * G::BYTES + (r * COLS + side * (FI + 1)) * 128 + c8 * 16) = f32x4{0.f, 0.f, 0.f, 0.f};
     }
     if (threadIdx.x < 64) biasl[threadIdx.x] = a.bias ? a.bias[threadIdx.x] : 0.f;
+    if (POOL && threadIdx.x >= 64 && threadIdx.x < 128) {
+        const int t = threadIdx.x - 64, c = (t >> 2) & 7, j = (t >> 5) ? ((t & 3) ^ 2) : (t & 3);
+        const float ga = a.gamma[c * 8 + 2 * j], gb = a.gamma[c * 8 + 2 * j + 1];
+        gsign[t] = (ga < 0.f ? 0x8000u : 0u) | (gb < 0.f ? 0x80000000u : 0u);
+    }
 
     if (rts) { asm volatile("s_waitcnt vmcnt(0)" ::: "memory"); rts[3] = __builtin_amdgcn_s_memrealtime(); }
     const __amdgpu_buffer_rsrc_t rsrc = __builtin_amdgcn_make_buffer_rsrc(const_cast<bf16*>(a.X), 0, (unsigned)((long)a.rows_total * FI * 128), 0x00020000);
@@ -281,14 +300,14 @@
     asm volatile("s_waitcnt vmcnt(0) lgkmcnt(0)" ::: "memory");
     __builtin_amdgcn_s_barrier();
 
-    long* const ts = (!STATS && (a.dbg & 16) && blockIdx.x == 0 && threadIdx.x == 0) ? reinterpret_cast<long*>(a.sum) : nullptr;
+    long* const ts = (!STATS && (dbg & 16) && blockIdx.x == 0 && threadIdx.x == 0) ? reinterpret_cast<long*>(a.sum) : nullptr;
     int tsi = 0;
     if (rts) rts[1] = __builtin_amdgcn_s_memrealtime();
     for (; tile < a.tiles; tile += gridDim.x, cur ^= 1) {
         if (ts) ts[tsi++] = __builtin_amdgcn_s_memtime();
         const int g0 = tile * TT;
         const int next = tile + gridDim.x;
-        if (next < a.tiles && !(a.dbg & 2)) dma_tile(next * TT, smem + (cur ^ 1) * G::BYTES);
+        if (next < a.tiles && !(dbg & 2)) dma_tile(next * TT, smem + (cur ^ 1) * G::BYTES);
         const char* const hl = smem + cur * G::BYTES;
 
         int bdt[2][3];
@@ -320,7 +339,7 @@
             for (int i = 0; i < 2; ++i)
                 f[i] = Vec8<bf16>::load(reinterpret_cast<const bf16*>((const char*)(lptr_t)(size_t)(bdt[i][dt] + df * 128 + (hs[df] ^ (cc * 32)))));
         };
-        if (!(a.dbg & 4)) {
+        if (!(dbg & 4)) {
 #pragma unroll
         for (int ks = 0; ks < PF; ++ks) fetch(ks, fa[ks]);
 #pragma unroll
@@ -340,7 +359,7 @@
         if (ts) ts[tsi++] = __builtin_amdgcn_s_memtime();
         asm volatile("s_waitcnt vmcnt(0)" ::: "memory");
         if (ts) ts[tsi++] = __builtin_amdgcn_s_memtime();
-        if (!(a.dbg & 1)) {
+        if (!(dbg & 1)) {
 #pragma unroll
             for (int i = 0; i < 2; ++i) {
                 char* const st = stg + i * 32 * OPIX;
@@ -382,7 +401,7 @@
                         f32x4 v = *reinterpret_cast<const f32x4*>(st + p * 128 + ((c ^ (k >> 1)) << 4));
                         if (k & 1) v = f32x4{v[2], v[3], v[0], v[1]};
                         if ((p >> (FI == 32 ? 5 : 4)) < prow_ok) {
-                            *reinterpret_cast<f32x4*>(yrow + p * 128 + c * 16) = v;
+                            if (KEEP_Y) *reinterpret_cast<f32x4*>(yrow + p * 128 + c * 16) = v;
                             if (STATS) {
                                 const bf16x8 hv = __builtin_bit_cast(bf16x8, v);
 #pragma unroll
@@ -393,6 +412,40 @@
                             }
                         }
                     }
+                }
+            }
+            if (POOL) {
+                const u32x4 sm = *reinterpret_cast<const u32x4*>(gsign + ((pl & 1) * 8 + cp) * 4);
+#pragma unroll
+                for (int s = 0; s < 2; ++s) {
+                    const int po = FI == 32 ? s * 8 + pl : pl;
+                    const int grow = g0 + (FI == 32 ? 2 * wave : 2 * (2 * wave + s));
+                    const int pos = (cp ^ (po >> 1)) << 4;
+                    const char* const s0 = stg + (FI == 32 ? 0 : s * 32 * 128) + (2 * po) * 128;
+                    u32x4 q[4];
+                    q[0] = *reinterpret_cast<const u32x4*>(s0 + pos);
+                    q[1] = *reinterpret_cast<const u32x4*>(s0 + 128 + pos);
+                    if (FI == 32) {
+                        q[2] = *reinterpret_cast<const u32x4*>(s0 + 32 * 128 + pos);
+                        q[3] = *reinterpret_cast<const u32x4*>(s0 + 33 * 128 + pos);
+                    } else {
+                        q[2] = *reinterpret_cast<const u32x4*>(s0 + 16 * 128 + (pos ^ 64));
+                        q[3] = *reinterpret_cast<const u32x4*>(s0 + 17 * 128 + (pos ^ 64));
+                    }
+                    u32x4 r;
+#pragma unroll
+                    for (int j = 0; j < 4; ++j) {
+                        const unsigned d0 = q[0][j] ^ sm[j], d1 = q[1][j] ^ sm[j], d2 = q[2][j] ^ sm[j], d3 = q[3][j] ^ sm[j];
+                        const float hi = vmax4(__builtin_bit_cast(float, d0), __builtin_bit_cast(float, d1),
+                                               __builtin_bit_cast(float, d2), __builtin_bit_cast(float, d3));
+                        const float lo = vmax4(__builtin_bit_cast(float, d0 << 16), __builtin_bit_cast(float, d1 << 16),
+                                               __builtin_bit_cast(float, d2 << 16), __builtin_bit_cast(float, d3 << 16));
+                        r[j] = __builtin_amdgcn_perm(__builtin_bit_cast(unsigned, hi), __builtin_bit_cast(unsigned, lo), 0x07060302u) ^ sm[j];
+                    }
+                    const unsigned odd = 0u - (unsigned)(pl & 1);
+                    r = u32x4{(r[2] & odd) | (r[0] & ~odd), (r[3] & odd) | (r[1] & ~odd), (r[0] & odd) | (r[2] & ~odd), (r[1] & odd) | (r[3] & ~odd)};
+                    if (a.rows_total - grow >= 2)
+                        *reinterpret_cast<u32x4*>(reinterpret_cast<char*>(a.Praw) + ((grow >> 1) * (FI / 2) * 128 + po * 128 + cp * 16)) = r;
                 }
             }
         }
@@ -639,6 +692,36 @@
     if (Fi == 32) { if (nw == 8) CONV_LAUNCH(32, 8, 0); else CONV_LAUNCH(32, 4, 1); }
     else          { if (nw == 8) CONV_LAUNCH(16, 8, 2); else CONV_LAUNCH(16, 4, 3); }
 #undef CONV_LAUNCH
+    ASSL_LAUNCH_CHECK();
+}
+
+extern "C" int audiossl_conv3x3_pool_fwd(const void* X, const void* W, const float* bias, const float* gamma, void* Y, void* Praw,
+                                         double* sum, double* sumsq, int stat_replicas, int N, int Ti, int Fi, void* stream) {
+    ASSL_REQUIRE(X && W && gamma && Praw && sum && sumsq && N > 0 && Ti > 0 && (Ti % 2) == 0 && (Fi == 32 || Fi == 16));
+    ASSL_REQUIRE(stat_replicas >= 1 && stat_replicas <= 64 && (stat_replicas == 1 || sumsq == sum + 64));
+    const int rows = N * Ti, TT = 256 / Fi, tiles = (rows + TT - 1) / TT;
+    ASSL_REQUIRE((long)rows * Fi * 128 < 0x7FFFFF00L);
+    if (!ASSL_ALIGNED16(X) || !ASSL_ALIGNED16(W) || !ASSL_ALIGNED16(Y) || !ASSL_ALIGNED16(Praw)) return ASSL_EALIGN;
+    hipStream_t s = static_cast<hipStream_t>(stream);
+    if (sumsq == sum + 64) {
+        ASSL_ZERO(sum, sizeof(double) * 128 * stat_replicas, s);
+    } else {
+        ASSL_ZERO(sum, sizeof(double) * 64, s);
+        ASSL_ZERO(sumsq, sizeof(double) * 64, s);
+    }
+    ConvArgs a{static_cast<const bf16*>(X), static_cast<const bf16*>(W), bias, static_cast<bf16*>(Y), sum, sumsq, Ti, rows, tiles, 0, 0,
+               stat_replicas, gamma, static_cast<bf16*>(Praw)};
+    const int grid = tiles < 256 ? tiles : 256;
+    static bool pattr[4] = {false, false, false, false};
+#define POOL_LAUNCH(FI_, KEEP_, SLOT)                                                                     \
+    do {                                                                                                  \
+        const size_t lds = 2 * WsGeom<FI_>::BYTES + sizeof(float) * (64 + 4 * 64 * 2) + 4 * 64 * 128 + 512 + 256; \
+        if (!pattr[SLOT]) { if (set_lds(conv3x3_ws_kernel<FI_, true, false, 2, true, KEEP_>, lds)) return ASSL_ELAUNCH; pattr[SLOT] = true; } \
+        hipLaunchKernelGGL((conv3x3_ws_kernel<FI_, true, false, 2, true, KEEP_>), dim3(grid), dim3(256), lds, s, a); \
+    } while (0)
+    if (Fi == 32) { if (Y) POOL_LAUNCH(32, true, 0); else POOL_LAUNCH(32, false, 1); }
+    else          { if (Y) POOL_LAUNCH(16, true, 2); else POOL_LAUNCH(16, false, 3); }
+#undef POOL_LAUNCH
     ASSL_LAUNCH_CHECK();
 }
 
diff --git a/audio-ssl_amd/src/encoder/audiontt.py b/audio-ssl_amd/src/encoder/audiontt.py
--- a/audio-ssl_amd/src/encoder/audiontt.py
+++ b/audio-ssl_amd/src/encoder/audiontt.py
@@ -136,7 +136,7 @@
             x1, x2, x3, h = _EncoderFn.apply(self, x, keep, *params)
         else:
             x1, x2, x3, h, _ = E.encoder_forward(self.param_dict(), x, self.precision, keep=keep, p_drop=self.fc[2].p,
-                                                 train=self.training)
+                                                 train=self.training, need_bwd=False)
         if self.return_all_layers:
             return x1, x2, x3, h
         return h
diff --git a/audio-ssl_amd/src/engine.py b/audio-ssl_amd/src/engine.py
--- a/audio-ssl_amd/src/engine.py
+++ b/audio-ssl_amd/src/engine.py
@@ -266,9 +266,11 @@
 LOSS_REPLICAS = 32
 _BN_STATS_P = os.environ.get("AUDIOSSL_BN_STATS_P", "1") != "0"
 _DP1_BF16 = os.environ.get("AUDIOSSL_DP1_BF16", "1") != "0"
-
-
-def _conv_block_fwd(dtype, Pin, Nimg, Ti, Fi, W, bias, bn, train, update_running, col, packed=None):
+_CONV_POOL = os.environ.get("AUDIOSSL_CONV_POOL", "1") != "0"
+_CONV_WS = int(os.environ.get("AUDIOSSL_CONV_WS", "1")) != 0
+
+
+def _conv_block_fwd(dtype, Pin, Nimg, Ti, Fi, W, bias, bn, train, update_running, col, packed=None, keep_y=True):
     td = N.torch_dtype(dtype)
     if packed is not None:
         Wf, Wd = packed
@@ -277,9 +279,32 @@
         N.call("pack_conv_w", dtype, W, Wf, Wd)
     M = Nimg * Ti * Fi
     ad = _ad(dtype)
-    Y = _empty((M, 64), N.torch_dtype(ad), like=Pin)
     gamma, beta, rm, rv = bn
     fused = dtype == N.BF16 and Fi in (16, 32)
+    if fused and ad == dtype and _CONV_POOL and _CONV_WS and Ti % 2 == 0 and M * 128 < 0x7FFFFF00:
+        rep = STAT_REPLICAS if (train and SYNC_BN is None) else 1
+        sq = ARENA.scratch((rep, 2, 64), torch.float64, Pin)
+        Y = _empty((M, 64), td, like=Pin) if keep_y else None
+        Pout = _empty((Nimg, Ti // 2, Fi // 2, 64), td, like=Pin)
+        N.call("conv3x3_pool_fwd", Pin, Wf, bias, gamma, Y, Pout, sq[0, 0], sq[0, 1], rep, Nimg, Ti, Fi)
+        if train and SYNC_BN is None:
+            st = _empty((4, 64), torch.float32, like=Pin)
+            N.call("bn_relu_pooled_train_fwd", dtype, Pout, sq[0, 0], sq[0, 1], rep, float(M), gamma, beta, rm if update_running else None,
+                   rv if update_running else None, BN_MOMENTUM, BN_EPS, Pout, st[0], st[1], st[2], st[3], Nimg, Ti // 2, Fi // 2)
+            return Y, Pout, (st[0], st[1], st[2], st[3]), Wf, Wd
+        if train:
+            st = _empty((4, 64), torch.float32, like=Pin)
+            sq = sq[0]
+            SYNC_BN.all_reduce(sq)
+            N.call("bn_finalize", sq[0], sq[1], 1, float(M * SYNC_BN.world), 64, gamma, beta, rm if update_running else None,
+                   rv if update_running else None, BN_MOMENTUM, BN_EPS, st[0], st[1], st[2], st[3])
+            scale, shift, mean, rstd = st[0], st[1], st[2], st[3]
+        else:
+            scale, shift = _bn_eval(Pin, 64, gamma, beta, rm, rv)
+            mean = rstd = None
+        N.call("bn_relu_pooled_fwd", dtype, Pout, scale, shift, Pout, Nimg, Ti // 2, Fi // 2)
+        return Y, Pout, (scale, shift, mean, rstd), Wf, Wd
+    Y = _empty((M, 64), N.torch_dtype(ad), like=Pin)
     rep = STAT_REPLICAS if (fused and train and SYNC_BN is None) else 1
     sq = ARENA.scratch((rep, 2, 64), torch.float64, Pin) if (fused and train) else None
     if fused:
@@ -333,13 +358,14 @@
 
 
 def encoder_forward(P, x, dtype, keep=None, p_drop=0.3, train=True, update_running=True, want_layers=True, Wc=None,
-                    layer_out=None, before_fc=None, stem_moments=None):
+                    layer_out=None, before_fc=None, stem_moments=None, need_bwd=True):
     Nimg, _, F, T = x.shape
     assert F == 64, "the HIP encoder is built for n_mels = 64 (the reference's only setting)"
     td = N.torch_dtype(dtype)
     c = EncoderCtx()
     c.P = P
     c.dtype, c.N, c.F, c.T, c.train, c.p_drop = dtype, Nimg, F, T, train, p_drop
+    c.need_bwd = need_bwd
     img = x.reshape(Nimg, F, T).contiguous()
     c.img = img
     w1 = P["features_1.0.weight"].reshape(64, 9)
@@ -383,11 +409,13 @@
     packs = [_empty((64, 576), td, like=x) for _ in range(4)]
     N.call("pack_conv_w2", dtype, P["features_2.0.weight"], packs[0], packs[1], P["features_3.0.weight"], packs[2], packs[3])
     c.Y2, c.P2, c.st2, c.W2f, c.W2d = _conv_block_fwd(dtype, c.P1, Nimg, T1, F1, P["features_2.0.weight"],
-                                                       P["features_2.0.bias"], bn2, train, update_running, col, packed=packs[:2])
+                                                       P["features_2.0.bias"], bn2, train, update_running, col, packed=packs[:2],
+                                                       keep_y=need_bwd)
     T2, F2 = T1 // 2, F1 // 2
     bn3 = (P["features_3.1.weight"], P["features_3.1.bias"], P["features_3.1.running_mean"], P["features_3.1.running_var"])
     c.Y3, c.P3, c.st3, c.W3f, c.W3d = _conv_block_fwd(dtype, c.P2, Nimg, T2, F2, P["features_3.0.weight"],
-                                                       P["features_3.0.bias"], bn3, train, update_running, col, packed=packs[2:])
+                                                       P["features_3.0.bias"], bn3, train, update_running, col, packed=packs[2:],
+                                                       keep_y=need_bwd)
     del col
     T3, F3 = T2 // 2, F2 // 2
     c.dims = (T1, F1, T2, F2, T3, F3)
@@ -466,6 +494,7 @@
     T1, F1, T2, F2, T3, F3 = c.dims
     td = N.torch_dtype(dtype)
     assert c.train, "backward needs a train-mode forward (batch statistics)"
+    assert c.need_bwd, "this forward ran with need_bwd=False: the conv outputs were not kept"
     if dA2 is None:
         dA2 = _empty((M, d), td, like=c.H2)
         N.call("relu_bwd", dtype, dH2.contiguous(), c.H2, dA2, M * d)
diff --git a/audio-ssl_amd/src/upstream/decar_v2/model.py b/audio-ssl_amd/src/upstream/decar_v2/model.py
--- a/audio-ssl_amd/src/upstream/decar_v2/model.py
+++ b/audio-ssl_amd/src/upstream/decar_v2/model.py
@@ -71,7 +71,8 @@
         params = self.encoder_parameters()
         if torch.is_grad_enabled() and any(p.requires_grad for p in params):
             return _EncoderFn.apply(self, x, keep, *params)[3]
-        return E.encoder_forward(self.param_dict(), x, self.precision, keep=keep, p_drop=self.fc[2].p, train=self.training)[3]
+        return E.encoder_forward(self.param_dict(), x, self.precision, keep=keep, p_drop=self.fc[2].p, train=self.training,
+                                 need_bwd=False)[3]
 
     def project(self, z):
         ph = self.projection_head
diff --git a/audio-ssl_amd/src/upstream/delores_m/upstream_expert.py b/audio-ssl_amd/src/upstream/delores_m/upstream_expert.py
--- a/audio-ssl_amd/src/upstream/delores_m/upstream_expert.py
+++ b/audio-ssl_amd/src/upstream/delores_m/upstream_expert.py
@@ -103,7 +103,7 @@
             keepk = ek.encoder.next_keep_mask(B, x.shape[-1])
             _, _, _, Hk, _ = E.encoder_forward(ek.encoder.param_dict(), x, dt, keep=keepk, p_drop=0.3, train=self.training,
                                                Wc=strip(Wk, "encoder."), layer_out=tuple(y[B:] for y in Ys),
-                                               stem_moments=None if moms is None else moms[1])
+                                               stem_moments=None if moms is None else moms[1], need_bwd=False)
             yk, _ = E.maxmean_forward(dt, Hk)
             wk = Wk["fc.weight"]
             return E.linear_fwd(dt, yk, wk, B, wk.shape[0], wk.shape[1], bias=ek.fc.bias.data, out_f32=1)
diff --git a/include/audiossl_hip.h b/include/audiossl_hip.h
--- a/include/audiossl_hip.h
+++ b/include/audiossl_hip.h
@@ -75,6 +75,12 @@
                                     double count, const float* gamma, const float* beta, float* running_mean, float* running_var,
                                     float momentum, float eps, void* P, float* scale, float* shift, float* save_mean, float* save_rstd,
                                     int N, int Ti, int Fi, void* stream);
+int audiossl_bn_relu_pooled_fwd(int dtype, const void* Praw, const float* scale, const float* shift, void* P, int N, int To, int Fo,
+                                void* stream);
+int audiossl_bn_relu_pooled_train_fwd(int dtype, const void* Praw, const double* sum, const double* sumsq, int stat_replicas,
+                                      double count, const float* gamma, const float* beta, float* running_mean, float* running_var,
+                                      float momentum, float eps, void* P, float* scale, float* shift, float* save_mean,
+                                      float* save_rstd, int N, int To, int Fo, void* stream);
 int audiossl_tmean_fwd(int dtype, int out_f32, const void* P, void* xl, int N, int To, int Fo, void* stream);
 int audiossl_tmean3_fwd(int dtype, int out_f32, const void* P1, void* x1, const float* x1_parts, int To1, int Fo1, const void* P2,
                         void* x2, int To2, int Fo2, const void* P3, void* x3, int To3, int Fo3, int N, void* stream);
@@ -114,6 +120,8 @@
 
 int audiossl_conv3x3_fwd(const void* X, const void* W, const float* bias, void* Y, int out_f32, double* sum,
                          double* sumsq, int stat_replicas, int N, int Ti, int Fi, void* stream);
+int audiossl_conv3x3_pool_fwd(const void* X, const void* W, const float* bias, const float* gamma, void* Y, void* Praw, double* sum,
+                              double* sumsq, int stat_replicas, int N, int Ti, int Fi, void* stream);
 int audiossl_conv3x3_wgrad(const void* dY, const void* X, float* dWp, float* workspace, long workspace_floats, int N, int Ti,
                            int Fi, void* stream);
 
```

Result: faster. 271,400 clips/s, median of 6 (+1.4%).
